# Shizheng-Wen/GAOT-3D

Hardware: AMD Instinct MI355X
Metric: mesh-points/sec fwd+bwd, 500K-pt DrivAerNet++ sample (higher is better)
Workload: dtype bf16; 1 GPU; configs[1]: one 500000-point car-like surface sample, latent 64x64x32, knn k=8 encoder + flipped decoder, C=32 P=2 d=256 h=8 F=1024 L=10 rope, attention dropout 0.1 (training mode), MSE + AdamW step; CSR build and geoembed stats inside the step (a decoder list that is the encoder's with its rows swapped shares the encoder's two lists); points=500000, edges=4000000, edges_decoder=4000000, layers=10, precision=bf16, points_per_gpu=500000, point_order=random

## Files before the change

gaot_3d_amd/_lib.py:

```python
from __future__ import annotations

import ctypes as C
import os

_HERE = os.path.dirname(os.path.abspath(__file__))
LIB_PATH = os.environ.get("GAOT_LIB") or os.path.join(_HERE, "lib", "libgaot3d_hip.so")

MAX_MLP_LAYERS = 5


class GaotError(RuntimeError):
    pass


class MlpT(C.Structure):
    _fields_ = [("n_hidden", C.c_int), ("hidden", C.c_int), ("channels", C.c_int),
                ("weight", C.c_void_p * MAX_MLP_LAYERS), ("bias", C.c_void_p * MAX_MLP_LAYERS)]


class MlpGradT(C.Structure):
    _fields_ = [("weight", C.c_void_p * MAX_MLP_LAYERS), ("bias", C.c_void_p * MAX_MLP_LAYERS)]


_lib = None

_p, _i, _i64, _sz, _f, _d = C.c_void_p, C.c_int, C.c_int64, C.c_size_t, C.c_float, C.c_double

SIGNATURES = {
    "gaot_abi_version": (_i, []),
    "gaot_last_error": (C.c_char_p, []),
    "gaot_launch_count": (_i64, [_i]),
    "gaot_csr_workspace_bytes": (_sz, [_i64, _i64]),
    "gaot_csr_build": (_i, [_p, _i, _i64, _i, _i64, _p, _p, _p, _p, _p, _sz, _p]),
    "gaot_gno_fwd_workspace_bytes": (_sz, [_i64, _i]),
    "gaot_gno_fwd": (_i, [C.POINTER(MlpT), _p, _p, _p, _p, _p, _p, _i64, _i64, _p, _i, _p, _sz, _p]),
    "gaot_gno_bwd_workspace_bytes": (_sz, [C.POINTER(MlpT), _i64, _i64]),
    "gaot_gno_bwd": (_i, [C.POINTER(MlpT), _p, _p, _p, _p, _p, _p, _p, _p, _i64, _i64, _i64, _p,
                          C.POINTER(MlpGradT), _i, _p, _sz, _p]),
    "gaot_gno_bwd_coords": (_i, [C.POINTER(MlpT), _p, _p, _p, _p, _p, _p, _p, _p, _i64, _i64, _i64, _p,
                                 C.POINTER(MlpGradT), _p, _i, _p, _sz, _p]),
    "gaot_geoembed_stats_workspace_bytes": (_sz, []),
    "gaot_geoembed_moments": (_i, [_p, _p, _p, _p, _i64, _p, _p]),
    "gaot_geoembed_from_moments": (_i, [_p, _i64, _p, _p, _sz, _p]),
    "gaot_geoembed_raw": (_i, [_p, _p, _p, _p, _i64, _p, _p, _p, _sz, _p]),
    "gaot_geoembed_finalize": (_i, [_p, _i64, _p, _i64, _p, _sz, _p]),
    "gaot_geoembed_from_moments_bwd_workspace_bytes": (_sz, [_i64]),
    "gaot_geoembed_from_moments_bwd": (_i, [_p, _p, _i64, _p, _p, _sz, _p]),
    "gaot_geoembed_moments_bwd": (_i, [_p, _p, _p, _p, _i64, _p, _p, _p, _p]),
    "gaot_gemm_workspace_bytes": (_sz, [_i64, _i64, _i64]),
    "gaot_gemm": (_i, [_p, _p, _p, _i64, _i64, _i64, _i64, _i64, _i64, _i, _i, _p, _i, _p, _i64, _p, _i, _p, _sz, _p]),
    "gaot_gemm_ex": (_i, [_p, _p, _p, _i64, _i64, _i64, _i64, _i64, _i64, _i, _i, _i, _i, _i, _p, _i, _p, _i64, _p, _i, _p,
                          _sz, _p]),
    "gaot_attn_fwd": (_i, [_p, _p, _p, _p, _p, _i64, _i64, _i64, _i64, _i, _i, _i, _i, _i, _f, _f, _p, _i, _i, _i, _p]),
    "gaot_attn_bwd": (_i, [_p] * 10 + [_i64] * 8 + [_i, _i, _i, _i, _i, _f, _f, _p, _i, _i, _i, _i, _p]),
    "gaot_attn_bwd_fused_f32_scratch_bytes": (_i64, [_i, _i, _i]),
    "gaot_attn_bwd_fused_f32": (_i, [_p] * 10 + [_i64] * 8 + [_i, _i, _i, _i, _i, _f, _f, _p, _i, _i, _i, _p, C.c_size_t, _p]),
    "gaot_attn_hd_fwd": (_i, [_p, _p, _p, _p, _p, _i64, _i64, _i64, _i64, _i, _i, _i, _i, _i, _f, _f, _p, _i, _i, _p]),
    "gaot_attn_hd_bwd": (_i, [_p] * 10 + [_i64] * 8 + [_i, _i, _i, _i, _i, _f, _f, _p, _i, _i, _i, _p]),
    "gaot_attn_dropout_mask": (_i, [_p, _f, _i, _i, _i, _p, _p]),
    "gaot_dropout_seed_next": (_i, [_p, C.c_uint64, _p, _p]),
    "gaot_dropout_seed_block": (_i, [_p, C.c_uint64, _i, _p, _p]),
    "gaot_attn_bf16_image_bytes": (_sz, [_i, _i, _i, _i]),
    "gaot_rope_table": (_i, [_p, _i, _i, _p, _p]),
    "gaot_qkv_image": (_i, [_p, _p, _p, _i64, _i64, _i64, _i, _i, _i, _p, _f, _p]),
    "gaot_qkv_image_packed": (_i, [_p, _p, _p, _i64, _i64, _i64, _i64, _i, _i, _p, _f, _i, _p]),
    "gaot_pack_heads": (_i, [_p, _p, _i64, _i, _i, _i, _p, _p, _i, _i, _i, _p]),
    "gaot_attn_bwd_bf16_scratch_bytes": (_sz, [_i, _i, _i, _i]),
    "gaot_attn_bwd_bf16_fused_eligible": (_i, [_i, _i, _i, _i]),
    "gaot_attn_fwd_bf16": (_i, [_p, _p, _p, _p, _p, _i, _i, _i, _i, _i, _f, _f, _p, _i, _i, _p]),
    "gaot_attn_bwd_bf16": (_i, [_p, _p, _p, _p, _p, _p, _p, _p, _i, _i, _i, _i, _i, _f, _f, _p, _i, _i, _i, _p]),
    "gaot_rmsnorm_fwd": (_i, [_p, _p, _p, _p, _p, _i64, _i, _f, _p]),
    "gaot_rmsnorm_bwd_workspace_bytes": (_sz, [_i64, _i]),
    "gaot_rmsnorm_bwd": (_i, [_p, _p, _p, _p, _p, _p, _p, _i64, _i, _p, _sz, _p]),
    "gaot_rmsnorm_bwd2": (_i, [_p, _p, _p, _p, _p, _p, _p, _p, _i64, _i, _p, _sz, _p]),
    "gaot_colsum_workspace_bytes": (_sz, [_i64, _i64]),
    "gaot_colsum": (_i, [_p, _i64, _i64, _i64, _p, _p, _sz, _p]),
    "gaot_gemm_ex_partials": (_i, [_p, _p, _p, _i64, _i64, _i64, _i64, _i64, _i64, _i, _i, _i, _i, _i, _p, _sz, _p, _p, _p]),
    "gaot_rmsnorm_bwd_parts": (_i64, [_i64]),
    "gaot_colsum_parts": (_i64, [_i64]),
    "gaot_reduce_multi": (_i, [_p, _i, _p]),
    "gaot_rope": (_i, [_p, _i64, _i64, _i, _i, _i, _i, _p, _i, _p]),
    "gaot_swiglu_fwd": (_i, [_p, _p, _i64, _i, _p]),
    "gaot_swiglu_bwd": (_i, [_p, _p, _p, _i64, _i, _p]),
    "gaot_adamw_step": (_i, [_p, _i, _p, _p, _d, _d, _d, _d, _p]),
    "gaot_mlp2_fwd": (_i, [_p, _i64, _i, _i, _i, _p, _p, _p, _p, _p, _p]),
    "gaot_mlp2_bwd_workspace_bytes": (_sz, [_i, _i]),
    "gaot_mlp2_bwd": (_i, [_p, _i64, _i, _i, _i, _p, _p, _p, _p, _p, _p, _p, _p, _p, _sz, _p]),
    "gaot_knn_grid": (_i, [_p, _i64, _p, _p, _i, _p, _p]),
    "gaot_radius_grid_count": (_i, [_p, _i64, _p, _p, _f, _i, _p, _p]),
    "gaot_radius_grid_fill": (_i, [_p, _i64, _p, _p, _f, _i, _p, _p, _p, _p]),
    "gaot_knn_brute": (_i, [_p, _i64, _p, _i64, _i, _p, _p]),
    "gaot_radius_brute_count": (_i, [_p, _i64, _p, _i64, _f, _i, _p, _p]),
    "gaot_radius_brute_fill": (_i, [_p, _i64, _p, _i64, _f, _i, _p, _p, _p, _p]),
    "gaot_exclusive_scan_workspace_bytes": (_sz, [_i64]),
    "gaot_exclusive_scan_i32": (_i, [_p, _i64, _p, _p, _sz, _p]),
    "gaot_segment_cap_flags": (_i, [_p, _p, _i64, _i, _p, _p]),
    "gaot_unique_pair_flags": (_i, [_p, _p, _i64, _p, _p]),
    "gaot_random_keep_flags": (_i, [_p, _i64, _d, _p, _p]),
    "gaot_dropout": (_i, [_p, _p, _d, _i64, _p, _p]),
    "gaot_segment_random_cap_flags": (_i, [_p, _p, _p, _i64, _i, _p, _p]),
    "gaot_compact_pairs": (_i, [_p, _p, _p, _p, _i64, _p, _p, _p]),
    "gaot_cast_bf16": (_i, [_p, _p, _i64, _p]),
    "gaot_cast_bf16_multi": (_i, [_p, _i, _p]),
    "gaot_cast_bf16_transpose_multi": (_i, [_p, _p, _p, _i, _p]),
    "gaot_swiglu_fwd_bf16": (_i, [_p, _p, _i64, _i, _p]),
    "gaot_ffn_w13_swiglu": (_i, [_p, _p, _p, _p, _i64, _i64, _i64, _i, _p]),
    "gaot_ffn_w2_bwd_swiglu": (_i, [_p, _p, _p, _p, _i64, _i64, _i64, _i, _p]),
    "gaot_swiglu_bwd_bf16": (_i, [_p, _p, _p, _i64, _i, _p]),
    "gaot_ffn_packed_bytes": (_i64, [_i, _i]),
    "gaot_ffn_pack": (_i, [_p, _p, _i, _p, _i, _p]),
    "gaot_ffn_pack_multi": (_i, [_p, _i, _i, _i, _p]),
    "gaot_ffn_fwd": (_i, [_p, _p, _p, _i64, _p, _p, _p, _i64, _i, _p]),
    "gaot_norm_ffn_fwd": (_i, [_p, _i64, _p, _f, _p, _p, _p, _p, _i64, _i, _p]),
    "gaot_block_packed_bytes": (_i64, [_i]),
    "gaot_block_pack_multi": (_i, [_p, _i, _i, _p]),
    "gaot_block_tail_fwd": (_i, [_p, _i64, _p, _i64, _p, _f, _p, _p, _p, _p, _p, _i64, _i, _p]),
    "gaot_qkv_packed_bytes": (_i64, [_i64, _i]),
    "gaot_qkv_pack_multi": (_i, [_p, _i, _i64, _i, _p]),
    "gaot_norm_qkv_image": (_i, [_p, _i64, _p, _f, _p, _p, _p, _p, _i64, _i, _i, _i, _p, _f, _p]),
    "gaot_skip_packed_bytes": (_i64, []),
    "gaot_skip_pack_multi": (_i, [_p, _i, _p]),
    "gaot_cat_norm_qkv_image": (_i, [_p, _i64, _p, _i64, _p, _p, _p, _p, _f, _p, _p, _p, _p, _i64, _i, _i, _i, _p, _f, _p]),
    "gaot_norm_bwd_parts": (_i64, [_i64]),
    "gaot_ffn_bwd_norm": (_i, [_p, _p, _p, _p, _i64, _p, _p, _p, _p, _p, _p, _p, _i64, _i, _p]),
    "gaot_qkv_bwd_norm": (_i, [_p, _i64, _p, _p, _i64, _p, _p, _p, _p, _p, _p, _i64, _p]),
    "gaot_qkv_bwd_norm_cat": (_i, [_p, _i64, _p, _p, _i64, _p, _p, _p, _p, _p, _p, _p, _i, _p, _i64, _p]),
    "gaot_oproj_bwd_image": (_i, [_p, _p, _p, _i, _p, _p, _i64, _i, _p]),
    "gaot_ffn_bwd_dag": (_i, [_p, _p, _p, _p, _p, _p, _i64, _i, _p]),
    "gaot_ffn_bwd": (_i, [_p, _p, _p, _p, _p, _p, _p, _i, _i64, _i, _p]),
    "gaot_act_bwd": (_i, [_p, _p, _p, _i64, _i, _p]),
    "gaot_act_fwd": (_i, [_p, _p, _i64, _i, _p]),
    "gaot_axpy": (_i, [_p, _p, _f, _p, _i64, _i64, _p]),
    "gaot_stream_copy": (_i, [_p, _p, _i64, _p]),
    "gaot_stream_copy_ex": (_i, [_p, _p, _i64, _i, _p]),
    "gaot_patchify": (_i, [_p, _p, _i, _i, _i, _i, _i, _i, _i, _p]),
    "gaot_mse_workspace_bytes": (_sz, []),
    "gaot_mse_fwd": (_i, [_p, _p, _i64, _p, _p, _sz, _p]),
    "gaot_mse_bwd": (_i, [_p, _p, _i64, _p, _p, _p]),
    "gaot_gather_rows": (_i, [_p, _i64, _p, _i64, _i, _p, _i64, _p]),
    "gaot_segment_reduce": (_i, [_p, _i64, _p, _p, _i64, _i, _i, _p, _p, _p]),
    "gaot_segment_reduce_bwd": (_i, [_p, _p, _p, _p, _i64, _i64, _i, _i, _p, _p]),
    "gaot_segment_softmax_fwd": (_i, [_p, _p, _i64, _p, _p]),
    "gaot_segment_softmax_bwd": (_i, [_p, _p, _p, _i64, _p, _p]),
    "gaot_edge_coords": (_i, [_p, _p, _p, _p, _i64, _i, _p, _i64, _p]),
    "gaot_mul": (_i, [_p, _p, _i64, _i, _i, _p, _p]),
    "gaot_mul_rowsum": (_i, [_p, _p, _i64, _i, _p, _p]),
    "gaot_affine_cols": (_i, [_p, _p, _p, _i64, _i, _p, _p]),
    "gaot_scale_mix_fwd": (_i, [_p, _i, _p, _p, _p, _i64, _i, _p]),
    "gaot_scale_mix_bwd": (_i, [_p, _i, _p, _p, _p, _p, _i64, _i, _p]),
}


def load():
    global _lib
    if _lib is not None:
        return _lib
    if not os.path.exists(LIB_PATH):
        raise GaotError(f"{LIB_PATH} not found: build it with `python -c 'import __graft_entry__ as g; g.build()'` "
                        f"or `make -C gaot_3d_amd/csrc` (there is no CPU/PyTorch fallback)")
    lib = C.CDLL(LIB_PATH)
    for name, (res, args) in SIGNATURES.items():
        fn = getattr(lib, name)
        fn.restype = res
        fn.argtypes = args
    if lib.gaot_abi_version() != 11:
        raise GaotError("libgaot3d_hip.so ABI version mismatch")
    _lib = lib
    return lib


def check(rc: int, what: str):
    if rc != 0:
        msg = load().gaot_last_error()
        raise GaotError(f"{what} failed (code {rc}): {msg.decode() if msg else ''}")
```

gaot_3d_amd/csrc/attn_bf16.hip:

```cpp
#include <stdlib.h>

#include <type_traits>

#include "attn_dropout.h"
#include "common.h"
#include "tile32.h"

namespace {

constexpr int D = 32;
constexpr float LOG2E = 1.4426950408889634f;
constexpr float LN2 = 0.6931471805599453f;
typedef float f32x2 __attribute__((ext_vector_type(2)));

__device__ __forceinline__ float xhalf(float v) { return __shfl_xor(v, 32, 64); }
__device__ __forceinline__ float max_halves(float v) {
    const unsigned u = __builtin_bit_cast(unsigned, v);
    const auto r = __builtin_amdgcn_permlane32_swap(u, u, false, false);
    return fmaxf(__builtin_bit_cast(float, (unsigned)r[0]), __builtin_bit_cast(float, (unsigned)r[1]));
}

__device__ __forceinline__ void stage_load4(uint4 (&regs)[2], const bf16_t* pa, int64_t lda, const bf16_t* pb, int64_t ldb,
                                            int64_t row0, int64_t nrows) {
#pragma unroll
// ... 67 lines not shown
                          float* __restrict__ delta, int B, int S, int H) {
    const int64_t i = (int64_t)blockIdx.x * blockDim.x + threadIdx.x;
    const int64_t n = (int64_t)B * S * H;
    if (i >= n) return;
    const int head = (int)(i % H);
    const int64_t row = i / H;
    const float* dp = d_o + row * H * D + head * D;
    const float* op = o + row * H * D + head * D;
    bf16_t* yp = dob + row * H * D + head * D;
    float s = 0.f;
#pragma unroll
    for (int c = 0; c < D / 4; ++c) {
        const float4 a = *reinterpret_cast<const float4*>(dp + 4 * c);
        const float4 b = *reinterpret_cast<const float4*>(op + 4 * c);
        s += a.x * b.x + a.y * b.y + a.z * b.z + a.w * b.w;
        const uint2 pk = make_uint2((unsigned)f2bf(a.x) | ((unsigned)f2bf(a.y) << 16),
                                    (unsigned)f2bf(a.z) | ((unsigned)f2bf(a.w) << 16));
        *reinterpret_cast<uint2*>(yp + 4 * c) = pk;
    }
    delta[((row / S) * H + head) * S + (row % S)] = s;
}

__global__ void k_delta_bf16(const bf16_t* __restrict__ dob, const float* __restrict__ o, float* __restrict__ delta, int B,
                             int S, int H) {
    const int64_t i = (int64_t)blockIdx.x * blockDim.x + threadIdx.x;
    const int64_t n = (int64_t)B * S * H;
    if (i >= n) return;
    const int head = (int)(i % H);
    const int64_t row = i / H;
    const bf16_t* dp = dob + row * H * D + head * D;
    const float* op = o + row * H * D + head * D;
    float s = 0.f;
#pragma unroll
    for (int c = 0; c < D / 8; ++c) {
        const uint4 a = *reinterpret_cast<const uint4*>(dp + 8 * c);
        const float4 b0 = *reinterpret_cast<const float4*>(op + 8 * c), b1 = *reinterpret_cast<const float4*>(op + 8 * c + 4);
        s += __uint_as_float(a.x << 16) * b0.x + __uint_as_float(a.x & 0xffff0000u) * b0.y + __uint_as_float(a.y << 16) * b0.z +
             __uint_as_float(a.y & 0xffff0000u) * b0.w + __uint_as_float(a.z << 16) * b1.x + __uint_as_float(a.z & 0xffff0000u) * b1.y +
             __uint_as_float(a.w << 16) * b1.z + __uint_as_float(a.w & 0xffff0000u) * b1.w;
    }
    delta[((row / S) * H + head) * S + (row % S)] = s;
}

struct FwdArgs {
    const bf16_t* qkv;
    float* o;
    float* lse;
    int64_t ld;
    int B, S, H, HKV;
    gdrop::Drop drop;
    int chunk;
    int64_t o_part, lse_part;
    const float* kmax2;
    int* redo;
};

constexpr int KN_BLOCKS = 64;
__global__ __launch_bounds__(256) void k_key_norm_max(const bf16_t* __restrict__ img, int64_t ld, int S, int H, int HKV,
                                                      float* __restrict__ out) {
    __shared__ float red[4];
    const int b = blockIdx.y, hkv = blockIdx.z;
    float m = 0.f;
    for (int64_t row = (int64_t)blockIdx.x * 256 + threadIdx.x; row < S; row += (int64_t)KN_BLOCKS * 256) {
        const bf16_t* kp = img + ((int64_t)b * S + row) * ld + (H + hkv) * D;
        float n2 = 0.f;
#pragma unroll
        for (int c = 0; c < D / 8; ++c) {
            const uint4 a = *reinterpret_cast<const uint4*>(kp + 8 * c);
            const unsigned w[4] = {a.x, a.y, a.z, a.w};
#pragma unroll
            for (int j = 0; j < 4; ++j) {
                const float lo = __uint_as_float(w[j] << 16), hi = __uint_as_float(w[j] & 0xffff0000u);
                n2 = fmaf(lo, lo, fmaf(hi, hi, n2));
            }
        }
        m = fmaxf(m, n2);
    }
#pragma unroll
    for (int o = 32; o > 0; o >>= 1) m = fmaxf(m, __shfl_xor(m, o, 64));
    if ((threadIdx.x & 63) == 0) red[threadIdx.x >> 6] = m;
    __syncthreads();
    if (threadIdx.x == 0) out[((int64_t)b * KN_BLOCKS + blockIdx.x) * HKV + hkv] = fmaxf(fmaxf(red[0], red[1]), fmaxf(red[2], red[3]));
}

template <int NTILES>
__device__ __forceinline__ void stage_col_words(uint32_t* bw_s, uint32_t ck, int64_t k0) {
    if (threadIdx.x < 16 * NTILES) {
        const int t = threadIdx.x >> 4, jj = threadIdx.x & 15;
        bw_s[t * 16 + ((jj >> 1) & 1) * 8 + (jj >> 2) * 2 + (jj & 1)] = gdrop::col_word(ck, (uint32_t)(k0 >> 1) + threadIdx.x);
    }
}
template <bool ZERO>
__device__ __forceinline__ void drop_select(f32x16& v, const f32x16& other, uint32_t aw, const uint32_t* bw_tile, int hf,
                                            uint32_t thr) {
    const uint4 w0 = *reinterpret_cast<const uint4*>(bw_tile + hf * 8);
    const uint4 w1 = *reinterpret_cast<const uint4*>(bw_tile + hf * 8 + 4);
    const uint32_t wd[8] = {w0.x, w0.y, w0.z, w0.w, w1.x, w1.y, w1.z, w1.w};
#pragma unroll
    for (int j = 0; j < 8; ++j) {
        const uint32_t x = aw ^ wd[j];
        v[2 * j] = ((x & 0xffffu) >= thr) ? v[2 * j] : (ZERO ? 0.f : other[2 * j]);
        v[2 * j + 1] = ((x >> 16) >= thr) ? v[2 * j + 1] : (ZERO ? 0.f : other[2 * j + 1]);
    }
}

typedef short s16x2 __attribute__((ext_vector_type(2)));
// ... 16 lines not shown

constexpr float RESCALE_SUM = 64.0f;
template <int OCC, int TPM, bool DROP, bool FAST, int FSB = 0>
__global__ __launch_bounds__(256, OCC) void k_attn_fwd_bf16(FwdArgs a) {
    __shared__ __attribute__((aligned(16))) char lds[2 * TPM * TILE_BYTES];
    __shared__ __attribute__((aligned(16))) uint32_t bw_s[DROP ? 16 * TPM : 4];
    const int wave = threadIdx.x >> 6, lane = threadIdx.x & 63, l31 = lane & 31, hf = lane >> 5;
    const int head = blockIdx.x % a.H, b = blockIdx.z;
    const int hkv = head / (a.H / a.HKV);
    const int64_t q0 = (int64_t)(blockIdx.x / a.H) * 128 + wave * 32;
    const int64_t rowbase = (int64_t)b * a.S;
    const bf16_t* qp = a.qkv + rowbase * a.ld + head * D;
    const bf16_t* kp = a.qkv + rowbase * a.ld + (a.H + hkv) * D;
    const bf16_t* vp = a.qkv + rowbase * a.ld + (a.H + a.HKV + hkv) * D;

    bf16x8 qf[2];
    {
        const int64_t qi = q0 + l31;
#pragma unroll
        for (int s = 0; s < 2; ++s) {
            if (qi < a.S) qf[s] = *reinterpret_cast<const bf16x8*>(qp + qi * a.ld + 16 * s + 8 * hf);
            else {
#pragma unroll
                for (int j = 0; j < 8; ++j) qf[s][j] = 0;
            }
        }
    }
    f32x16 acc, negm;
#pragma unroll
    for (int r = 0; r < 16; ++r) { acc[r] = 0.f; negm[r] = 0.f; }
    float m = 0.f, l = 0.f;
    uint32_t aw = 0, ck = 0;
    if constexpr (DROP) {
        const unsigned long long seed = *a.drop.seed;
        const int bh = a.drop.bh(b, head);
        aw = gdrop::row_word(gdrop::row_key(seed, bh), (uint32_t)(q0 + l31)) ^ 0x80008000u;
        ck = gdrop::col_key(seed, bh);
    }
    const short ts = (short)((int)a.drop.thr - 1 - 32768);
    const s16x2 tpk = {ts, ts};

    const int wg = blockIdx.x + gridDim.x * (blockIdx.y + gridDim.y * blockIdx.z);
    if constexpr (FAST) {
        constexpr float BOUND2 = 54.f * 54.f;
        float q2 = 0.f;
#pragma unroll
        for (int s = 0; s < 2; ++s)
#pragma unroll
            for (int j = 0; j < 8; ++j) {
                const float v = __uint_as_float((unsigned)(unsigned short)qf[s][j] << 16);
                q2 = fmaf(v, v, q2);
            }
        q2 += xhalf(q2);
        float k2 = a.kmax2[((int64_t)b * KN_BLOCKS + lane) * a.HKV + hkv];
#pragma unroll
        for (int o = 32; o > 0; o >>= 1) k2 = fmaxf(k2, __shfl_xor(k2, o, 64));
        const int over = __syncthreads_or(!(q2 * k2 <= BOUND2));
        if (threadIdx.x == 0) a.redo[wg] = over ? 1 : 0;
        if (over) return;
    } else {
        if (a.redo[wg] == 0) return;
    }

    const int64_t lo = (int64_t)blockIdx.y * a.chunk, hi = min((int64_t)a.S, lo + a.chunk);
    uint4 regs[TPM];
    stage_loadN<TPM>(regs, kp, a.ld, vp, a.ld, lo, a.S);
    for (int64_t k0 = lo; k0 < hi; k0 += 32 * TPM) {
        __syncthreads();
        stage_storeN<TPM>(regs, lds);
        if constexpr (DROP) stage_col_words<TPM>(bw_s, ck, k0);
        __syncthreads();
        if (k0 + 32 * TPM < hi) stage_loadN<TPM>(regs, kp, a.ld, vp, a.ld, k0 + 32 * TPM, a.S);
        auto do_tile = [&](int t, int64_t kb) {
            const char* kt = lds + t * TILE_BYTES;
            const char* vt = lds + (TPM + t) * TILE_BYTES;
            const bool first = (kb == lo);
            f32x16 sc;
            auto scores = [&]() {
                sc = __builtin_amdgcn_mfma_f32_32x32x16_bf16(frag_rows(kt, l31, hf, 0), qf[0], negm, 0, 0, 0);
                sc = __builtin_amdgcn_mfma_f32_32x32x16_bf16(frag_rows(kt, l31, hf, 1), qf[1], sc, 0, 0, 0);
                if (kb + 32 > a.S) {
                    const int nv = (int)(a.S - kb);
    #pragma unroll
                    for (int r = 0; r < 16; ++r)
                        if (mfma32_row(r, hf) >= nv) sc[r] = -INFINITY;
                }
            };
            if constexpr (FAST) {
                if constexpr ((FSB & 1) != 0) __builtin_amdgcn_sched_barrier(0);
                f32x16 zero;
    #pragma unroll
                for (int r = 0; r < 16; ++r) zero[r] = 0.f;
                sc = __builtin_amdgcn_mfma_f32_32x32x16_bf16(frag_rows(kt, l31, hf, 0), qf[0], zero, 0, 0, 0);
                sc = __builtin_amdgcn_mfma_f32_32x32x16_bf16(frag_rows(kt, l31, hf, 1), qf[1], sc, 0, 0, 0);
                if (kb + 32 > a.S) {
                    const int nv = (int)(a.S - kb);
    #pragma unroll
                    for (int r = 0; r < 16; ++r)
                        if (mfma32_row(r, hf) >= nv) sc[r] = -INFINITY;
                }
    #pragma unroll
                for (int r = 0; r < 16; ++r) sc[r] = __builtin_amdgcn_exp2f(sc[r]);
                if constexpr ((FSB & 2) != 0) __builtin_amdgcn_sched_barrier(0);
                bf16x8 p0, p1;
                acc_to_frags(sc, p0, p1);
                if constexpr ((FSB & 8) != 0) {
                    typedef __bf16 bf16x2_t __attribute__((ext_vector_type(2)));
// ... 1292 lines not shown
            for (int g = 0; g < 4; ++g) {
                float4 t = make_float4(dk[4 * g] * ksc, dk[4 * g + 1] * ksc, dk[4 * g + 2] * ksc, dk[4 * g + 3] * ksc);
                *reinterpret_cast<float4*>(dkp + 8 * g + 4 * hf) = unrope4(t, a.freqs, (int)ki, g, hf);
                float4 u = make_float4(dv[4 * g] * vsc, dv[4 * g + 1] * vsc, dv[4 * g + 2] * vsc, dv[4 * g + 3] * vsc);
                *reinterpret_cast<float4*>(dvp + 8 * g + 4 * hf) = u;
            }
        }
    });
}

#include "attn_fwd_asm.inc"
struct FwdAsmLds {
    static constexpr int QT = GAOT_ATTN_FWD_ASM_QT, KT = GAOT_ATTN_FWD_ASM_KT;
    static constexpr int STAGE = 0;
    static constexpr int BW = STAGE + 2 * KT * TILE_BYTES;
    static constexpr int TOTAL = BW + 16 * KT * 4;
    static constexpr int QUERIES = 4 * QT * 32, KEYS = KT * 32;
};
template <bool DROP, int LAB = 0>
__global__ __launch_bounds__(256, 1) void k_attn_fwd_asm(FwdArgs a) {
    using L = FwdAsmLds;
    constexpr int QT = L::QT, KT = L::KT;
    __shared__ __attribute__((aligned(1024))) char lds[L::TOTAL];
    const int wave = threadIdx.x >> 6, lane = threadIdx.x & 63, l31 = lane & 31, hf = lane >> 5;
    const int head = blockIdx.x % a.H, b = blockIdx.z, qblk = blockIdx.x / a.H;
    const int hkv = head / (a.H / a.HKV);
    const int64_t q0 = (int64_t)qblk * L::QUERIES + wave * (QT * 32);
    const int64_t rowbase = (int64_t)b * a.S;
    const bf16_t* qp = a.qkv + rowbase * a.ld + head * D;
    const bf16_t* kp = a.qkv + rowbase * a.ld + (a.H + hkv) * D;
    const bf16_t* vp = a.qkv + rowbase * a.ld + (a.H + a.HKV + hkv) * D;

    float q2max = 0.f;
    static_for<0, QT>([&](auto qc) {
        constexpr int qt = decltype(qc)::value;
        const int64_t qi = q0 + 32 * qt + l31;
        float q2 = 0.f;
        static_for<0, 2>([&](auto sc) {
            constexpr int s = decltype(sc)::value;
            const uint4 f = *reinterpret_cast<const uint4*>(qp + qi * a.ld + 16 * s + 8 * hf);
            agpr_write4<8 * qt + 4 * s>(f);
            const unsigned w[4] = {f.x, f.y, f.z, f.w};
#pragma unroll
            for (int j = 0; j < 4; ++j) {
                const float lo = __uint_as_float(w[j] << 16), hi = __uint_as_float(w[j] & 0xffff0000u);
                q2 = fmaf(lo, lo, fmaf(hi, hi, q2));
            }
        });
        q2 += xhalf(q2);
        q2max = fmaxf(q2max, q2);
    });
    {
        constexpr float BOUND2 = 54.f * 54.f;
        float k2 = a.kmax2[((int64_t)b * KN_BLOCKS + lane) * a.HKV + hkv];
#pragma unroll
        for (int o = 32; o > 0; o >>= 1) k2 = fmaxf(k2, __shfl_xor(k2, o, 64));
        const int over = __syncthreads_or(!(q2max * k2 <= BOUND2));
        if (threadIdx.x < 4)
            a.redo[(qblk * 4 + threadIdx.x) * a.H + head + (int64_t)(a.S / 128) * a.H * (blockIdx.y + gridDim.y * b)] = over ? 1 : 0;
        if (over) return;
    }
    uint32_t aw[QT] = {0, 0, 0, 0}, ck = 0;
    if constexpr (DROP) {
        const unsigned long long seed = *a.drop.seed;
        const int bh = a.drop.bh(b, head);
        const uint32_t rk = gdrop::row_key(seed, bh);
        ck = gdrop::col_key(seed, bh);
#pragma unroll
        for (int qt = 0; qt < QT; ++qt) aw[qt] = gdrop::row_word(rk, (uint32_t)(q0 + 32 * qt + l31)) ^ 0x80008000u;
    }
    const uint32_t ts = (uint32_t)((int)a.drop.thr - 1 - 32768) & 0xffffu;
    const uint32_t tpk = ts | (ts << 16);
    asm volatile(GAOT_ATTN_FWD_ASM_ZERO_ACC ::: GAOT_ATTN_FWD_ASM_ACC_CLOBBERS);
    float l0[QT] = {0.f, 0.f, 0.f, 0.f}, l1[QT] = {0.f, 0.f, 0.f, 0.f};

    const unsigned lbase = (unsigned)(uintptr_t)(__attribute__((address_space(3))) char*)lds;
    const unsigned a_k0 = lbase + L::STAGE + tile_off(l31, hf), a_k1 = lbase + L::STAGE + tile_off(l31, 2 + hf);
    unsigned a_v0, a_v1;
    {
        const int i = lane & 15, grp = (lane >> 4) & 1, col = 16 * grp + 4 * (i & 3), r0 = 4 * hf + (i >> 2), r1 = r0 + 8;
        a_v0 = lbase + L::STAGE + tile_off(r0, col >> 3) + ((col & 7) << 1);
        a_v1 = lbase + L::STAGE + tile_off(r1, col >> 3) + ((col & 7) << 1);
    }
    const unsigned a_w = lbase + L::BW + hf * 32;
    uint32_t* bw_s = reinterpret_cast<uint32_t*>(lds + L::BW);

    const int64_t lo = (int64_t)blockIdx.y * a.chunk, hi = min((int64_t)a.S, lo + a.chunk);
    uint4 regs[KT];
    stage_loadN<KT>(regs, kp, a.ld, vp, a.ld, lo, a.S);
    for (int64_t k0 = lo; k0 < hi; k0 += L::KEYS) {
        __syncthreads();
        stage_storeN<KT>(regs, lds + L::STAGE);
        if constexpr (DROP) stage_col_words<KT>(bw_s, ck, k0);
        __syncthreads();
        if (k0 + L::KEYS < hi) stage_loadN<KT>(regs, kp, a.ld, vp, a.ld, k0 + L::KEYS, a.S);
        if constexpr (LAB == 1) continue;
#if GAOT_ATTN_FWD_ASM_LSUM_MFMA
        if constexpr (DROP)
            asm volatile(GAOT_ATTN_FWD_STAGE_ASM_DROP
                         :: [a_k0] "v"(a_k0), [a_k1] "v"(a_k1), [a_v0] "v"(a_v0), [a_v1] "v"(a_v1), [a_w] "v"(a_w),
                            [aw0] "v"(aw[0]), [aw1] "v"(aw[1]), [aw2] "v"(aw[2]), [aw3] "v"(aw[3]), [tpk] "s"(tpk)
                         : GAOT_ATTN_FWD_STAGE_ASM_CLOBBERS);
        else
            asm volatile(GAOT_ATTN_FWD_STAGE_ASM_NODROP
                         :: [a_k0] "v"(a_k0), [a_k1] "v"(a_k1), [a_v0] "v"(a_v0), [a_v1] "v"(a_v1)
                         : GAOT_ATTN_FWD_STAGE_ASM_CLOBBERS);
#else
// ... 85 lines not shown
    const int64_t li = ((row / S) * H + head) * S + (row % S);
    float mx = -INFINITY;
    for (int p = 0; p < P; ++p) mx = fmaxf(mx, lse_parts[p * lse_part + li]);
    float den = 0.f;
    for (int p = 0; p < P; ++p) den += __expf(lse_parts[p * lse_part + li] - mx);
    float4 acc = make_float4(0.f, 0.f, 0.f, 0.f);
    const int64_t oi = row * (H * D) + head * D + 4 * g;
    for (int p = 0; p < P; ++p) {
        const float w = __expf(lse_parts[p * lse_part + li] - mx) / den;
        const float4 v = *reinterpret_cast<const float4*>(o_parts + p * o_part + oi);
        acc.x += w * v.x; acc.y += w * v.y; acc.z += w * v.z; acc.w += w * v.w;
    }
    *reinterpret_cast<float4*>(o + oi) = acc;
    if (g == 0) lse[li] = mx + logf(den);
}

__global__ void k_sum_parts(const float* __restrict__ parts, int P, int64_t part, int64_t n4, float* __restrict__ out) {
    const int64_t i = (int64_t)blockIdx.x * blockDim.x + threadIdx.x;
    if (i >= n4) return;
    float4 acc = reinterpret_cast<const float4*>(parts)[i];
    for (int p = 1; p < P; ++p) {
        const float4 v = reinterpret_cast<const float4*>(parts + p * part)[i];
        acc.x += v.x; acc.y += v.y; acc.z += v.z; acc.w += v.w;
    }
    reinterpret_cast<float4*>(out)[i] = acc;
}

__global__ void k_sum_cols(const float* __restrict__ parts, int P, int64_t part, int64_t rows, int ld, int col0, int ncols,
                           float* __restrict__ out) {
    const int64_t i = (int64_t)blockIdx.x * blockDim.x + threadIdx.x;
    const int c4 = ncols / 4;
    if (i >= rows * c4) return;
    const int64_t off = (i / c4) * ld + col0 + 4 * (i % c4);
    float4 acc = *reinterpret_cast<const float4*>(parts + off);
    for (int p = 1; p < P; ++p) {
        const float4 v = *reinterpret_cast<const float4*>(parts + p * part + off);
        acc.x += v.x; acc.y += v.y; acc.z += v.z; acc.w += v.w;
    }
    *reinterpret_cast<float4*>(out + off) = acc;
}

int split_parts(int64_t wgs, int S) {
    constexpr int tgt = 2048;
    if (wgs >= tgt / 2) return 1;
    int p = (int)std::min<int64_t>(8, ceil_div(tgt, wgs));
    p = std::min(p, std::max(1, S / 1024));
    return std::max(p, 1);
}
int split_chunk(int S, int P) { return (int)(ceil_div(ceil_div(S, P), 128) * 128); }

}

static size_t align256(size_t v) { return (v + 255) & ~(size_t)255; }
static size_t key_norm_off(int B, int S, int H, int HKV) { return (sizeof(bf16_t) * (size_t)B * S * (H + 2 * HKV) * D + 64 + 15) & ~(size_t)15; }
static size_t fwd_flags(int B, int S, int H) { return (size_t)B * 8 * (size_t)ceil_div(S, 128) * H; }
static size_t image_only_bytes(int B, int S, int H, int HKV) {
    return align256(key_norm_off(B, S, H, HKV) + sizeof(float) * (size_t)B * KN_BLOCKS * HKV + sizeof(int) * fwd_flags(B, S, H));
}

extern "C" size_t gaot_attn_bf16_image_bytes(int B, int S, int H, int HKV) {
    const int P = split_parts(ceil_div(S, 128) * H * B, S);
    size_t parts = P > 1 ? (size_t)P * ((size_t)B * S * H * D + (size_t)B * H * S) * sizeof(float) : 0;
    return image_only_bytes(B, S, H, HKV) + parts;
}
static size_t fused_dqpart_bytes(int B, int S, int H) { return (size_t)B * H * (size_t)ceil_div(S, 512) * (size_t)S * D * sizeof(bf16_t); }
static int fused_parts(int B, int S, int HKV) {
    const int64_t wgs = (int64_t)ceil_div(S, 512) * HKV * B;
    int p = 1;
    while (wgs * p < 256 && p < 8 && S / (2 * p) >= 1024) p *= 2;
    return p;
}
static int fused_chunk(int S, int P) { return (int)(ceil_div(ceil_div(S, P), 64) * 64); }
static bool fused_bwd_ok(int B, int S, int H, int HKV) {
    return (int64_t)ceil_div(S, 512) * HKV * B * fused_parts(B, S, HKV) >= 128 && fused_dqpart_bytes(B, S, H) <= ((size_t)1 << 30) &&
           (int64_t)S * (H + 2 * HKV) * D * 2 < 0x7fffffff;
}
extern "C" int gaot_attn_bwd_bf16_fused_eligible(int B, int S, int H, int HKV) { return fused_bwd_ok(B, S, H, HKV) ? 1 : 0; }
static size_t bwd_parts_bytes(int B, int S, int H, int HKV) {
    const int P = std::max(split_parts(ceil_div(S, 128) * H * B, S), fused_bwd_ok(B, S, H, HKV) ? fused_parts(B, S, HKV) : 1);
    return P > 1 ? align256((size_t)P * (size_t)B * S * (H + 2 * HKV) * D * sizeof(float)) : 0;
}
extern "C" size_t gaot_attn_bwd_bf16_scratch_bytes(int B, int S, int H, int HKV) {
    const size_t dqpart = fused_bwd_ok(B, S, H, HKV) ? fused_dqpart_bytes(B, S, H) : 0;
    return align256(sizeof(bf16_t) * (size_t)B * S * H * D + 64) + bwd_parts_bytes(B, S, H, HKV) + dqpart;
}

extern "C" int gaot_attn_fwd_bf16(const float* qkv, const float* rope_freqs, void* qkv_image, float* o, float* lse,
                                  int B, int S, int H, int HKV, int head_dim, float scale, float dropout_p,
                                  const unsigned long long* dropout_seed, int head0, int heads_total, gaot_stream_t stream) {
    GAOT_ENTER();
    if (head_dim != D) {
        gaot_set_error("gaot_attn_fwd_bf16: head_dim %d unsupported (only 32)", head_dim);
        return GAOT_ERR_UNSUPPORTED;
    }
    GAOT_CHECK_ARG(B > 0 && S > 0 && H > 0 && HKV > 0 && H % HKV == 0, "bad shape");
    GAOT_CHECK_ARG(qkv_image && o && lse, "null pointer");
    GAOT_CHECK_ARG((((uintptr_t)qkv | (uintptr_t)qkv_image | (uintptr_t)o) & 15) == 0, "buffers must be 16-byte aligned");
    GAOT_CHECK_ARG(dropout_p >= 0.f && dropout_p < 1.f && (dropout_p == 0.f || dropout_seed), "dropout_p in [0,1) and a seed");
    GAOT_CHECK_ARG(heads_total == 0 || (head0 >= 0 && head0 + H <= heads_total), "head0 + H <= heads_total");
    hipStream_t st = (hipStream_t)stream;
    const int ld = (H + 2 * HKV) * D;
    const int64_t rows = (int64_t)B * S;
    const int64_t n = rows * (ld / 2);
    if (qkv)
        GAOT_KLAUNCH(k_prep_qkv, dim3((unsigned)ceil_div(n, 256)), dim3(256), 0, st, qkv, (bf16_t*)qkv_image, rows, ld, H,
                     HKV, S, rope_freqs, scale * LOG2E);
    float* kmax2 = reinterpret_cast<float*>(reinterpret_cast<char*>(qkv_image) + key_norm_off(B, S, H, HKV));
    int* redo = reinterpret_cast<int*>(kmax2 + (size_t)B * KN_BLOCKS * HKV);
    GAOT_KLAUNCH(k_key_norm_max, dim3(KN_BLOCKS, (unsigned)B, (unsigned)HKV), dim3(256), 0, st, (const bf16_t*)qkv_image,
                 (int64_t)ld, S, H, HKV, kmax2);
    const int P = split_parts(ceil_div(S, 128) * H * B, S);
    float* o_parts = reinterpret_cast<float*>(reinterpret_cast<char*>(qkv_image) + image_only_bytes(B, S, H, HKV));
    const int64_t o_part = rows * H * D, lse_part = (int64_t)B * H * S;
    float* lse_parts = o_parts + (size_t)P * o_part;
    FwdArgs a{(const bf16_t*)qkv_image, P > 1 ? o_parts : o, P > 1 ? lse_parts : lse, ld, B, S, H, HKV,
              gdrop::make_drop(dropout_seed, dropout_p, H, head0, heads_total), P > 1 ? split_chunk(S, P) : S, o_part, lse_part, kmax2, redo};
    const dim3 fgrid((unsigned)(ceil_div(S, 128) * H), (unsigned)(P > 1 ? ceil_div(S, a.chunk) : 1), (unsigned)B);
    static const int fwd_lab = [] { const char* e = getenv("GAOT_ATTN_FWD_LAB"); return e ? atoi(e) : 0; }();
    const bool dot2 = fwd_lab == 8 || (fwd_lab != 1 && a.drop.thr);
    const bool fwd_asm = [] { const char* e = getenv("GAOT_ATTN_FWD_ASM"); return !e || atoi(e) != 0; }();
    if (fwd_asm && fwd_lab == 0 && S % FwdAsmLds::QUERIES == 0 && (P == 1 || a.chunk % FwdAsmLds::KEYS == 0) &&
        (int64_t)(S / FwdAsmLds::QUERIES) * H * B * fgrid.y >= 128) {
        const dim3 agrid((unsigned)((S / FwdAsmLds::QUERIES) * H), fgrid.y, (unsigned)B);
        static const int asm_lab = [] { const char* e = getenv("GAOT_ATTN_FWD_ASM_LAB"); return e ? atoi(e) : 0; }();
        if (asm_lab == 1) {
            if (a.drop.thr) GAOT_KLAUNCH((k_attn_fwd_asm<true, 1>), agrid, dim3(256), 0, st, a);
            else GAOT_KLAUNCH((k_attn_fwd_asm<false, 1>), agrid, dim3(256), 0, st, a);
        } else if (a.drop.thr) {
            GAOT_KLAUNCH((k_attn_fwd_asm<true>), agrid, dim3(256), 0, st, a);
            GAOT_KLAUNCH((k_attn_fwd_bf16<3, 4, true, false>), fgrid, dim3(256), 0, st, a);
        } else {
            GAOT_KLAUNCH((k_attn_fwd_asm<false>), agrid, dim3(256), 0, st, a);
            GAOT_KLAUNCH((k_attn_fwd_bf16<3, 4, false, false>), fgrid, dim3(256), 0, st, a);
        }
    } else if (a.drop.thr) {
        if (dot2) GAOT_KLAUNCH((k_attn_fwd_bf16<4, 4, true, true, 8>), fgrid, dim3(256), 0, st, a);
        else GAOT_KLAUNCH((k_attn_fwd_bf16<4, 4, true, true>), fgrid, dim3(256), 0, st, a);
        GAOT_KLAUNCH((k_attn_fwd_bf16<3, 4, true, false>), fgrid, dim3(256), 0, st, a);
    } else {
        if (dot2) GAOT_KLAUNCH((k_attn_fwd_bf16<4, 4, false, true, 8>), fgrid, dim3(256), 0, st, a);
        else GAOT_KLAUNCH((k_attn_fwd_bf16<4, 4, false, true>), fgrid, dim3(256), 0, st, a);
        GAOT_KLAUNCH((k_attn_fwd_bf16<3, 4, false, false>), fgrid, dim3(256), 0, st, a);
    }
    if (P > 1)
        GAOT_KLAUNCH(k_attn_combine, dim3((unsigned)ceil_div(rows * H * 8, 256)), dim3(256), 0, st, o_parts, lse_parts,
                           (int)fgrid.y, o_part, lse_part, B, S, H, o, lse);
    GAOT_LAUNCH_CHECK();
    return GAOT_OK;
}

extern "C" int gaot_attn_bwd_bf16(const void* qkv_image, const float* o, const float* d_o, const float* lse,
                                  void* do_image, float* delta, float* dqkv, const float* rope_freqs, int B, int S, int H,
                                  int HKV, int head_dim, float scale, float dropout_p,
                                  const unsigned long long* dropout_seed, int head0, int heads_total, int phase_mask,
                                  gaot_stream_t stream) {
    GAOT_ENTER();
    if (head_dim != D) {
        gaot_set_error("gaot_attn_bwd_bf16: head_dim %d unsupported (only 32)", head_dim);
        return GAOT_ERR_UNSUPPORTED;
    }
    GAOT_CHECK_ARG(B > 0 && S > 0 && H > 0 && HKV > 0 && H % HKV == 0, "bad shape");
    GAOT_CHECK_ARG(qkv_image && o && (d_o || !(phase_mask & 1)) && lse && do_image && delta && dqkv, "null pointer");
    GAOT_CHECK_ARG(dropout_p >= 0.f && dropout_p < 1.f && (dropout_p == 0.f || dropout_seed), "dropout_p in [0,1) and a seed");
    GAOT_CHECK_ARG(heads_total == 0 || (head0 >= 0 && head0 + H <= heads_total), "head0 + H <= heads_total");
    hipStream_t st = (hipStream_t)stream;
    const int ld = (H + 2 * HKV) * D;
    const int P0 = split_parts(ceil_div(S, 128) * H * B, S);
    const bool kb_dkv = (int64_t)ceil_div(S, 256) * HKV * B >= 512, kb_dq = (int64_t)ceil_div(S, 256) * H * B >= 512;
    const int P = (kb_dkv || kb_dq) ? 1 : P0;
// ... 126 lines not shown
```

gaot_3d_amd/csrc/csr.hip:

```cpp
#include "csr_impl.h"

extern "C" size_t gaot_csr_workspace_bytes(int64_t num_edges, int64_t num_rows) {
    (void)num_rows;
    const int64_t nblk = ceil_div(num_edges, RS_TILE);
    const int64_t tn = 256 * nblk;
    const int64_t nbt = ceil_div(tn, SCAN_TILE);
    return sizeof(int) * (size_t)(4 + 4 * num_edges + 2 * (tn + 1) + nbt + 1) + 64;
}

extern "C" int gaot_csr_build(const void* edge_index, int index_is_i64, int64_t num_edges, int sort_row,
                              int64_t num_rows, int32_t* rowptr, int32_t* perm, int32_t* key_sorted,
                              int32_t* other_sorted, void* workspace, size_t workspace_bytes, gaot_stream_t stream) {
    GAOT_ENTER();
    GAOT_CHECK_ARG(num_edges >= 0 && num_rows >= 0, "negative size");
    GAOT_CHECK_ARG(num_edges < (int64_t)1 << 31 && num_rows < ((int64_t)1 << 31) - 1, "sizes must fit int32");
    GAOT_CHECK_ARG(sort_row == 0 || sort_row == 1, "sort_row must be 0 or 1");
    GAOT_CHECK_ARG(rowptr && workspace, "null pointer");
    GAOT_CHECK_ARG(num_edges == 0 || (edge_index && perm && key_sorted && other_sorted), "null pointer");
    GAOT_CHECK_ARG(workspace_bytes >= gaot_csr_workspace_bytes(num_edges, num_rows), "workspace too small");
    hipStream_t st = (hipStream_t)stream;
    int rc = index_is_i64 ? csr_build_t<int64_t>((const int64_t*)edge_index, num_edges, sort_row, num_rows, rowptr,
                                                 perm, key_sorted, other_sorted, workspace, st)
                          : csr_build_t<int32_t>((const int32_t*)edge_index, num_edges, sort_row, num_rows, rowptr,
                                                 perm, key_sorted, other_sorted, workspace, st);
    if (rc != GAOT_OK) return rc;
    GAOT_LAUNCH_CHECK();
    return GAOT_OK;
}
```

gaot_3d_amd/csrc/csr_impl.h:

```cpp
#pragma once
#include "common.h"

namespace {

__global__ void k_zero_flags(int* __restrict__ p, int n) {
    if ((int)threadIdx.x < n) p[threadIdx.x] = 0;
}

template <typename IDX>
__global__ void k_check_sorted(const IDX* __restrict__ keys, int64_t E, int* __restrict__ unsorted) {
    int64_t i = (int64_t)blockIdx.x * blockDim.x + threadIdx.x;
    const int64_t stride = (int64_t)gridDim.x * blockDim.x;
    bool bad = false;
    for (; i < E; i += stride) bad |= (i > 0) && (keys[i] < keys[i - 1]);
    if (__any(bad) && (threadIdx.x & 63) == 0) *unsorted = 1;
}

template <typename IDX>
__global__ void k_sorted_build(const IDX* __restrict__ keys, const IDX* __restrict__ other, int64_t E, int64_t Q,
                               const int* __restrict__ unsorted, int* __restrict__ rowptr, int* __restrict__ perm,
                               int* __restrict__ key_sorted, int* __restrict__ other_sorted) {
    if (*unsorted) return;
    int64_t i = (int64_t)blockIdx.x * blockDim.x + threadIdx.x;
    const int64_t stride = (int64_t)gridDim.x * blockDim.x;
    for (; i < E; i += stride) {
        const int k = (int)keys[i];
        perm[i] = (int)i;
        key_sorted[i] = k;
        other_sorted[i] = (int)other[i];
        const int kprev = (i > 0) ? (int)keys[i - 1] : -1;
        for (int r = kprev + 1; r <= k; ++r) rowptr[r] = (int)i;
        if (i == E - 1)
            for (int64_t r = (int64_t)k + 1; r <= Q; ++r) rowptr[r] = (int)E;
    }
}

constexpr int SCAN_BLOCK = 256;
constexpr int SCAN_ITEMS = 8;
constexpr int SCAN_TILE = SCAN_BLOCK * SCAN_ITEMS;

__global__ void k_scan_reduce(const int* __restrict__ in, int64_t n, int* __restrict__ block_sums) {
    __shared__ int red[SCAN_BLOCK / 64];
    const int64_t base = (int64_t)blockIdx.x * SCAN_TILE;
    int s = 0;
#pragma unroll
    for (int j = 0; j < SCAN_ITEMS; ++j) {
        int64_t i = base + (int64_t)threadIdx.x * SCAN_ITEMS + j;
        if (i < n) s += in[i];
    }
#pragma unroll
    for (int o = 32; o > 0; o >>= 1) s += __shfl_xor(s, o, 64);
    if ((threadIdx.x & 63) == 0) red[threadIdx.x >> 6] = s;
    __syncthreads();
    if (threadIdx.x == 0) {
        int t = 0;
        for (int w = 0; w < SCAN_BLOCK / 64; ++w) t += red[w];
        block_sums[blockIdx.x] = t;
    }
}

__global__ void k_scan_blocksums(int* __restrict__ block_sums, int nb) {
    __shared__ int carry;
    __shared__ int wsum[SCAN_BLOCK / 64];
    if (threadIdx.x == 0) carry = 0;
    __syncthreads();
    for (int base = 0; base < nb; base += SCAN_BLOCK) {
        int i = base + threadIdx.x;
        int v = (i < nb) ? block_sums[i] : 0;
        int incl = v;
        const int lane = threadIdx.x & 63;
#pragma unroll
        for (int o = 1; o < 64; o <<= 1) {
            int t = __shfl_up(incl, o, 64);
            if (lane >= o) incl += t;
        }
        if (lane == 63) wsum[threadIdx.x >> 6] = incl;
        __syncthreads();
        int woff = 0;
        for (int w = 0; w < (int)(threadIdx.x >> 6); ++w) woff += wsum[w];
        const int c = carry;
        if (i < nb) block_sums[i] = c + woff + incl - v;
        __syncthreads();
        if (threadIdx.x == SCAN_BLOCK - 1) carry = c + woff + incl;
        __syncthreads();
    }
}

__global__ void k_scan_apply(const int* __restrict__ in, int64_t n, const int* __restrict__ block_offs,
                             int* __restrict__ out) {
    __shared__ int wsum[SCAN_BLOCK / 64];
    const int64_t base = (int64_t)blockIdx.x * SCAN_TILE + (int64_t)threadIdx.x * SCAN_ITEMS;
    int v[SCAN_ITEMS];
    int s = 0;
#pragma unroll
    for (int j = 0; j < SCAN_ITEMS; ++j) {
        v[j] = (base + j < n) ? in[base + j] : 0;
        s += v[j];
    }
    int incl = s;
    const int lane = threadIdx.x & 63;
#pragma unroll
    for (int o = 1; o < 64; o <<= 1) {
        int t = __shfl_up(incl, o, 64);
        if (lane >= o) incl += t;
    }
    if (lane == 63) wsum[threadIdx.x >> 6] = incl;
    __syncthreads();
    int off = block_offs[blockIdx.x];
    for (int w = 0; w < (int)(threadIdx.x >> 6); ++w) off += wsum[w];
    int run = off + incl - s;
#pragma unroll
    for (int j = 0; j < SCAN_ITEMS; ++j) {
        if (base + j < n) {
            out[base + j] = run;
        }
        run += v[j];
        if (base + j == n - 1) out[n] = run;
    }
}

constexpr int RS_TILE = 4096;
constexpr int RS_ROUNDS = RS_TILE / 256;

template <typename KIN>
__global__ __launch_bounds__(256) void k_rs_hist(const KIN* __restrict__ keys, int64_t E, int shift, int nd, int nblk,
                                                 int* __restrict__ table, const int* __restrict__ unsorted) {
    __shared__ int h[256];
    if (!*unsorted) return;
    h[threadIdx.x] = 0;
    __syncthreads();
    const int64_t base = (int64_t)blockIdx.x * RS_TILE;
#pragma unroll 4
    for (int j = 0; j < RS_ROUNDS; ++j) {
        const int64_t i = base + j * 256 + threadIdx.x;
        if (i < E) atomicAdd(&h[((int)keys[i] >> shift) & (nd - 1)], 1);
    }
    __syncthreads();
    if ((int)threadIdx.x < nd) table[(int64_t)threadIdx.x * nblk + blockIdx.x] = h[threadIdx.x];
}

template <typename KIN>
__global__ __launch_bounds__(256) void k_rs_scatter(const KIN* __restrict__ keys_in, const int* __restrict__ ids_in,
                                                    int64_t E, int shift, int nbits, int nblk,
                                                    const int* __restrict__ table, int* __restrict__ keys_out,
                                                    int* __restrict__ ids_out, const int* __restrict__ unsorted) {
    __shared__ int wcnt[4][256];
    if (!*unsorted) return;
    const int wave = threadIdx.x >> 6, lane = threadIdx.x & 63;
    const int nd = 1 << nbits;
    const int64_t base = (int64_t)blockIdx.x * RS_TILE + (int64_t)wave * (RS_ROUNDS * 64);
    for (int i = threadIdx.x; i < 4 * 256; i += 256) (&wcnt[0][0])[i] = 0;
    __syncthreads();
    int key[RS_ROUNDS], rnk[RS_ROUNDS];
    const unsigned long long lt = (1ull << lane) - 1ull;
#pragma unroll
    for (int j = 0; j < RS_ROUNDS; ++j) {
        const int64_t idx = base + j * 64 + lane;
        const bool valid = idx < E;
        const int k = valid ? (int)keys_in[idx] : 0;
        const int d = (k >> shift) & (nd - 1);
        unsigned long long m = __ballot(valid);
        for (int b = 0; b < nbits; ++b) {
            const bool bit = (d >> b) & 1;
            const unsigned long long bb = __ballot(bit);
            m &= bit ? bb : ~bb;
        }
        const int r = __popcll(m & lt);
        const int before = wcnt[wave][d];
        rnk[j] = before + r;
        key[j] = k;
        if (valid && r == 0) wcnt[wave][d] = before + __popcll(m);
    }
    __syncthreads();
    if ((int)threadIdx.x < nd) {
        int run = table[(int64_t)threadIdx.x * nblk + blockIdx.x];
#pragma unroll
        for (int w = 0; w < 4; ++w) {
            const int c = wcnt[w][threadIdx.x];
            wcnt[w][threadIdx.x] = run;
            run += c;
        }
    }
    __syncthreads();
#pragma unroll
    for (int j = 0; j < RS_ROUNDS; ++j) {
        const int64_t idx = base + j * 64 + lane;
        if (idx < E) {
            const int pos = wcnt[wave][(key[j] >> shift) & (nd - 1)] + rnk[j];
            keys_out[pos] = key[j];
            ids_out[pos] = ids_in ? ids_in[idx] : (int)idx;
        }
    }
}

template <typename IDX>
__global__ void k_emit_sorted(const int* __restrict__ keys, const int* __restrict__ ids, const IDX* __restrict__ other,
                              int64_t E, int64_t Q, const int* __restrict__ unsorted, int* __restrict__ rowptr,
                              int* __restrict__ perm, int* __restrict__ key_sorted, int* __restrict__ other_sorted) {
    if (!*unsorted) return;
    int64_t i = (int64_t)blockIdx.x * blockDim.x + threadIdx.x;
    const int64_t stride = (int64_t)gridDim.x * blockDim.x;
    for (; i < E; i += stride) {
        const int k = keys[i], id = ids[i];
        perm[i] = id;
        key_sorted[i] = k;
        other_sorted[i] = (int)other[id];
        const int kprev = (i > 0) ? keys[i - 1] : -1;
        for (int r = kprev + 1; r <= k; ++r) rowptr[r] = (int)i;
        if (i == E - 1)
            for (int64_t r = (int64_t)k + 1; r <= Q; ++r) rowptr[r] = (int)E;
    }
}

static int rs_bits(int64_t Q) {
    int b = 1;
    while (((int64_t)1 << b) < Q) ++b;
    return b;
}

template <typename IDX>
int csr_build_t(const IDX* edge_index, int64_t E, int sort_row, int64_t Q, int32_t* rowptr, int32_t* perm,
                int32_t* key_sorted, int32_t* other_sorted, void* ws, hipStream_t st) {
    const IDX* keys = edge_index + (sort_row ? E : 0);
    const IDX* other = edge_index + (sort_row ? 0 : E);
    const int nblk = (int)ceil_div(E, RS_TILE);
    const int64_t tn = (int64_t)256 * nblk;
    int* flags = (int*)ws;
    int* unsorted = flags + 1;
    int* kbuf0 = flags + 4;
    int* kbuf1 = kbuf0 + E;
    int* ibuf0 = kbuf1 + E;
    int* ibuf1 = ibuf0 + E;
    int* table = ibuf1 + E;
    int* tscan = table + tn + 1;
    int* bsum = tscan + tn + 1;
    GAOT_KLAUNCH(k_zero_flags, dim3(1), dim3(64), 0, st, flags, 4);
    if (E == 0) {
        (void)hipMemsetAsync(rowptr, 0, sizeof(int) * (size_t)(Q + 1), st);
        return GAOT_OK;
    }
    const int tb = 256;
    const int gb = (int)std::min<int64_t>(ceil_div(E, tb), 256 * 16);
    GAOT_KLAUNCH((k_check_sorted<IDX>), dim3(gb), dim3(tb), 0, st, keys, E, unsorted);
    GAOT_KLAUNCH((k_sorted_build<IDX>), dim3(gb), dim3(tb), 0, st, keys, other, E, Q, unsorted, rowptr, perm,
                       key_sorted, other_sorted);
    const int bits = rs_bits(Q);
    const int passes = (bits + 7) / 8;
    const int width = (bits + passes - 1) / passes;
    const int* kin = nullptr;
    const int* iin = nullptr;
    for (int p = 0; p < passes; ++p) {
        const int shift = p * width;
        const int nd = 1 << width;
        int* kout = (p & 1) ? kbuf1 : kbuf0;
        int* iout = (p & 1) ? ibuf1 : ibuf0;
        const int64_t n = (int64_t)nd * nblk;
        const int nb = (int)ceil_div(n, SCAN_TILE);
        if (p == 0) GAOT_KLAUNCH((k_rs_hist<IDX>), dim3(nblk), dim3(256), 0, st, keys, E, shift, nd, nblk, table, unsorted);
        else GAOT_KLAUNCH((k_rs_hist<int>), dim3(nblk), dim3(256), 0, st, kin, E, shift, nd, nblk, table, unsorted);
        GAOT_KLAUNCH(k_scan_reduce, dim3(nb), dim3(SCAN_BLOCK), 0, st, table, n, bsum);
        GAOT_KLAUNCH(k_scan_blocksums, dim3(1), dim3(SCAN_BLOCK), 0, st, bsum, nb);
        GAOT_KLAUNCH(k_scan_apply, dim3(nb), dim3(SCAN_BLOCK), 0, st, table, n, bsum, tscan);
        if (p == 0)
            GAOT_KLAUNCH((k_rs_scatter<IDX>), dim3(nblk), dim3(256), 0, st, keys, (const int*)nullptr, E, shift, width,
                               nblk, tscan, kout, iout, unsorted);
        else
            GAOT_KLAUNCH((k_rs_scatter<int>), dim3(nblk), dim3(256), 0, st, kin, iin, E, shift, width, nblk, tscan,
                               kout, iout, unsorted);
        kin = kout;
        iin = iout;
    }
    GAOT_KLAUNCH((k_emit_sorted<IDX>), dim3(gb), dim3(tb), 0, st, kin, iin, other, E, Q, unsorted, rowptr, perm,
                       key_sorted, other_sorted);
    return GAOT_OK;
}

}
```

gaot_3d_amd/csrc/ffn_fused.hip:

```cpp
#include "common.h"

namespace {

typedef unsigned short bf16_t;
typedef unsigned u32x4 __attribute__((ext_vector_type(4)));

#ifndef GAOT_FFN_ABL
#define GAOT_FFN_ABL 0
#endif
#ifdef GAOT_FFN_TIMING
__device__ unsigned long long g_ffn_t[64];
#define FFN_STAMP(i) do { if (blockIdx.x == 0 && threadIdx.x == 0) g_ffn_t[i] = __builtin_readcyclecounter(); } while (0)
#else
#define FFN_STAMP(i) do { } while (0)
#endif
constexpr int D = 256, RB = 64, FC = 128;
constexpr int H_BYTES = RB * D * 2;
constexpr int U_BYTES = RB * FC * 2;
constexpr int AG_BYTES = RB * 2 * FC * 2;

__device__ __forceinline__ unsigned pack2(float a, float b) {
    return (unsigned)__builtin_bit_cast(bf16_t, (__bf16)a) | ((unsigned)__builtin_bit_cast(bf16_t, (__bf16)b) << 16);
}
__device__ __forceinline__ float rbf(float v) { return __uint_as_float((unsigned)__builtin_bit_cast(bf16_t, (__bf16)v) << 16); }
// ... 1368 lines not shown
        gaot_set_error("gaot_oproj_bwd_image: too many rows for 32-bit buffer offsets");
        return GAOT_ERR_UNSUPPORTED;
    }
    const bf16_t* wotp = (const bf16_t*)packed + ((int64_t)2 * F * D + (int64_t)D * F) * 2 + (int64_t)D * D;
    const int nblk = ((int)rows + RB - 1) / RB, per = (nblk + 7) / 8;
    GAOT_KLAUNCH(k_oproj_bwd, dim3((unsigned)(8 * per)), dim3(256), H_BYTES, (hipStream_t)stream, dh, attn_out, (const u32x4*)wotp, (bf16_t*)do_image,
                 delta, (int)rows, S, D / 32);
    GAOT_LAUNCH_CHECK();
    return GAOT_OK;
}

namespace {
struct QkvTable {
    const float* w[PACK_MAX];
    bf16_t* packed[PACK_MAX];
};
__global__ void k_qkv_pack(QkvTable t, int N, int with_backward) {
    const float* w = t.w[blockIdx.y];
    bf16_t* p = t.packed[blockIdx.y];
    const int nfr = N * D / 8;
    for (int id = blockIdx.x * blockDim.x + threadIdx.x; id < nfr * (with_backward ? 2 : 1); id += gridDim.x * blockDim.x) {
        if (id < nfr) {
            const int lane = id & 63, s2 = (id >> 6) & 15, jt = (id >> 10) & 1, wv = (id >> 11) & 3, pn = id >> 13;
            const float* src = w + (int64_t)(256 * pn + 64 * wv + 32 * jt + (lane & 31)) * D + 16 * s2 + 8 * (lane >> 5);
            *reinterpret_cast<u32x4*>(p + (int64_t)id * 8) = u32x4{pack2(src[0], src[1]), pack2(src[2], src[3]), pack2(src[4], src[5]), pack2(src[6], src[7])};
        } else {
            const int i2 = id - nfr, ns = N / 16;
            const int lane = i2 & 63, rest = i2 >> 6, s2 = rest % ns, jt = (rest / ns) & 1, wv = rest / (2 * ns);
            const float* st = w + (int64_t)(16 * s2 + 8 * (lane >> 5)) * D + (wv * 64 + jt * 32 + (lane & 31));
            *reinterpret_cast<u32x4*>(p + (int64_t)id * 8) =
                u32x4{pack2(st[0], st[D]), pack2(st[2 * D], st[3 * D]), pack2(st[4 * D], st[5 * D]), pack2(st[6 * D], st[7 * D])};
        }
    }
}

__global__ void k_skip_pack(QkvTable t) {
    const float* w = t.w[blockIdx.y];
    bf16_t* p = t.packed[blockIdx.y];
    for (int id = blockIdx.x * blockDim.x + threadIdx.x; id < D * 2 * D / 8; id += gridDim.x * blockDim.x) {
        const int lane = id & 63, s2 = (id >> 6) & 31, jt = (id >> 11) & 1, wv = id >> 12;
        const float* src = w + (int64_t)(64 * wv + 32 * jt + (lane & 31)) * (2 * D) + 16 * s2 + 8 * (lane >> 5);
        *reinterpret_cast<u32x4*>(p + (int64_t)id * 8) = u32x4{pack2(src[0], src[1]), pack2(src[2], src[3]), pack2(src[4], src[5]), pack2(src[6], src[7])};
        const int s3 = (id >> 6) & 15, jt3 = (id >> 10) & 1, w3 = (id >> 11) & 3, half = id >> 13;
        const float* st = w + (int64_t)(16 * s3 + 8 * (lane >> 5)) * (2 * D) + (256 * half + 64 * w3 + 32 * jt3 + (lane & 31));
        *reinterpret_cast<u32x4*>(p + (int64_t)D * 2 * D + (int64_t)id * 8) =
            u32x4{pack2(st[0], st[2 * D]), pack2(st[4 * D], st[6 * D]), pack2(st[8 * D], st[10 * D]), pack2(st[12 * D], st[14 * D])};
    }
}

struct QkvArgs {
    const float* X; int ldx; const float* NW; float eps; const u32x4* Wp; bf16_t* IMG; bf16_t* YB; float* RSTD;
    const float* table; int S, nq, nk; float qscale; int M, N;
    const float* XB; int ldxb; const u32x4* WSp; const float* BS; float* XO;
};
constexpr int QKV_LDS = H_BYTES + 256 + 64 * 144, QKV_LDS_CAT = 2 * H_BYTES + 256 + 1024 + 64 * 144;
template <bool CAT>
__global__ __launch_bounds__(256, 1) void k_norm_qkv(QkvArgs a) {
    constexpr int RD = 3, LA = 2;
    extern __shared__ __attribute__((aligned(1024))) char lds[];
    const int wave = threadIdx.x >> 6, lane = threadIdx.x & 63, l31 = lane & 31, hf = lane >> 5;
    const int M = a.M, N = a.N, NP = N / 256;
    const int nblk = (M + RB - 1) / RB, per = (nblk + 7) / 8;
    const int t = (blockIdx.x & 7) * per + (blockIdx.x >> 3);
    if ((int)(blockIdx.x >> 3) >= per || t >= nblk) return;
    const int m0 = t * RB;
    const int wv = __builtin_amdgcn_readfirstlane(wave);
    const __amdgpu_buffer_rsrc_t wrs = __builtin_amdgcn_make_buffer_rsrc((void*)a.Wp, 0, N * D * 2, 0x00020000);
    u32x4 wr[RD][8];
    auto wload = [&](u32x4 (&dst)[8], int g) {
        const int pn = g >> 2, st = g & 3;
#pragma unroll
        for (int jt = 0; jt < 2; ++jt)
#pragma unroll
            for (int s2 = 0; s2 < 4; ++s2)
                dst[jt * 4 + s2] = __builtin_bit_cast(u32x4, __builtin_amdgcn_raw_buffer_load_b128(wrs, lane * 16, ((((pn * 4 + wv) * 2 + jt) * 16) + 4 * st + s2) * 1024, 0));
    };
    wload(wr[0], 0);
    wload(wr[1], 1);
    float* rstd_l = reinterpret_cast<float*>(lds + (CAT ? 2 * H_BYTES : H_BYTES));
    if constexpr (CAT) {
        const int sw0 = l31 & 15;
        const int64_t xab = (int64_t)M * a.ldx * 4, xbb = (int64_t)M * a.ldxb * 4, xob = (int64_t)M * D * 4, ybbytes = (int64_t)M * D * 2;
        const __amdgpu_buffer_rsrc_t xars = __builtin_amdgcn_make_buffer_rsrc((void*)a.X, 0, (int)(xab > 0x7fffffff ? 0x7fffffff : xab), 0x00020000);
        const __amdgpu_buffer_rsrc_t xbrs = __builtin_amdgcn_make_buffer_rsrc((void*)a.XB, 0, (int)(xbb > 0x7fffffff ? 0x7fffffff : xbb), 0x00020000);
        const __amdgpu_buffer_rsrc_t xors = __builtin_amdgcn_make_buffer_rsrc((void*)a.XO, 0, (int)(xob > 0x7fffffff ? 0x7fffffff : xob), 0x00020000);
        const __amdgpu_buffer_rsrc_t ybrs = __builtin_amdgcn_make_buffer_rsrc((void*)a.YB, 0, (int)(ybbytes > 0x7fffffff ? 0x7fffffff : ybbytes), 0x00020000);
        const __amdgpu_buffer_rsrc_t wsrs = __builtin_amdgcn_make_buffer_rsrc((void*)a.WSp, 0, D * 2 * D * 2, 0x00020000);
        u32x4 wo[2][8];
        auto woload = [&](u32x4 (&dst)[8], int st) {
#pragma unroll
            for (int jt = 0; jt < 2; ++jt)
#pragma unroll
                for (int s2 = 0; s2 < 4; ++s2)
                    dst[jt * 4 + s2] = __builtin_bit_cast(u32x4, __builtin_amdgcn_raw_buffer_load_b128(wsrs, lane * 16, (((wv * 2 + jt) * 32) + 4 * st + s2) * 1024, 0));
        };
        woload(wo[0], 0);
        woload(wo[1], 1);
#pragma unroll
        for (int half = 0; half < 2; ++half) {
            f32x4 d0[8], d1[8];
#pragma unroll
            for (int i = 0; i < 8; ++i) {
                const int row = 8 * i + (threadIdx.x >> 5), m = m0 + row;
                const unsigned off = m < M ? (unsigned)m * (unsigned)(half ? a.ldxb : a.ldx) * 4u + (unsigned)(threadIdx.x & 31) * 32u : 0x80000000u;
                d0[i] = __builtin_bit_cast(f32x4, __builtin_amdgcn_raw_buffer_load_b128(half ? xbrs : xars, off, 0, 0));
                d1[i] = __builtin_bit_cast(f32x4, __builtin_amdgcn_raw_buffer_load_b128(half ? xbrs : xars, off, 16, 0));
// ... 79 lines not shown
        }
    } else {
        const int64_t xbytes = (int64_t)M * a.ldx * 4, ybbytes = (int64_t)M * D * 2;
        const __amdgpu_buffer_rsrc_t xrs = __builtin_amdgcn_make_buffer_rsrc((void*)a.X, 0, (int)(xbytes > 0x7fffffff ? 0x7fffffff : xbytes), 0x00020000);
        const __amdgpu_buffer_rsrc_t ybrs = __builtin_amdgcn_make_buffer_rsrc((void*)a.YB, 0, (int)(ybbytes > 0x7fffffff ? 0x7fffffff : ybbytes), 0x00020000);
        const float4 g = reinterpret_cast<const float4*>(a.NW)[lane];
        float4 v[16];
        float ss[16];
#pragma unroll
        for (int j = 0; j < 16; ++j) {
            const int m = m0 + wave * 16 + j;
            v[j] = __builtin_bit_cast(float4, __builtin_amdgcn_raw_buffer_load_b128(xrs, m < M ? (unsigned)m * (unsigned)a.ldx * 4u + lane * 16u : 0x80000000u, 0, 0));
        }
#pragma unroll
        for (int j = 0; j < 16; ++j) {
            ss[j] = 0.f;
            ss[j] += v[j].x * v[j].x + v[j].y * v[j].y + v[j].z * v[j].z + v[j].w * v[j].w;
        }
#pragma unroll
        for (int o = 32; o > 0; o >>= 1)
#pragma unroll
            for (int j = 0; j < 16; ++j) ss[j] += __shfl_xor(ss[j], o, 64);
#pragma unroll
        for (int j = 0; j < 16; ++j) {
            const int rl = wave * 16 + j, m = m0 + rl;
            const float r = rsqrtf(ss[j] / (float)D + a.eps);
            const float4 o = make_float4(v[j].x * r * g.x, v[j].y * r * g.y, v[j].z * r * g.z, v[j].w * r * g.w);
            typedef unsigned u32x2 __attribute__((ext_vector_type(2)));
            const u32x2 pk = {pack2(o.x, o.y), pack2(o.z, o.w)};
            *reinterpret_cast<u32x2*>(lds + rl * 512 + ((((lane >> 1) ^ (rl & 15))) << 4) + 8 * (lane & 1)) = pk;
            __builtin_amdgcn_raw_buffer_store_b64(pk, ybrs, m < M ? (unsigned)m * (unsigned)D * 2u + lane * 8u : 0x80000000u, 0, 0);
            if (lane == 0) {
                rstd_l[rl] = r;
                if (m < M) a.RSTD[m] = r;
            }
        }
    }
    __builtin_amdgcn_s_barrier();
    const int64_t ibytes = (int64_t)M * N * 2;
    const __amdgpu_buffer_rsrc_t irs = __builtin_amdgcn_make_buffer_rsrc((void*)a.IMG, 0, (int)(ibytes > 0x7fffffff ? 0x7fffffff : ibytes), 0x00020000);
    const __amdgpu_buffer_rsrc_t trs = __builtin_amdgcn_make_buffer_rsrc((void*)a.table, 0, a.table ? a.S * 128 : 0, 0x00020000);
    const int sw = l31 & 15;
    const char* hb = lds + l31 * 512;
    char* tabl = lds + (CAT ? QKV_LDS_CAT : QKV_LDS) - 64 * 144;
    {
        const int row = threadIdx.x >> 2, pc = threadIdx.x & 3, m = m0 + row, mm = m < M ? m : M - 1;
        const f32x4 t0 = __builtin_bit_cast(f32x4, __builtin_amdgcn_raw_buffer_load_b128(trs, (mm % a.S) * 128 + 32 * pc, 0, 0));
        const f32x4 t1 = __builtin_bit_cast(f32x4, __builtin_amdgcn_raw_buffer_load_b128(trs, (mm % a.S) * 128 + 32 * pc + 16, 0, 0));
        *reinterpret_cast<f32x4*>(tabl + row * 144 + 32 * pc) = t0;
        *reinterpret_cast<f32x4*>(tabl + row * 144 + 32 * pc + 16) = t1;
    }
    __builtin_amdgcn_s_barrier();
    f32x16 accc[2][2], accn[2][2];
    bf16x8 hn0 = *reinterpret_cast<const bf16x8*>(hb + ((hf ^ sw) << 4)), hn1 = *reinterpret_cast<const bf16x8*>(hb + 32 * 512 + ((hf ^ sw) << 4));
    auto panel_step = [&](f32x16 (&acc)[2][2], int pn, int st, auto epi) {
        const int g = 4 * pn + st;
        auto run = [&](auto rot) {
            constexpr int R = decltype(rot)::value;
            wload(wr[(R + st + LA) % RD], g + LA);
#pragma unroll
            for (int s2 = 0; s2 < 4; ++s2) {
                __builtin_amdgcn_sched_barrier(0);
                const bf16x8 h0 = hn0, h1 = hn1;
                const int slot = ((2 * ((4 * st + s2 + 1) & 15) + hf) ^ sw) << 4;
                hn0 = *reinterpret_cast<const bf16x8*>(hb + slot);
                hn1 = *reinterpret_cast<const bf16x8*>(hb + 32 * 512 + slot);
                const bf16x8 w0 = __builtin_bit_cast(bf16x8, wr[(R + st) % RD][s2]), w1 = __builtin_bit_cast(bf16x8, wr[(R + st) % RD][4 + s2]);
                acc[0][0] = __builtin_amdgcn_mfma_f32_32x32x16_bf16(w0, h0, acc[0][0], 0, 0, 0);
                acc[1][0] = __builtin_amdgcn_mfma_f32_32x32x16_bf16(w1, h0, acc[1][0], 0, 0, 0);
                acc[0][1] = __builtin_amdgcn_mfma_f32_32x32x16_bf16(w0, h1, acc[0][1], 0, 0, 0);
                acc[1][1] = __builtin_amdgcn_mfma_f32_32x32x16_bf16(w1, h1, acc[1][1], 0, 0, 0);
                epi(4 * st + s2);
                __builtin_amdgcn_sched_group_barrier(0x100, 2, 0);
#pragma unroll
                for (int k = 0; k < 4; ++k) {
                    __builtin_amdgcn_sched_group_barrier(0x008, 1, 0);
                    __builtin_amdgcn_sched_group_barrier(0x002, 8, 0);
                }
            }
        };
        const int rot = (4 * pn) % 3;
        if (rot == 0) run(std::integral_constant<int, 0>{});
        else if (rot == 1) run(std::integral_constant<int, 1>{});
        else run(std::integral_constant<int, 2>{});
    };
    auto zero4 = [&](f32x16 (&acc)[2][2]) {
#pragma unroll
        for (int jt = 0; jt < 2; ++jt)
#pragma unroll
            for (int i = 0; i < 2; ++i)
#pragma unroll
                for (int r = 0; r < 16; ++r) acc[jt][i][r] = 0.f;
    };
    zero4(accc);
#pragma unroll
    for (int st = 0; st < 4; ++st) panel_step(accc, 0, st, [](int) {});
    for (int pn = 0; pn < NP; ++pn) {
        auto piece = [&](int e) {
            const int i = e >> 2, jt = (e >> 1) & 1, q0 = e & 1;
            const int m = m0 + 32 * i + l31;
            const unsigned rowoff = m < M ? (unsigned)m * (unsigned)N * 2u : 0x80000000u;
            const int head = 8 * pn + 2 * wave + jt;
            const bool rope = a.table && head < a.nq + a.nk;
            const float sc = head < a.nq ? a.qscale : 1.0f;
            unsigned pk[2][2];
#pragma unroll
            for (int h2 = 0; h2 < 2; ++h2) {
                const int q = q0 + 2 * h2;
                float v0 = accc[jt][i][4 * q], v1 = accc[jt][i][4 * q + 1], v2 = accc[jt][i][4 * q + 2], v3 = accc[jt][i][4 * q + 3];
                if (rope) {
                    const f32x4 tb = *reinterpret_cast<const f32x4*>(tabl + (32 * i + l31) * 144 + 16 * hf + 32 * q);
                    const float r0 = v0 * tb[0] - v1 * tb[1], r1 = v1 * tb[0] + v0 * tb[1];
                    const float r2 = v2 * tb[2] - v3 * tb[3], r3 = v3 * tb[2] + v2 * tb[3];
                    v0 = r0; v1 = r1; v2 = r2; v3 = r3;
                }
                pk[h2][0] = pack2(v0 * sc, v1 * sc);
                pk[h2][1] = pack2(v2 * sc, v3 * sc);
            }
            const auto r0 = __builtin_amdgcn_permlane32_swap(pk[0][0], pk[1][0], false, false);
            const auto r1 = __builtin_amdgcn_permlane32_swap(pk[0][1], pk[1][1], false, false);
            const u32x4 v = {(unsigned)r0[0], (unsigned)r1[0], (unsigned)r0[1], (unsigned)r1[1]};
            __builtin_amdgcn_raw_buffer_store_b128(v, irs, rowoff + (head * 32 + 8 * q0 + 16 * hf) * 2, 0, 0);
        };
        zero4(accn);
#pragma unroll
        for (int st = 0; st < 4; ++st)
            panel_step(accn, pn + 1, st, [&](int ks) { if ((ks & 1) == 0) piece(ks >> 1); });
        __builtin_amdgcn_sched_barrier(0);
#pragma unroll
        for (int jt = 0; jt < 2; ++jt)
#pragma unroll
            for (int i = 0; i < 2; ++i) accc[jt][i] = accn[jt][i];
    }
}
}

extern "C" int64_t gaot_qkv_packed_bytes(int64_t N, int with_backward) { return N * D * 2 * (with_backward ? 2 : 1); }

extern "C" int gaot_qkv_pack_multi(const gaot_qkv_pack_t* items, int num, int64_t N, int with_backward, gaot_stream_t stream) {
    GAOT_ENTER();
    GAOT_CHECK_ARG(items && num > 0 && N > 0 && N % 256 == 0, "bad argument (N must be a multiple of 256)");
    for (int i0 = 0; i0 < num; i0 += PACK_MAX) {
        QkvTable t{};
        const int n = std::min(PACK_MAX, num - i0);
        for (int i = 0; i < n; ++i) {
            GAOT_CHECK_ARG(items[i0 + i].w && items[i0 + i].packed && ((uintptr_t)items[i0 + i].packed % 16) == 0, "null or misaligned pointer in the table");
            t.w[i] = items[i0 + i].w; t.packed[i] = (bf16_t*)items[i0 + i].packed;
        }
        GAOT_KLAUNCH(k_qkv_pack, dim3((unsigned)std::min<int64_t>(ceil_div(N * D / 8 * (with_backward ? 2 : 1), 256), 256), (unsigned)n), dim3(256), 0,
                     (hipStream_t)stream, t, (int)N, with_backward);
    }
    GAOT_LAUNCH_CHECK();
    return GAOT_OK;
}

extern "C" int gaot_norm_qkv_image(const float* x, int64_t ldx, const float* norm_weight, float eps, const void* packed, void* image, void* yb,
                                   float* rstd, int64_t rows, int S, int H, int HKV, const float* rope_table, float qscale, gaot_stream_t stream) {
    GAOT_ENTER();
    const int64_t N = (int64_t)(H + 2 * HKV) * 32;
    GAOT_CHECK_ARG(x && norm_weight && packed && image && yb && rstd && rows > 0 && S > 0 && H > 0 && HKV > 0 && N % 256 == 0,
                   "bad argument ((H + 2 HKV) * 32 must be a multiple of 256)");
    GAOT_CHECK_ARG(((uintptr_t)x % 16) == 0 && ((uintptr_t)norm_weight % 16) == 0 && ((uintptr_t)packed % 16) == 0 && ((uintptr_t)image % 16) == 0 &&
                   ((uintptr_t)yb % 16) == 0 && ldx % 4 == 0 && ldx >= D, "16-byte alignment");
    if (rows * N * 2 >= 0x7fffffff || rows * ldx * 4 >= 0x7fffffff) {
        gaot_set_error("gaot_norm_qkv_image: too many rows for 32-bit buffer offsets");
        return GAOT_ERR_UNSUPPORTED;
    }
    static bool attr_set = false;
    if (!attr_set) {
        hipError_t e = hipFuncSetAttribute((const void*)k_norm_qkv<false>, hipFuncAttributeMaxDynamicSharedMemorySize, QKV_LDS);
        if (e != hipSuccess) {
            gaot_set_error("norm_qkv: cannot set dynamic LDS %d: %s", QKV_LDS, hipGetErrorString(e));
            return GAOT_ERR_LAUNCH;
        }
        attr_set = true;
    }
    const QkvArgs a{x, (int)ldx, norm_weight, eps, (const u32x4*)packed, (bf16_t*)image, (bf16_t*)yb, rstd, rope_table, S, H, HKV, qscale, (int)rows, (int)N,
                    nullptr, 0, nullptr, nullptr, nullptr};
    const int nblk = ((int)rows + RB - 1) / RB, per = (nblk + 7) / 8;
    GAOT_KLAUNCH(k_norm_qkv<false>, dim3((unsigned)(8 * per)), dim3(256), QKV_LDS, (hipStream_t)stream, a);
    GAOT_LAUNCH_CHECK();
    return GAOT_OK;
}

extern "C" int64_t gaot_skip_packed_bytes(void) { return 2 * (int64_t)D * 2 * D * 2; }
extern "C" int gaot_skip_pack_multi(const gaot_qkv_pack_t* items, int num, gaot_stream_t stream) {
    GAOT_ENTER();
    GAOT_CHECK_ARG(items && num > 0, "bad argument");
    for (int i0 = 0; i0 < num; i0 += PACK_MAX) {
        QkvTable t{};
        const int n = std::min(PACK_MAX, num - i0);
        for (int i = 0; i < n; ++i) {
            GAOT_CHECK_ARG(items[i0 + i].w && items[i0 + i].packed && ((uintptr_t)items[i0 + i].packed % 16) == 0, "null or misaligned pointer in the table");
            t.w[i] = items[i0 + i].w; t.packed[i] = (bf16_t*)items[i0 + i].packed;
        }
        GAOT_KLAUNCH(k_skip_pack, dim3(64, (unsigned)n), dim3(256), 0, (hipStream_t)stream, t);
    }
    GAOT_LAUNCH_CHECK();
    return GAOT_OK;
}
extern "C" int gaot_cat_norm_qkv_image(const float* xa, int64_t ldxa, const float* xb, int64_t ldxb, const void* skip_packed, const float* skip_bias,
                                       float* x_out, const float* norm_weight, float eps, const void* packed, void* image, void* yb, float* rstd,
                                       int64_t rows, int S, int H, int HKV, const float* rope_table, float qscale, gaot_stream_t stream) {
    GAOT_ENTER();
    const int64_t N = (int64_t)(H + 2 * HKV) * 32;
    GAOT_CHECK_ARG(xa && xb && skip_packed && x_out && norm_weight && packed && image && yb && rstd && rows > 0 && S > 0 && H > 0 && HKV > 0 &&
                   N % 256 == 0, "bad argument ((H + 2 HKV) * 32 must be a multiple of 256)");
    GAOT_CHECK_ARG(((uintptr_t)xa % 16) == 0 && ((uintptr_t)xb % 16) == 0 && ((uintptr_t)skip_packed % 16) == 0 && ((uintptr_t)skip_bias % 16) == 0 &&
                   ((uintptr_t)x_out % 16) == 0 && ((uintptr_t)norm_weight % 16) == 0 && ((uintptr_t)packed % 16) == 0 && ((uintptr_t)image % 16) == 0 &&
                   ((uintptr_t)yb % 16) == 0 && ldxa % 4 == 0 && ldxa >= D && ldxb % 4 == 0 && ldxb >= D, "16-byte alignment");
    if (rows * N * 2 >= 0x7fffffff || rows * ldxa * 4 >= 0x7fffffff || rows * ldxb * 4 >= 0x7fffffff) {
        gaot_set_error("gaot_cat_norm_qkv_image: too many rows for 32-bit buffer offsets");
        return GAOT_ERR_UNSUPPORTED;
    }
    static bool attr_set = false;
    if (!attr_set) {
        hipError_t e = hipFuncSetAttribute((const void*)k_norm_qkv<true>, hipFuncAttributeMaxDynamicSharedMemorySize, QKV_LDS_CAT);
        if (e != hipSuccess) {
            gaot_set_error("cat_norm_qkv: cannot set dynamic LDS %d: %s", QKV_LDS_CAT, hipGetErrorString(e));
            return GAOT_ERR_LAUNCH;
        }
        attr_set = true;
    }
    const QkvArgs a{xa, (int)ldxa, norm_weight, eps, (const u32x4*)packed, (bf16_t*)image, (bf16_t*)yb, rstd, rope_table, S, H, HKV, qscale, (int)rows, (int)N,
                    xb, (int)ldxb, (const u32x4*)skip_packed, skip_bias, x_out};
    const int nblk = ((int)rows + RB - 1) / RB, per = (nblk + 7) / 8;
    GAOT_KLAUNCH(k_norm_qkv<true>, dim3((unsigned)(8 * per)), dim3(256), QKV_LDS_CAT, (hipStream_t)stream, a);
    GAOT_LAUNCH_CHECK();
    return GAOT_OK;
}

extern "C" int64_t gaot_norm_bwd_parts(int64_t rows) { return (rows + RB - 1) / RB; }

extern "C" int gaot_ffn_bwd_norm(const void* yb, const float* dy, const void* packed, const float* h, int64_t ldh, const float* norm_weight,
                                 const float* rstd, void* dag, void* u, void* dyb, float* dh, float* dw_part, int64_t rows, int F,
                                 gaot_stream_t stream) {
    GAOT_ENTER();
    GAOT_CHECK_ARG(yb && dy && packed && h && norm_weight && rstd && dag && u && dh && dw_part && rows > 0 && F > 0 && F % FC == 0,
                   "bad argument (F must be a multiple of 128)");
    GAOT_CHECK_ARG(((uintptr_t)yb % 16) == 0 && ((uintptr_t)packed % 16) == 0 && ((uintptr_t)dy % 16) == 0 && ((uintptr_t)dag % 16) == 0 &&
                   ((uintptr_t)u % 16) == 0 && ((uintptr_t)dyb % 16) == 0 && ((uintptr_t)dh % 16) == 0 && ((uintptr_t)h % 16) == 0 &&
                   ((uintptr_t)norm_weight % 16) == 0 && ldh % 4 == 0 && ldh >= D, "16-byte alignment");
    if (rows * (int64_t)F * 4 >= 0x7fffffff) {
        gaot_set_error("gaot_ffn_bwd_norm: rows * F too large for 32-bit buffer offsets");
        return GAOT_ERR_UNSUPPORTED;
    }
    static_assert(BWDX_LDS >= NB_LDS, "the epilogue reuses the kernel's LDS");
    static bool attr_set = false;
    if (!attr_set) {
        hipError_t e = hipFuncSetAttribute((const void*)k_ffn_bwd_dx<true>, hipFuncAttributeMaxDynamicSharedMemorySize, BWDX_LDS);
        if (e != hipSuccess) {
            gaot_set_error("ffn_bwd_norm: cannot set dynamic LDS %d: %s", BWDX_LDS, hipGetErrorString(e));
            return GAOT_ERR_LAUNCH;
        }
        attr_set = true;
    }
    const bf16_t* p = (const bf16_t*)packed;
    const bf16_t* w2tp = p + (int64_t)2 * F * D + (int64_t)D * F;
    const bf16_t* w13tp = w2tp + (int64_t)D * F;
    const int nblk = ((int)rows + RB - 1) / RB, per = (nblk + 7) / 8;
    GAOT_KLAUNCH(k_ffn_bwd_dx<true>, dim3((unsigned)(8 * per)), dim3(256), BWDX_LDS, (hipStream_t)stream, (const bf16_t*)yb, dy, (const u32x4*)p,
                 (const u32x4*)w2tp, (const u32x4*)w13tp, (bf16_t*)dag, (bf16_t*)u, (bf16_t*)dyb, dh, (int)rows, F, 1,
                 NormBwdArgs{h, (int)ldh, norm_weight, rstd, dw_part});
    GAOT_LAUNCH_CHECK();
    return GAOT_OK;
}

namespace {
struct QkvBwdArgs {
    const float* DQKV; const u32x4* WTp; const float* X; int ldx; const float* NW; const float* RSTD; const float* DRES; const float* DTAP;
    float* DX; float* DWP; int M, N;
    const u32x4* WSTp; float* DXA; float* DXB; int same;
};
constexpr int QKVB_LDS = NB_LDS > 2 * H_BYTES ? NB_LDS : 2 * H_BYTES, QKVB_LDS_CAT = NB_LDS + H_BYTES;
template <bool CATB>
__global__ __launch_bounds__(256, 1) void k_qkv_bwd_norm(QkvBwdArgs a) {
    constexpr int RD = 3, LA = 2;
    extern __shared__ __attribute__((aligned(1024))) char lds[];
// ... 201 lines not shown
```

gaot_3d_amd/csrc/gno.hip:

```cpp
#include <type_traits>

#include "gno_common.h"

namespace {

using namespace gno;

template <int NH, int H>
struct FwdLds {
    static constexpr int KB = H / 32;
    static constexpr int w0 = 0;
    static constexpr int b0 = w0 + IN0P * H;
    static constexpr int wl = b0 + H;
    static constexpr int wL = wl + (NH - 1) * (H * H + H);
    static constexpr int bL = wL + H * 32;
    static constexpr int weights_end = bL + 32;
};

template <int NH, int H, int T>
__global__ __launch_bounds__(256, 2) void k_gno_fwd(MlpPtrs mlp, const float* __restrict__ y_pos,
                                                    const float* __restrict__ x_pos, const float* __restrict__ f_y,
                                                    const int* __restrict__ src_s, const int* __restrict__ dst_s,
                                                    const int* __restrict__ rowptr, int64_t E, float* __restrict__ out,
                                                    float* __restrict__ part) {
// ... 690 lines not shown
                + (size_t)num_queries * 32;
    return sizeof(float) * fl + gaot_gno_bwd_bf16_image_bytes(mlp->n_hidden) + 512;
}

namespace {
#define GNO_BWD_CHECK(cond, msg)                          \
    do {                                                  \
        if (!(cond)) {                                    \
            gaot_set_error("%s: %s", fn, msg);            \
            return GAOT_ERR_ARG;                          \
        }                                                 \
    } while (0)
int gno_bwd_impl(const char* fn, const gaot_mlp_t* mlp, const float* y_pos, const float* x_pos, const float* f_y,
                 const float* grad_out, const int32_t* rowptr_dst, const int32_t* src_sorted, const int32_t* dst_sorted,
                 const int32_t* rowptr_src, int64_t num_edges, int64_t num_sources, int64_t num_queries, float* grad_f_y,
                 const gaot_mlp_grad_t* grads, float* gcoord, int precision, void* workspace, size_t workspace_bytes,
                 gaot_stream_t stream) {
    GNO_BWD_CHECK(mlp && grads, "null mlp");
    if (!mlp_supported(mlp, true, precision)) {
        gaot_set_error("%s: unsupported MLP shape (n_hidden=%d hidden=%d channels=%d; four hidden layers in bf16 mode only)", fn,
                       mlp->n_hidden, mlp->hidden, mlp->channels);
        return GAOT_ERR_UNSUPPORTED;
    }
    GNO_BWD_CHECK(num_edges >= 0 && num_sources >= 0 && num_queries >= 0, "negative size");
    GNO_BWD_CHECK(precision != 1 || (num_sources <= (1 << 24) && num_queries <= (1 << 24)),
                   "bf16 GNO backward: more than 2^24 source or query rows (run the mesh point-sharded or in fp32 mode)");
    GNO_BWD_CHECK(precision != 1 || num_edges < ((int64_t)1 << 27),
                   "bf16 GNO backward: 2^27 or more edges in one launch (run the mesh point-sharded or in fp32 mode)");
    GNO_BWD_CHECK(workspace_bytes >= gaot_gno_bwd_workspace_bytes(mlp, num_edges, num_queries), "workspace too small");
    GNO_BWD_CHECK(rowptr_src && rowptr_dst, "null rowptr");
    hipStream_t st = (hipStream_t)stream;
    const int nh = mlp->n_hidden, h = mlp->hidden;
    const int total = param_total(nh, h);
    const int grid = bwd_grid(num_edges);
    const int n_waves = grid;
    float* part = (float*)workspace;
    float* wt = part + ceil_div(num_edges, 16) * 2 * 32;
    float* flat = wt + total;
    float* wpart = flat + total;
    float* gs = wpart + (size_t)grid * total;
    void* images = (void*)(((uintptr_t)(gs + (size_t)num_queries * 32) + 255) & ~(uintptr_t)255);
    GNO_BWD_CHECK(precision == 0 || precision == 1, "precision must be 0 (fp32) or 1 (bf16 matrix cores)");

    MlpPtrs p, pt;
    int off = 0;
    for (int l = 0; l <= nh; ++l) {
        p.w[l] = mlp->weight[l];
        p.b[l] = mlp->bias[l];
        GNO_BWD_CHECK(p.w[l] && p.b[l] && grads->weight[l] && grads->bias[l], "null MLP parameter / gradient");
        const int out_dim = (l == nh) ? 32 : h;
        const int in_dim = (l == 0) ? IN0 : h;
        pt.w[l] = wt + off;
        pt.b[l] = p.b[l];
        if (num_edges > 0)
            GAOT_KLAUNCH(k_transpose_w, dim3((unsigned)ceil_div(out_dim * in_dim, 256)), dim3(256), 0, st, p.w[l],
                               out_dim, in_dim, wt + off);
        off += out_dim * in_dim;
    }
    ScatterDesc sd;
    sd.n = 2 * (nh + 1);
    {
        int o = 0;
        for (int l = 0; l <= nh; ++l) {
            const int out_dim = (l == nh) ? 32 : h;
            const int in_dim = (l == 0) ? IN0 : h;
            sd.dst[2 * l] = grads->weight[l];
            sd.off[2 * l] = o;
            o += out_dim * in_dim;
            sd.dst[2 * l + 1] = grads->bias[l];
            sd.off[2 * l + 1] = o;
            o += out_dim;
        }
        sd.off[sd.n] = o;
    }
    if (num_edges == 0) {
        hipMemsetAsync(flat, 0, sizeof(float) * total, st);
    } else {
        GNO_BWD_CHECK(y_pos && x_pos && f_y && grad_out && src_sorted && dst_sorted && grad_f_y, "null pointer");
        const bool cg = gcoord != nullptr;
        GAOT_KLAUNCH(k_scale_by_inv_deg, dim3((unsigned)ceil_div(num_queries * 8, 256)), dim3(256), 0, st, grad_out,
                           rowptr_dst, num_queries, gs);
        int rc = GAOT_OK;
        if (precision == 1) {
            rc = gaot_gno_bwd_bf16_dispatch(nh, p.w, p.b, pt.w[0], images, y_pos, x_pos, f_y, gs, src_sorted, dst_sorted,
                                            rowptr_src, num_edges, grad_f_y, part, wpart, gcoord, grid, st);
        } else if (!cg) {
            switch (nh) {
                case 1: rc = launch_bwd<1, 64, false>(p, pt, y_pos, x_pos, f_y, gs, src_sorted, dst_sorted, rowptr_src, num_edges, grad_f_y, part, wpart, nullptr, grid, st); break;
                case 2: rc = launch_bwd<2, 64, false>(p, pt, y_pos, x_pos, f_y, gs, src_sorted, dst_sorted, rowptr_src, num_edges, grad_f_y, part, wpart, nullptr, grid, st); break;
                case 3: rc = launch_bwd<3, 64, false>(p, pt, y_pos, x_pos, f_y, gs, src_sorted, dst_sorted, rowptr_src, num_edges, grad_f_y, part, wpart, nullptr, grid, st); break;
            }
        } else {
            switch (nh) {
                case 1: rc = launch_bwd<1, 64, true>(p, pt, y_pos, x_pos, f_y, gs, src_sorted, dst_sorted, rowptr_src, num_edges, grad_f_y, part, wpart, gcoord, grid, st); break;
                case 2: rc = launch_bwd<2, 64, true>(p, pt, y_pos, x_pos, f_y, gs, src_sorted, dst_sorted, rowptr_src, num_edges, grad_f_y, part, wpart, gcoord, grid, st); break;
                case 3: rc = launch_bwd<3, 64, true>(p, pt, y_pos, x_pos, f_y, gs, src_sorted, dst_sorted, rowptr_src, num_edges, grad_f_y, part, wpart, gcoord, grid, st); break;
            }
        }
        if (rc != GAOT_OK) return rc;
        GAOT_KLAUNCH(k_reduce_params, dim3((unsigned)ceil_div(total, 64)), dim3(256), 0, st, wpart, n_waves,
                           total, flat);
    }
    GAOT_KLAUNCH(k_scatter_params, dim3((unsigned)ceil_div(total, 256)), dim3(256), 0, st, flat, sd);
    if (num_sources > 0) {
        const int64_t n = num_sources * 8;
        if (precision == 1)
            GAOT_KLAUNCH((k_segment_fixup<32, 4>), dim3(segment_fixup_grid(n)), dim3(256), 0, st, rowptr_src,
// ... 35 lines not shown
```

gaot_3d_amd/ops.py:

```python
from __future__ import annotations

import ctypes as C
import functools
import os
from dataclasses import dataclass
from typing import List, Optional, Sequence, Tuple

import torch

from . import _lib
from ._lib import GaotError, MlpGradT, MlpT, check

Tensor = torch.Tensor


_raw_stream = getattr(torch._C, "_cuda_getCurrentRawStream", None)


def _stream() -> C.c_void_p:
    if _raw_stream is not None:
        return C.c_void_p(_raw_stream(torch.cuda.current_device()))
    return C.c_void_p(torch.cuda.current_stream().cuda_stream)


# ... 38 lines not shown
        return False


def timing_reset(enabled: bool):
    TIMING["enabled"] = enabled
    TIMING["events"] = {}


def timing_summary():
    return {k: (len(v), sum(a.elapsed_time(b) for a, b in v)) for k, v in TIMING["events"].items()}


@dataclass
class SortedEdges:
    rowptr: Tensor
    perm: Tensor
    key: Tensor
    other: Tensor
    num_rows: int

    @property
    def num_edges(self) -> int:
        return int(self.key.shape[0])


def csr_build(edge_index: Tensor, sort_row: int, num_rows: int) -> SortedEdges:
    lib = _lib.load()
    if edge_index.dtype not in (torch.int32, torch.int64):
        raise GaotError(f"edge_index must be int32 or int64, got {edge_index.dtype}")
    ei = _req(edge_index, edge_index.dtype, "edge_index")
    if ei.dim() != 2 or ei.shape[0] != 2:
        raise GaotError(f"edge_index must be [2,E], got {tuple(ei.shape)}")
    e = int(ei.shape[1])
    dev = ei.device
    rowptr = torch.empty(num_rows + 1, dtype=torch.int32, device=dev)
    perm = torch.empty(e, dtype=torch.int32, device=dev)
    key = torch.empty(e, dtype=torch.int32, device=dev)
    other = torch.empty(e, dtype=torch.int32, device=dev)
    nb = lib.gaot_csr_workspace_bytes(e, num_rows)
    ws = _ws(nb, dev)
    check(lib.gaot_csr_build(_ptr(ei), int(ei.dtype == torch.int64), e, sort_row, num_rows, _ptr(rowptr), _ptr(perm),
                             _ptr(key), _ptr(other), _ptr(ws), ws.numel(), _stream()), "gaot_csr_build")
    return SortedEdges(rowptr, perm, key, other, num_rows)


@dataclass
class BipartiteGraph:
    by_dst: SortedEdges
    by_src: SortedEdges
    num_src: int
    num_dst: int


def build_graph(edge_index: Tensor, num_src: int, num_dst: int) -> BipartiteGraph:
    return BipartiteGraph(csr_build(edge_index, 1, num_dst), csr_build(edge_index, 0, num_src), num_src, num_dst)


def _mlp_struct(weights: Sequence[Tensor], biases: Sequence[Tensor]) -> Tuple[MlpT, List[Tensor]]:
    n = len(weights)
    if n < 2 or n > _lib.MAX_MLP_LAYERS:
        raise GaotError(f"kernel MLP must have 2..{_lib.MAX_MLP_LAYERS} linear layers, got {n}")
    keep = []
    m = MlpT()
    m.n_hidden = n - 1
    m.hidden = int(weights[0].shape[0])
    m.channels = int(weights[-1].shape[0])
    for l, (w, b) in enumerate(zip(weights, biases)):
        if w.dim() == 3:
            w = w[:, :, 0]
        w = _req(w, torch.float32, f"mlp.weight[{l}]")
        b = _req(b, torch.float32, f"mlp.bias[{l}]")
        exp_in = 6 if l == 0 else m.hidden
        exp_out = m.channels if l == n - 1 else m.hidden
        if tuple(w.shape) != (exp_out, exp_in):
            raise GaotError(f"kernel MLP layer {l}: weight shape {tuple(w.shape)} unsupported by the fused HIP path "
                            f"(needs [{exp_out},{exp_in}]: coord_dim 3, equal hidden widths)")
        keep += [w, b]
        m.weight[l] = w.data_ptr()
        m.bias[l] = b.data_ptr()
    return m, keep


def gno_forward(weights, biases, y_pos: Tensor, x_pos: Tensor, f_y: Tensor, g: BipartiteGraph,
                precision: Optional[int] = None) -> Tensor:
    lib = _lib.load()
    prec = _PRECISION["mode"] if precision is None else precision
    m, keep = _mlp_struct(weights, biases)
    y_pos = _req(y_pos, torch.float32, "y_pos")
    x_pos = _req(x_pos, torch.float32, "x_pos")
    f_y = _req(f_y, torch.float32, "f_y")
    if f_y.shape[1] != m.channels:
        raise GaotError(f"f_y has {f_y.shape[1]} channels, kernel MLP outputs {m.channels}")
    q = g.num_dst
    e = g.by_dst.num_edges
    out = torch.empty(q, m.channels, dtype=torch.float32, device=x_pos.device)
    ws = _ws(lib.gaot_gno_fwd_workspace_bytes(e, m.channels), x_pos.device)
    with _timed(f"gno_fwd_nh{m.n_hidden}"):
        check(lib.gaot_gno_fwd(C.byref(m), _ptr(y_pos), _ptr(x_pos), _ptr(f_y), _ptr(g.by_dst.other), _ptr(g.by_dst.key),
                               _ptr(g.by_dst.rowptr), e, q, _ptr(out), prec, _ptr(ws), ws.numel(), _stream()), "gaot_gno_fwd")
    return out


def gno_backward(weights, biases, y_pos: Tensor, x_pos: Tensor, f_y: Tensor, grad_out: Tensor, g: BipartiteGraph,
                 precision: Optional[int] = None, coords: bool = False):
    lib = _lib.load()
    prec = _PRECISION["mode"] if precision is None else precision
    m, keep = _mlp_struct(weights, biases)
    y_pos = _req(y_pos, torch.float32, "y_pos")
# ... 397 lines not shown
    if qkv.dim() != 2 or tuple(qkv.shape) != (b * s, (h + 2 * hkv) * head_dim):
        raise GaotError(f"attn_hd_fwd: qkv must be [{b * s}, {(h + 2 * hkv) * head_dim}], got {tuple(qkv.shape)}")
    ld = qkv.shape[1]
    dev = qkv.device
    o = torch.empty(b * s, h * head_dim, dtype=torch.float32, device=dev)
    lse = torch.empty(b, h, s, dtype=torch.float32, device=dev)
    base = qkv.data_ptr()
    q, k, v = C.c_void_p(base), C.c_void_p(base + 4 * h * head_dim), C.c_void_p(base + 4 * (h + hkv) * head_dim)
    with _timed("attn_hd_fwd"):
        dp, sp = _drop_args(dropout_p, seed)
        check(lib.gaot_attn_hd_fwd(q, k, v, _ptr(o), _ptr(lse), ld, ld, ld, h * head_dim, b, s, h, hkv, head_dim, float(scale),
                                   dp, sp, int(head0), int(heads_total), _stream()), "gaot_attn_hd_fwd")
    return o, lse


def attn_hd_bwd(qkv: Tensor, o: Tensor, d_o: Tensor, lse: Tensor, b: int, s: int, h: int, hkv: int, head_dim: int,
                scale: float, dropout_p: float = 0.0, seed: Optional[Tensor] = None, head0: int = 0,
                heads_total: int = 0) -> Tensor:
    lib = _lib.load()
    dp, sp = _drop_args(dropout_p, seed)
    qkv = _req(qkv, torch.float32, "qkv")
    o = _req(o, torch.float32, "o")
    d_o = _req(d_o, torch.float32, "d_o")
    lse = _req(lse, torch.float32, "lse")
    if head_dim not in (64, 128):
        raise GaotError(f"attn_hd_bwd: head_dim {head_dim} unsupported (only 64 and 128)")
    if tuple(qkv.shape) != (b * s, (h + 2 * hkv) * head_dim) or tuple(o.shape) != (b * s, h * head_dim) or o.shape != d_o.shape \
            or lse.numel() != b * h * s:
        raise GaotError("attn_hd_bwd: qkv / o / d_o / lse do not match (b, s, h, hkv, head_dim)")
    ld = qkv.shape[1]
    dev = qkv.device
    dqkv = torch.empty_like(qkv)
    delta = torch.empty(b, h, s, dtype=torch.float32, device=dev)
    base, gbase = qkv.data_ptr(), dqkv.data_ptr()
    offk, offv = 4 * h * head_dim, 4 * (h + hkv) * head_dim
    for name, mask in (("attn_hd_bwd_delta", 1), ("attn_hd_bwd_dkv", 2), ("attn_hd_bwd_dq", 4)):
        with _timed(name):
            check(lib.gaot_attn_hd_bwd(C.c_void_p(base), C.c_void_p(base + offk), C.c_void_p(base + offv), _ptr(o),
                                       _ptr(d_o), _ptr(lse), _ptr(delta), C.c_void_p(gbase), C.c_void_p(gbase + offk),
                                       C.c_void_p(gbase + offv), ld, ld, ld, h * head_dim, h * head_dim, ld, ld, ld, b, s, h, hkv,
                                       head_dim, float(scale), dp, sp, int(head0), int(heads_total), mask, _stream()),
                  "gaot_attn_hd_bwd")
    return dqkv


def attn_fwd_bf16(qkv: Optional[Tensor], freqs: Optional[Tensor], b: int, s: int, h: int, hkv: int, scale: float,
                  dropout_p: float = 0.0, seed: Optional[Tensor] = None, image: Optional[Tensor] = None, head0: int = 0,
                  heads_total: int = 0):
    lib = _lib.load()
    dev = image.device if image is not None else qkv.device
    o = torch.empty(b * s, h * 32, dtype=torch.float32, device=dev)
    lse = torch.empty(b, h, s, dtype=torch.float32, device=dev)
    img = image if image is not None else _ws(lib.gaot_attn_bf16_image_bytes(b, s, h, hkv), dev)
    with _timed("attn_fwd"):
        dp, sp = _drop_args(dropout_p, seed)
        check(lib.gaot_attn_fwd_bf16(_ptr(None if image is not None else qkv), _ptr(freqs), _ptr(img), _ptr(o), _ptr(lse), b, s,
                                     h, hkv, 32, float(scale), dp, sp, int(head0), int(heads_total), _stream()), "gaot_attn_fwd_bf16")
    return o, lse, img


_ROPE_TABLES: dict = {}


def rope_table(freqs: Tensor, s: int) -> Tensor:
    key = (id(freqs), int(s))
    ent = _ROPE_TABLES.get(key)
    if ent is not None and ent[0] is freqs and ent[1] == freqs._version:
        _ROPE_TABLES[key] = _ROPE_TABLES.pop(key)
        return ent[2]
    if freqs.numel() != 16 or freqs.dtype != torch.float32:
        raise GaotError("rope_table: 16 fp32 frequencies (head_dim 32) expected")
    t = torch.empty(s, 16, 2, dtype=torch.float32, device=freqs.device)
    check(_lib.load().gaot_rope_table(_ptr(freqs), int(s), 16, _ptr(t), _stream()), "gaot_rope_table")
    _ROPE_TABLES.pop(key, None)
    _ROPE_TABLES[key] = (freqs, freqs._version, t)
    while len(_ROPE_TABLES) > 64:
        _ROPE_TABLES.pop(next(iter(_ROPE_TABLES)))
    return t


def qkv_image(xb: Tensor, wcat: Tensor, rows: int, b: int, s: int, h: int, hkv: int, freqs: Optional[Tensor],
              scale: float) -> Tensor:
    lib = _lib.load()
    if xb.dtype != torch.bfloat16 or wcat.dtype != torch.bfloat16 or not (xb.is_contiguous() and wcat.is_contiguous()):
        raise GaotError("qkv_image: contiguous bf16 operands expected")
    img = _ws(lib.gaot_attn_bf16_image_bytes(b, s, h, hkv), xb.device)
    table = rope_table(freqs, s) if freqs is not None else None
    with _timed("qkv_image"):
        check(lib.gaot_qkv_image(_ptr(xb), _ptr(wcat), _ptr(img), rows, xb.shape[1], wcat.shape[1], s, h, hkv, _ptr(table),
                                 _qscale(scale), _stream()), "gaot_qkv_image")
    return img


def attn_bwd_scratch(b: int, s: int, h: int, hkv: int, device) -> Tensor:
    return _ws(_lib.load().gaot_attn_bwd_bf16_scratch_bytes(b, s, h, hkv), device)


def attn_bwd_bf16(img: Tensor, o: Tensor, d_o: Optional[Tensor], lse: Tensor, b: int, s: int, h: int, hkv: int, scale: float,
                  dropout_p: float = 0.0, seed: Optional[Tensor] = None, freqs: Optional[Tensor] = None,
                  do_image: Optional[Tensor] = None, fused: Optional[bool] = None, head0: int = 0, heads_total: int = 0,
                  delta: Optional[Tensor] = None) -> Tensor:
    lib = _lib.load()
    dp, sp = _drop_args(dropout_p, seed)
    dev = o.device
    dqkv = torch.empty(b * s, (h + 2 * hkv) * 32, dtype=torch.float32, device=dev)
    have_delta = delta is not None
    if have_delta and (do_image is None or tuple(delta.shape) != (b, h, s) or delta.dtype != torch.float32):
        raise GaotError("attn_bwd_bf16: delta needs do_image and the shape [b, h, s]")
    if not have_delta:
        delta = torch.empty(b, h, s, dtype=torch.float32, device=dev)
    doimg = do_image if do_image is not None else attn_bwd_scratch(b, s, h, hkv, dev)
# ... 226 lines not shown
    _fields_ = [("w", C.c_void_p), ("packed", C.c_void_p)]


def qkv_pack_multi(ws, with_backward: bool) -> List[Tensor]:
    lib = _lib.load()
    ws = list(ws)
    if not ws:
        return []
    n = ws[0].shape[0]
    nb = int(lib.gaot_qkv_packed_bytes(n, int(with_backward)))
    buf = torch.empty(len(ws) * nb, dtype=torch.uint8, device=ws[0].device)
    outs = [buf[i * nb:(i + 1) * nb] for i in range(len(ws))]
    items = (_QkvPackItem * len(ws))()
    for i, (w, o) in enumerate(zip(ws, outs)):
        if w.dtype != torch.float32 or not w.is_contiguous() or tuple(w.shape) != (n, 256):
            raise GaotError("qkv_pack_multi: contiguous fp32 [N, 256] weights of one N expected")
        items[i] = _QkvPackItem(w.data_ptr(), o.data_ptr())
    check(lib.gaot_qkv_pack_multi(items, len(ws), n, int(with_backward), _stream()), "gaot_qkv_pack_multi")
    return outs


def skip_pack_multi(ws) -> List[Tensor]:
    lib = _lib.load()
    ws = list(ws)
    if not ws:
        return []
    nb = int(lib.gaot_skip_packed_bytes())
    buf = torch.empty(len(ws) * nb, dtype=torch.uint8, device=ws[0].device)
    outs = [buf[i * nb:(i + 1) * nb] for i in range(len(ws))]
    items = (_QkvPackItem * len(ws))()
    for i, (w, o) in enumerate(zip(ws, outs)):
        if w.dtype != torch.float32 or not w.is_contiguous() or tuple(w.shape) != (256, 512):
            raise GaotError("skip_pack_multi: contiguous fp32 [256, 512] weights expected")
        items[i] = _QkvPackItem(w.data_ptr(), o.data_ptr())
    check(lib.gaot_skip_pack_multi(items, len(ws), _stream()), "gaot_skip_pack_multi")
    return outs


def cat_norm_qkv_image(xa: Tensor, xb: Tensor, skip_packed: Tensor, skip_bias: Optional[Tensor], norm_weight: Tensor, eps: float, packed: Tensor,
                       b: int, s: int, h: int, hkv: int, freqs: Optional[Tensor], scale: float):
    lib = _lib.load()
    rows = xa.shape[0]
    for t in (xa, xb):
        if t.dtype != torch.float32 or t.dim() != 2 or tuple(t.shape) != (rows, 256) or t.stride(1) != 1 or rows != b * s:
            raise GaotError("cat_norm_qkv_image: fp32 [b * s, 256] inputs expected")
    nw = _req(norm_weight, torch.float32, "norm_weight")
    bs = None if skip_bias is None else _req(skip_bias, torch.float32, "skip_bias")
    img = _ws(lib.gaot_attn_bf16_image_bytes(b, s, h, hkv), xa.device)
    xo = torch.empty(rows, 256, dtype=torch.float32, device=xa.device)
    yb = torch.empty(rows, 256, dtype=torch.bfloat16, device=xa.device)
    rstd = torch.empty(rows, dtype=torch.float32, device=xa.device)
    table = rope_table(freqs, s) if freqs is not None else None
    with _timed("cat_norm_qkv_image"):
        check(lib.gaot_cat_norm_qkv_image(_ptr(xa), xa.stride(0), _ptr(xb), xb.stride(0), _ptr(skip_packed), _ptr(bs), _ptr(xo), _ptr(nw), float(eps),
                                          _ptr(packed), _ptr(img), _ptr(yb), _ptr(rstd), rows, s, h, hkv, _ptr(table), _qscale(scale), _stream()),
              "gaot_cat_norm_qkv_image")
    return img, xo, yb, rstd


def norm_qkv_image(x: Tensor, norm_weight: Tensor, eps: float, packed: Tensor, b: int, s: int, h: int, hkv: int, freqs: Optional[Tensor],
                   scale: float):
    lib = _lib.load()
    rows = x.shape[0]
    if x.dtype != torch.float32 or x.dim() != 2 or x.shape[1] != 256 or x.stride(1) != 1 or rows != b * s:
        raise GaotError("norm_qkv_image: fp32 [b * s, 256] input expected")
    nw = _req(norm_weight, torch.float32, "norm_weight")
    img = _ws(lib.gaot_attn_bf16_image_bytes(b, s, h, hkv), x.device)
    yb = torch.empty(rows, 256, dtype=torch.bfloat16, device=x.device)
    rstd = torch.empty(rows, dtype=torch.float32, device=x.device)
    table = rope_table(freqs, s) if freqs is not None else None
    with _timed("norm_qkv_image"):
        check(lib.gaot_norm_qkv_image(_ptr(x), x.stride(0), _ptr(nw), float(eps), _ptr(packed), _ptr(img), _ptr(yb), _ptr(rstd), rows, s, h, hkv,
                                      _ptr(table), _qscale(scale), _stream()), "gaot_norm_qkv_image")
    return img, yb, rstd


def _finish_parts(part: Tensor, n: int, parts: int, lanes: int, defer: bool) -> Tensor:
    out = torch.empty(n, dtype=torch.float32, device=part.device)
    if defer:
        _defer(part, out, n, parts, lanes)
        return out
    arr = (_ReduceDesc * 1)()
    arr[0].part, arr[0].out, arr[0].n, arr[0].parts, arr[0].lanes = part.data_ptr(), out.data_ptr(), n, parts, lanes
    check(_lib.load().gaot_reduce_multi(arr, 1, _stream()), "gaot_reduce_multi")
    return out


def ffn_bwd_norm(yb: Tensor, dy: Tensor, packed: Tensor, f: int, h: Tensor, norm_weight: Tensor, rstd: Tensor, defer: bool = False):
    lib = _lib.load()
    rows = yb.shape[0]
    if yb.dtype != torch.bfloat16 or not yb.is_contiguous() or yb.shape[1] != 256:
        raise GaotError("ffn_bwd_norm: contiguous bf16 [rows, 256] input expected")
    if dy.dtype != torch.float32 or not dy.is_contiguous() or tuple(dy.shape) != (rows, 256):
        raise GaotError("ffn_bwd_norm: contiguous fp32 [rows, 256] gradient expected")
    if h.dtype != torch.float32 or tuple(h.shape) != (rows, 256) or h.stride(1) != 1:
        raise GaotError("ffn_bwd_norm: fp32 [rows, 256] norm input expected")
    nw = _req(norm_weight, torch.float32, "norm_weight")
    dev = yb.device
    dag = torch.empty(rows, 2 * f, dtype=torch.bfloat16, device=dev)
    u = torch.empty(rows, f, dtype=torch.bfloat16, device=dev)
    dyb = torch.empty(rows, 256, dtype=torch.bfloat16, device=dev)
    dh = torch.empty(rows, 256, dtype=torch.float32, device=dev)
    parts = int(lib.gaot_norm_bwd_parts(rows))
    part = torch.empty(parts, 256, dtype=torch.float32, device=dev)
    with _timed("ffn_bwd_norm"):
        check(lib.gaot_ffn_bwd_norm(_ptr(yb), _ptr(dy), _ptr(packed), _ptr(h), h.stride(0), _ptr(nw), _ptr(rstd), _ptr(dag), _ptr(u), _ptr(dyb),
                                    _ptr(dh), _ptr(part), rows, int(f), _stream()), "gaot_ffn_bwd_norm")
    return dh, dag, u, dyb, _finish_parts(part, 256, parts, 32, defer)


def qkv_bwd_norm(dqkv: Tensor, packed: Tensor, x: Tensor, norm_weight: Tensor, rstd: Tensor, dres: Optional[Tensor] = None,
                 dtap: Optional[Tensor] = None, defer: bool = False):
    lib = _lib.load()
    rows, n = dqkv.shape
    if dqkv.dtype != torch.float32 or not dqkv.is_contiguous() or n % 256:
        raise GaotError("qkv_bwd_norm: contiguous fp32 [rows, N] gradient with N a multiple of 256 expected")
    if x.dtype != torch.float32 or tuple(x.shape) != (rows, 256) or x.stride(1) != 1:
        raise GaotError("qkv_bwd_norm: fp32 [rows, 256] norm input expected")
    nw = _req(norm_weight, torch.float32, "norm_weight")
    dres = None if dres is None else _req(dres, torch.float32, "dres")
    dtap = None if dtap is None else _req(dtap, torch.float32, "dtap")
    dev = dqkv.device
    dx = torch.empty(rows, 256, dtype=torch.float32, device=dev)
    parts = int(lib.gaot_norm_bwd_parts(rows))
    part = torch.empty(parts, 256, dtype=torch.float32, device=dev)
    with _timed("qkv_bwd_norm"):
# ... 248 lines not shown
```

include/gaot3d_hip.h:

```cpp
#ifndef GAOT3D_HIP_H
#define GAOT3D_HIP_H

#include <stddef.h>
#include <stdint.h>

#ifdef __cplusplus
extern "C" {
#endif

#define GAOT_OK 0
#define GAOT_ERR_ARG 1
#define GAOT_ERR_LAUNCH 2
#define GAOT_ERR_UNSUPPORTED 3

#define GAOT_ABI_VERSION 11
#define GAOT_MAX_MLP_LAYERS 5

typedef void* gaot_stream_t;

int gaot_abi_version(void);
const char* gaot_last_error(void);
int64_t gaot_launch_count(int reset);

size_t gaot_csr_workspace_bytes(int64_t num_edges, int64_t num_rows);
int gaot_csr_build(const void* edge_index, int index_is_i64, int64_t num_edges, int sort_row, int64_t num_rows,
                   int32_t* rowptr, int32_t* perm, int32_t* key_sorted, int32_t* other_sorted, void* workspace,
                   size_t workspace_bytes, gaot_stream_t stream);

typedef struct {
    int n_hidden;
    int hidden;
    int channels;
    const float* weight[GAOT_MAX_MLP_LAYERS];
    const float* bias[GAOT_MAX_MLP_LAYERS];
} gaot_mlp_t;

typedef struct {
    float* weight[GAOT_MAX_MLP_LAYERS];
    float* bias[GAOT_MAX_MLP_LAYERS];
} gaot_mlp_grad_t;

size_t gaot_gno_fwd_workspace_bytes(int64_t num_edges, int channels);
int gaot_gno_fwd(const gaot_mlp_t* mlp , const float* y_pos, const float* x_pos, const float* f_y,
                 const int32_t* src_sorted, const int32_t* dst_sorted, const int32_t* rowptr_dst, int64_t num_edges,
                 int64_t num_queries, float* out ,
                 int precision ,
                 void* workspace, size_t workspace_bytes, gaot_stream_t stream);

size_t gaot_gno_bwd_workspace_bytes(const gaot_mlp_t* mlp , int64_t num_edges, int64_t num_queries);
int gaot_gno_bwd(const gaot_mlp_t* mlp , const float* y_pos, const float* x_pos, const float* f_y,
                 const float* grad_out , const int32_t* rowptr_dst,
                 const int32_t* src_sorted , const int32_t* dst_sorted ,
                 const int32_t* rowptr_src, int64_t num_edges, int64_t num_sources, int64_t num_queries,
                 float* grad_f_y , const gaot_mlp_grad_t* grads ,
                 int precision, void* workspace, size_t workspace_bytes, gaot_stream_t stream);
int gaot_gno_bwd_coords(const gaot_mlp_t* mlp , const float* y_pos, const float* x_pos, const float* f_y,
                        const float* grad_out, const int32_t* rowptr_dst, const int32_t* src_sorted, const int32_t* dst_sorted,
                        const int32_t* rowptr_src, int64_t num_edges, int64_t num_sources, int64_t num_queries,
                        float* grad_f_y, const gaot_mlp_grad_t* grads , float* grad_edge_coords ,
                        int precision, void* workspace, size_t workspace_bytes, gaot_stream_t stream);

size_t gaot_geoembed_stats_workspace_bytes(void);
int gaot_geoembed_moments(const float* source_pos, const float* query_pos, const int32_t* rowptr_dst,
                          const int32_t* src_sorted, int64_t num_queries, double* moments, gaot_stream_t stream);
int gaot_geoembed_from_moments(const double* moments, int64_t num_queries, float* features, void* workspace,
                               size_t workspace_bytes, gaot_stream_t stream);
int gaot_geoembed_raw(const float* source_pos, const float* query_pos, const int32_t* rowptr_dst, const int32_t* src_sorted,
                      int64_t num_queries, float* features, double* colsums, void* workspace, size_t workspace_bytes,
                      gaot_stream_t stream);
int gaot_geoembed_finalize(float* features, int64_t num_queries, const double* colsums, int64_t num_queries_total,
                           void* workspace, size_t workspace_bytes, gaot_stream_t stream);
size_t gaot_geoembed_from_moments_bwd_workspace_bytes(int64_t num_queries);
int gaot_geoembed_from_moments_bwd(const double* moments, const float* grad_features, int64_t num_queries,
                                   double* grad_moments, void* workspace, size_t workspace_bytes, gaot_stream_t stream);
int gaot_geoembed_moments_bwd(const float* source_pos, const float* query_pos, const int32_t* rowptr_dst,
                              const int32_t* src_sorted, int64_t num_queries, const double* grad_moments,
                              float* grad_edge , float* grad_query , gaot_stream_t stream);

size_t gaot_gemm_workspace_bytes(int64_t M, int64_t N, int64_t K);
int gaot_gemm(const float* A, const float* B, float* C, int64_t M, int64_t N, int64_t K, int64_t lda, int64_t ldb,
              int64_t ldc, int a_trans, int b_trans, const float* bias, int act, const float* residual, int64_t ldr,
              float* preact, int precision, void* workspace, size_t workspace_bytes, gaot_stream_t stream);
int gaot_gemm_ex(const void* A, const void* B, void* C, int64_t M, int64_t N, int64_t K, int64_t lda, int64_t ldb,
                 int64_t ldc, int a_trans, int b_trans, int a_bf16, int b_bf16, int c_bf16, const float* bias, int act,
                 const float* residual, int64_t ldr, float* preact, int precision, void* workspace,
                 size_t workspace_bytes, gaot_stream_t stream);

int gaot_attn_fwd(const float* q, const float* k, const float* v, float* o, float* lse, int64_t ldq, int64_t ldk,
                  int64_t ldv, int64_t ldo, int B, int S, int H, int HKV, int head_dim, float scale, float dropout_p,
                  const unsigned long long* dropout_seed, int head0, int heads_total, int precision, gaot_stream_t stream);
int gaot_attn_bwd(const float* q, const float* k, const float* v, const float* o, const float* d_o, const float* lse,
                  float* delta, float* dq, float* dk, float* dv, int64_t ldq, int64_t ldk, int64_t ldv, int64_t ldo,
                  int64_t lddo, int64_t lddq, int64_t lddk, int64_t lddv, int B, int S, int H, int HKV, int head_dim,
                  float scale, float dropout_p, const unsigned long long* dropout_seed, int head0, int heads_total,
                  int precision, int phase_mask , gaot_stream_t stream);
int64_t gaot_attn_bwd_fused_f32_scratch_bytes(int B, int S, int H);
int gaot_attn_bwd_fused_f32(const float* q, const float* k, const float* v, const float* o, const float* d_o, const float* lse,
                            float* delta, float* dq, float* dk, float* dv, int64_t ldq, int64_t ldk, int64_t ldv, int64_t ldo,
                            int64_t lddo, int64_t lddq, int64_t lddk, int64_t lddv, int B, int S, int H, int HKV, int head_dim,
                            float scale, float dropout_p, const unsigned long long* dropout_seed, int head0, int heads_total,
                            int run_delta, void* scratch, size_t scratch_bytes, gaot_stream_t stream);
int gaot_attn_hd_fwd(const float* q, const float* k, const float* v, float* o, float* lse, int64_t ldq, int64_t ldk,
                     int64_t ldv, int64_t ldo, int B, int S, int H, int HKV, int head_dim, float scale, float dropout_p,
                     const unsigned long long* dropout_seed, int head0, int heads_total, gaot_stream_t stream);
int gaot_attn_hd_bwd(const float* q, const float* k, const float* v, const float* o, const float* d_o, const float* lse,
                     float* delta, float* dq, float* dk, float* dv, int64_t ldq, int64_t ldk, int64_t ldv, int64_t ldo,
                     int64_t lddo, int64_t lddq, int64_t lddk, int64_t lddv, int B, int S, int H, int HKV, int head_dim,
                     float scale, float dropout_p, const unsigned long long* dropout_seed, int head0, int heads_total,
                     int phase_mask , gaot_stream_t stream);
int gaot_attn_dropout_mask(const unsigned long long* dropout_seed, float dropout_p, int B, int H, int S,
                           unsigned char* keep, gaot_stream_t stream);
int gaot_dropout_seed_next(unsigned long long* state, unsigned long long stride, unsigned long long* out,
                           gaot_stream_t stream);
int gaot_dropout_seed_block(unsigned long long* state, unsigned long long stride, int n, unsigned long long* out, gaot_stream_t stream);

int gaot_rope_table(const float* freqs, int S, int half_dim, float* table, gaot_stream_t stream);
int gaot_qkv_image(const void* x_bf16, const void* w_bf16, void* image, int64_t rows, int64_t lda, int64_t ldw, int S, int H,
                   int HKV, const float* rope_table, float qscale, gaot_stream_t stream);
int gaot_qkv_image_packed(const void* x_bf16, const void* w_bf16, void* packed, int64_t rows, int64_t lda, int64_t ldw,
                          int64_t pos0, int H, int HKV, const float* rope_table, float qscale, int world, gaot_stream_t stream);
int gaot_pack_heads(void* rows_buf, void* blocks_buf, int64_t rows, int ld, int world, int nseg, const int* col0,
                    const int* width, int rows_dtype, int blocks_dtype, int to_blocks, gaot_stream_t stream);
size_t gaot_attn_bf16_image_bytes(int B, int S, int H, int HKV);
size_t gaot_attn_bwd_bf16_scratch_bytes(int B, int S, int H, int HKV);
int gaot_attn_bwd_bf16_fused_eligible(int B, int S, int H, int HKV);
int gaot_attn_fwd_bf16(const float* qkv, const float* rope_freqs, void* qkv_image, float* o, float* lse, int B, int S,
                       int H, int HKV, int head_dim, float scale, float dropout_p,
                       const unsigned long long* dropout_seed, int head0, int heads_total, gaot_stream_t stream);
int gaot_attn_bwd_bf16(const void* qkv_image, const float* o, const float* d_o, const float* lse, void* do_image,
                       float* delta, float* dqkv, const float* rope_freqs, int B, int S, int H, int HKV, int head_dim,
                       float scale, float dropout_p, const unsigned long long* dropout_seed, int head0, int heads_total,
                       int phase_mask, gaot_stream_t stream);

int gaot_rmsnorm_fwd(const float* x, const float* weight, float* y, float* rstd, void* y_bf16 , int64_t rows, int dim, float eps,
                     gaot_stream_t stream);
size_t gaot_rmsnorm_bwd_workspace_bytes(int64_t rows, int dim);
int gaot_rmsnorm_bwd(const float* x, const float* weight, const float* dy, const float* rstd, const float* dx_add,
                     float* dx, float* dweight, int64_t rows, int dim, void* workspace, size_t workspace_bytes,
                     gaot_stream_t stream);
int gaot_rmsnorm_bwd2(const float* x, const float* weight, const float* dy, const float* rstd, const float* dx_add,
                      const float* dx_add2, float* dx, float* dweight, int64_t rows, int dim, void* workspace, size_t workspace_bytes,
                      gaot_stream_t stream);
size_t gaot_colsum_workspace_bytes(int64_t M, int64_t N);
int gaot_colsum(const float* x, int64_t M, int64_t N, int64_t ld, float* out, void* workspace, size_t workspace_bytes,
                gaot_stream_t stream);
typedef struct {
    const float* part;
    float* out;
    int64_t n;
    int32_t parts;
    int32_t lanes;
} gaot_reduce_desc_t;
int gaot_gemm_ex_partials(const void* A, const void* B, void* C, int64_t M, int64_t N, int64_t K, int64_t lda, int64_t ldb,
                          int64_t ldc, int a_trans, int b_trans, int a_bf16, int b_bf16, int precision, void* workspace,
                          size_t workspace_bytes, int* splits_out, int* lanes_out, gaot_stream_t stream);
int64_t gaot_rmsnorm_bwd_parts(int64_t rows);
int64_t gaot_colsum_parts(int64_t M);
int gaot_reduce_multi(const gaot_reduce_desc_t* descs, int count, gaot_stream_t stream);
int gaot_rope(float* x, int64_t rows, int64_t ld, int col0, int nheads, int head_dim, int seq_len, const float* freqs,
              int inverse, gaot_stream_t stream);
int gaot_swiglu_fwd(const float* ag, float* u, int64_t rows, int F, gaot_stream_t stream);
int gaot_swiglu_bwd(const float* ag, const float* du, float* dag, int64_t rows, int F, gaot_stream_t stream);
int gaot_cast_bf16(const float* src, void* dst, int64_t n, gaot_stream_t stream);
typedef struct {
    const float* src;
    void* dst;
    int64_t numel;
} gaot_cast_tensor_t;
int gaot_cast_bf16_multi(const gaot_cast_tensor_t* tensors, int num_tensors, gaot_stream_t stream);
int gaot_cast_bf16_transpose_multi(const gaot_cast_tensor_t* tensors, const int* rows, const int* cols, int num_tensors,
                                   gaot_stream_t stream);
int gaot_swiglu_fwd_bf16(const void* ag, void* u, int64_t rows, int F, gaot_stream_t stream);
int gaot_ffn_w13_swiglu(const void* x_bf16, const void* w13_bf16, void* ag, void* u, int64_t rows, int64_t lda, int64_t ldw, int F,
                        gaot_stream_t stream);
int gaot_swiglu_bwd_bf16(const void* ag, const void* du, void* dag, int64_t rows, int F, gaot_stream_t stream);
int gaot_ffn_w2_bwd_swiglu(const void* dy_bf16, const void* w2t_bf16, const void* ag, void* dag, int64_t rows, int64_t lda,
                           int64_t ldw, int F, gaot_stream_t stream);
int64_t gaot_ffn_packed_bytes(int F, int with_backward);
int gaot_ffn_pack(const float* w13, const float* w2, int F, void* packed, int with_backward, gaot_stream_t stream);
typedef struct {
    const float* w13;
    const float* w2;
    void* packed;
} gaot_ffn_pack_t;
int gaot_ffn_pack_multi(const gaot_ffn_pack_t* items, int num, int F, int with_backward, gaot_stream_t stream);
int gaot_ffn_fwd(const void* x_bf16, const void* packed, const float* residual, int64_t ldr, float* y, void* ag, void* u, int64_t rows,
                 int F, gaot_stream_t stream);
int gaot_norm_ffn_fwd(const float* h, int64_t ldh, const float* norm_weight, float eps, const void* packed, float* y, void* yb,
                      float* rstd, int64_t rows, int F, gaot_stream_t stream);
typedef struct {
    const float* w13;
    const float* w2;
    const float* wo;
    void* packed;
} gaot_block_pack_t;
int64_t gaot_block_packed_bytes(int F);
int gaot_block_pack_multi(const gaot_block_pack_t* items, int num, int F, gaot_stream_t stream);
int gaot_block_tail_fwd(const float* attn_out, int64_t ldo, const float* x, int64_t ldx, const float* norm_weight, float eps,
                        const void* packed, float* h, float* y, void* yb, float* rstd, int64_t rows, int F, gaot_stream_t stream);
typedef struct {
    const float* w;
    void* packed;
} gaot_qkv_pack_t;
int64_t gaot_qkv_packed_bytes(int64_t N, int with_backward);
int gaot_qkv_pack_multi(const gaot_qkv_pack_t* items, int num, int64_t N, int with_backward, gaot_stream_t stream);
int gaot_norm_qkv_image(const float* x, int64_t ldx, const float* norm_weight, float eps, const void* packed, void* image, void* yb,
                        float* rstd, int64_t rows, int S, int H, int HKV, const float* rope_table, float qscale, gaot_stream_t stream);
int64_t gaot_skip_packed_bytes(void);
int gaot_skip_pack_multi(const gaot_qkv_pack_t* items, int num, gaot_stream_t stream);
int gaot_cat_norm_qkv_image(const float* xa, int64_t ldxa, const float* xb, int64_t ldxb, const void* skip_packed, const float* skip_bias,
                            float* x_out, const float* norm_weight, float eps, const void* packed, void* image, void* yb, float* rstd,
                            int64_t rows, int S, int H, int HKV, const float* rope_table, float qscale, gaot_stream_t stream);
int64_t gaot_norm_bwd_parts(int64_t rows);
int gaot_ffn_bwd_norm(const void* yb, const float* dy, const void* packed, const float* h, int64_t ldh, const float* norm_weight,
                      const float* rstd, void* dag, void* u, void* dyb, float* dh, float* dw_part, int64_t rows, int F, gaot_stream_t stream);
int gaot_qkv_bwd_norm(const float* dqkv, int64_t N, const void* packed, const float* x, int64_t ldx, const float* norm_weight,
                      const float* rstd, const float* dres, const float* dtap, float* dx, float* dw_part, int64_t rows, gaot_stream_t stream);
int gaot_qkv_bwd_norm_cat(const float* dqkv, int64_t N, const void* packed, const float* x, int64_t ldx, const float* norm_weight,
                          const float* rstd, const float* dres, const void* skip_packed, float* dx, float* dxa, float* dxb, int same,
                          float* dw_part, int64_t rows, gaot_stream_t stream);
int gaot_oproj_bwd_image(const float* dh, const float* attn_out, const void* packed, int F, void* do_image, float* delta, int64_t rows,
                         int S, gaot_stream_t stream);
int gaot_ffn_bwd_dag(const void* x_bf16, const float* dy, const void* packed, void* dag, void* u, void* dyb, int64_t rows, int F,
                     gaot_stream_t stream);
int gaot_ffn_bwd(const void* x_bf16, const float* dy, const void* packed, void* dag, void* u, void* dyb, float* dx, int add_dy,
                 int64_t rows, int F, gaot_stream_t stream);
int gaot_act_fwd(const float* z, float* h, int64_t n, int act, gaot_stream_t stream);
int gaot_act_bwd(const float* z, const float* dh, float* dz, int64_t n, int act, gaot_stream_t stream);
int gaot_axpy(const float* a, const float* b, float alpha, float* out, int64_t n, int64_t period, gaot_stream_t stream);
int gaot_stream_copy(const void* src, void* dst, int64_t bytes, gaot_stream_t stream);
int gaot_stream_copy_ex(const void* src, void* dst, int64_t bytes, int variant, gaot_stream_t stream);
int gaot_patchify(const float* src, float* dst, int B, int D, int H, int W, int P, int C, int to_tokens,
                  gaot_stream_t stream);
size_t gaot_mse_workspace_bytes(void);
int gaot_mse_fwd(const float* pred, const float* target, int64_t n, float* loss, void* workspace, size_t workspace_bytes,
                 gaot_stream_t stream);
int gaot_mse_bwd(const float* pred, const float* target, int64_t n, const float* grad_loss, float* dpred,
                 gaot_stream_t stream);

int gaot_scale_mix_fwd(const float* const* xs, int num_scales, const float* logits, float* out, float* weights,
                       int64_t n, int channels, gaot_stream_t stream);
int gaot_scale_mix_bwd(const float* const* xs, int num_scales, const float* weights, const float* dout,
                       float* const* dxs, float* dlogits, int64_t n, int channels, gaot_stream_t stream);

typedef struct {
    float* param;
    const float* grad;
    float* exp_avg;
    float* exp_avg_sq;
    int64_t numel;
} gaot_adamw_tensor_t;
int gaot_adamw_step(const gaot_adamw_tensor_t* tensors, int num_tensors, const float* lr, float* step, double beta1,
                    double beta2, double eps, double weight_decay, gaot_stream_t stream);

typedef struct {
    int32_t dims[3];
    float lo[3];
    float hi[3];
} gaot_grid_t;
int gaot_knn_grid(const float* pos, int64_t num_points, const gaot_grid_t* grid, const float* token_pos, int k,
                  int32_t* out_idx, gaot_stream_t stream);
int gaot_radius_grid_count(const float* pos, int64_t num_points, const gaot_grid_t* grid, const float* token_pos,
                           float radius, int cap, int32_t* counts, gaot_stream_t stream);
int gaot_radius_grid_fill(const float* pos, int64_t num_points, const gaot_grid_t* grid, const float* token_pos,
                          float radius, int cap, const int32_t* offsets, int32_t* out_point, int32_t* out_token,
// ... 51 lines not shown
```

Before: 25.19 million points/s.

## Build both CSR orderings in one pass and fuse key-norm max into QKV image

Adds a paired CSR builder that sorts the edge list by source and by destination in a single shared pipeline, replacing two separate csr_build calls. It also adds _kn variants of the norm+QKV image kernels that write per-64-row key-norm partial maxima while producing the image. The attention forward then skips its separate k_key_norm_max launch and reduces those partials inside the kernel. This saves launches and a re-read of the key image, at the cost of a longer reduction loop inside attention and more workspace for the partials.

```diff
diff --git a/gaot_3d_amd/_lib.py b/gaot_3d_amd/_lib.py
--- a/gaot_3d_amd/_lib.py
+++ b/gaot_3d_amd/_lib.py
@@ -32,6 +32,8 @@
     "gaot_launch_count": (_i64, [_i]),
     "gaot_csr_workspace_bytes": (_sz, [_i64, _i64]),
     "gaot_csr_build": (_i, [_p, _i, _i64, _i, _i64, _p, _p, _p, _p, _p, _sz, _p]),
+    "gaot_csr_pair_workspace_bytes": (_sz, [_i64, _i64, _i64]),
+    "gaot_csr_build_pair": (_i, [_p, _i, _i64, _i64, _i64, _p, _p, _p, _p, _p, _p, _p, _p, _p, _sz, _p]),
     "gaot_gno_fwd_workspace_bytes": (_sz, [_i64, _i]),
     "gaot_gno_fwd": (_i, [C.POINTER(MlpT), _p, _p, _p, _p, _p, _p, _i64, _i64, _p, _i, _p, _sz, _p]),
     "gaot_gno_bwd_workspace_bytes": (_sz, [C.POINTER(MlpT), _i64, _i64]),
@@ -68,6 +70,8 @@
     "gaot_attn_bwd_bf16_scratch_bytes": (_sz, [_i, _i, _i, _i]),
     "gaot_attn_bwd_bf16_fused_eligible": (_i, [_i, _i, _i, _i]),
     "gaot_attn_fwd_bf16": (_i, [_p, _p, _p, _p, _p, _i, _i, _i, _i, _i, _f, _f, _p, _i, _i, _p]),
+    "gaot_attn_bf16_key_norm_offset": (_sz, [_i, _i, _i, _i]),
+    "gaot_attn_fwd_bf16_kn": (_i, [_p, _p, _p, _i, _i, _i, _i, _i, _f, _f, _p, _i, _i, _i, _p]),
     "gaot_attn_bwd_bf16": (_i, [_p, _p, _p, _p, _p, _p, _p, _p, _i, _i, _i, _i, _i, _f, _f, _p, _i, _i, _i, _p]),
     "gaot_rmsnorm_fwd": (_i, [_p, _p, _p, _p, _p, _i64, _i, _f, _p]),
     "gaot_rmsnorm_bwd_workspace_bytes": (_sz, [_i64, _i]),
@@ -118,9 +122,11 @@
     "gaot_qkv_packed_bytes": (_i64, [_i64, _i]),
     "gaot_qkv_pack_multi": (_i, [_p, _i, _i64, _i, _p]),
     "gaot_norm_qkv_image": (_i, [_p, _i64, _p, _f, _p, _p, _p, _p, _i64, _i, _i, _i, _p, _f, _p]),
+    "gaot_norm_qkv_image_kn": (_i, [_p, _i64, _p, _f, _p, _p, _p, _p, _i64, _i, _i, _i, _p, _f, _p]),
     "gaot_skip_packed_bytes": (_i64, []),
     "gaot_skip_pack_multi": (_i, [_p, _i, _p]),
     "gaot_cat_norm_qkv_image": (_i, [_p, _i64, _p, _i64, _p, _p, _p, _p, _f, _p, _p, _p, _p, _i64, _i, _i, _i, _p, _f, _p]),
+    "gaot_cat_norm_qkv_image_kn": (_i, [_p, _i64, _p, _i64, _p, _p, _p, _p, _f, _p, _p, _p, _p, _i64, _i, _i, _i, _p, _f, _p]),
     "gaot_norm_bwd_parts": (_i64, [_i64]),
     "gaot_ffn_bwd_norm": (_i, [_p, _p, _p, _p, _i64, _p, _p, _p, _p, _p, _p, _p, _i64, _i, _p]),
     "gaot_qkv_bwd_norm": (_i, [_p, _i64, _p, _p, _i64, _p, _p, _p, _p, _p, _p, _i64, _p]),
diff --git a/gaot_3d_amd/csrc/attn_bf16.hip b/gaot_3d_amd/csrc/attn_bf16.hip
--- a/gaot_3d_amd/csrc/attn_bf16.hip
+++ b/gaot_3d_amd/csrc/attn_bf16.hip
@@ -143,6 +143,7 @@
     int chunk;
     int64_t o_part, lse_part;
     const float* kmax2;
+    int kn;
     int* redo;
 };
 
@@ -265,7 +266,8 @@
                 q2 = fmaf(v, v, q2);
             }
         q2 += xhalf(q2);
-        float k2 = a.kmax2[((int64_t)b * KN_BLOCKS + lane) * a.HKV + hkv];
+        float k2 = 0.f;
+        for (int i = lane; i < a.kn; i += 64) k2 = fmaxf(k2, a.kmax2[((int64_t)b * a.kn + i) * a.HKV + hkv]);
 #pragma unroll
         for (int o = 32; o > 0; o >>= 1) k2 = fmaxf(k2, __shfl_xor(k2, o, 64));
         const int over = __syncthreads_or(!(q2 * k2 <= BOUND2));
@@ -1664,7 +1666,8 @@
     });
     {
         constexpr float BOUND2 = 54.f * 54.f;
-        float k2 = a.kmax2[((int64_t)b * KN_BLOCKS + lane) * a.HKV + hkv];
+        float k2 = 0.f;
+        for (int i = lane; i < a.kn; i += 64) k2 = fmaxf(k2, a.kmax2[((int64_t)b * a.kn + i) * a.HKV + hkv]);
 #pragma unroll
         for (int o = 32; o > 0; o >>= 1) k2 = fmaxf(k2, __shfl_xor(k2, o, 64));
         const int over = __syncthreads_or(!(q2max * k2 <= BOUND2));
@@ -1856,10 +1859,11 @@
 }
 
 static size_t align256(size_t v) { return (v + 255) & ~(size_t)255; }
+static size_t key_norm_parts_max(int S) { return (size_t)std::max(KN_BLOCKS, S % 64 == 0 ? S / 64 : 0); }
 static size_t key_norm_off(int B, int S, int H, int HKV) { return (sizeof(bf16_t) * (size_t)B * S * (H + 2 * HKV) * D + 64 + 15) & ~(size_t)15; }
 static size_t fwd_flags(int B, int S, int H) { return (size_t)B * 8 * (size_t)ceil_div(S, 128) * H; }
 static size_t image_only_bytes(int B, int S, int H, int HKV) {
-    return align256(key_norm_off(B, S, H, HKV) + sizeof(float) * (size_t)B * KN_BLOCKS * HKV + sizeof(int) * fwd_flags(B, S, H));
+    return align256(key_norm_off(B, S, H, HKV) + sizeof(float) * (size_t)B * key_norm_parts_max(S) * HKV + sizeof(int) * fwd_flags(B, S, H));
 }
 
 extern "C" size_t gaot_attn_bf16_image_bytes(int B, int S, int H, int HKV) {
@@ -1889,12 +1893,31 @@
     return align256(sizeof(bf16_t) * (size_t)B * S * H * D + 64) + bwd_parts_bytes(B, S, H, HKV) + dqpart;
 }
 
+extern "C" size_t gaot_attn_bf16_key_norm_offset(int B, int S, int H, int HKV) { return key_norm_off(B, S, H, HKV); }
+
+static int attn_fwd_bf16_impl(const char* fn, const float* qkv, const float* rope_freqs, void* qkv_image, float* o, float* lse,
+                              int B, int S, int H, int HKV, int head_dim, float scale, float dropout_p,
+                              const unsigned long long* dropout_seed, int head0, int heads_total, int key_norm_parts,
+                              gaot_stream_t stream);
 extern "C" int gaot_attn_fwd_bf16(const float* qkv, const float* rope_freqs, void* qkv_image, float* o, float* lse,
                                   int B, int S, int H, int HKV, int head_dim, float scale, float dropout_p,
                                   const unsigned long long* dropout_seed, int head0, int heads_total, gaot_stream_t stream) {
+    return attn_fwd_bf16_impl("gaot_attn_fwd_bf16", qkv, rope_freqs, qkv_image, o, lse, B, S, H, HKV, head_dim, scale, dropout_p,
+                              dropout_seed, head0, heads_total, 0, stream);
+}
+extern "C" int gaot_attn_fwd_bf16_kn(void* qkv_image, float* o, float* lse, int B, int S, int H, int HKV, int head_dim,
+                                     float scale, float dropout_p, const unsigned long long* dropout_seed, int head0,
+                                     int heads_total, int key_norm_parts, gaot_stream_t stream) {
+    return attn_fwd_bf16_impl("gaot_attn_fwd_bf16_kn", nullptr, nullptr, qkv_image, o, lse, B, S, H, HKV, head_dim, scale, dropout_p,
+                              dropout_seed, head0, heads_total, key_norm_parts, stream);
+}
+static int attn_fwd_bf16_impl(const char* fn, const float* qkv, const float* rope_freqs, void* qkv_image, float* o, float* lse,
+                              int B, int S, int H, int HKV, int head_dim, float scale, float dropout_p,
+                              const unsigned long long* dropout_seed, int head0, int heads_total, int key_norm_parts,
+                              gaot_stream_t stream) {
     GAOT_ENTER();
     if (head_dim != D) {
-        gaot_set_error("gaot_attn_fwd_bf16: head_dim %d unsupported (only 32)", head_dim);
+        gaot_set_error("%s: head_dim %d unsupported (only 32)", fn, head_dim);
         return GAOT_ERR_UNSUPPORTED;
     }
     GAOT_CHECK_ARG(B > 0 && S > 0 && H > 0 && HKV > 0 && H % HKV == 0, "bad shape");
@@ -1902,6 +1925,8 @@
     GAOT_CHECK_ARG((((uintptr_t)qkv | (uintptr_t)qkv_image | (uintptr_t)o) & 15) == 0, "buffers must be 16-byte aligned");
     GAOT_CHECK_ARG(dropout_p >= 0.f && dropout_p < 1.f && (dropout_p == 0.f || dropout_seed), "dropout_p in [0,1) and a seed");
     GAOT_CHECK_ARG(heads_total == 0 || (head0 >= 0 && head0 + H <= heads_total), "head0 + H <= heads_total");
+    GAOT_CHECK_ARG(key_norm_parts == 0 || (!qkv && S % 64 == 0 && key_norm_parts == S / 64),
+                   "key_norm_parts: 0, or S / 64 for an image whose key-norm area is filled (S a multiple of 64)");
     hipStream_t st = (hipStream_t)stream;
     const int ld = (H + 2 * HKV) * D;
     const int64_t rows = (int64_t)B * S;
@@ -1910,15 +1935,17 @@
         GAOT_KLAUNCH(k_prep_qkv, dim3((unsigned)ceil_div(n, 256)), dim3(256), 0, st, qkv, (bf16_t*)qkv_image, rows, ld, H,
                      HKV, S, rope_freqs, scale * LOG2E);
     float* kmax2 = reinterpret_cast<float*>(reinterpret_cast<char*>(qkv_image) + key_norm_off(B, S, H, HKV));
-    int* redo = reinterpret_cast<int*>(kmax2 + (size_t)B * KN_BLOCKS * HKV);
-    GAOT_KLAUNCH(k_key_norm_max, dim3(KN_BLOCKS, (unsigned)B, (unsigned)HKV), dim3(256), 0, st, (const bf16_t*)qkv_image,
-                 (int64_t)ld, S, H, HKV, kmax2);
+    int* redo = reinterpret_cast<int*>(kmax2 + (size_t)B * key_norm_parts_max(S) * HKV);
+    if (key_norm_parts == 0)
+        GAOT_KLAUNCH(k_key_norm_max, dim3(KN_BLOCKS, (unsigned)B, (unsigned)HKV), dim3(256), 0, st, (const bf16_t*)qkv_image,
+                     (int64_t)ld, S, H, HKV, kmax2);
     const int P = split_parts(ceil_div(S, 128) * H * B, S);
     float* o_parts = reinterpret_cast<float*>(reinterpret_cast<char*>(qkv_image) + image_only_bytes(B, S, H, HKV));
     const int64_t o_part = rows * H * D, lse_part = (int64_t)B * H * S;
     float* lse_parts = o_parts + (size_t)P * o_part;
     FwdArgs a{(const bf16_t*)qkv_image, P > 1 ? o_parts : o, P > 1 ? lse_parts : lse, ld, B, S, H, HKV,
-              gdrop::make_drop(dropout_seed, dropout_p, H, head0, heads_total), P > 1 ? split_chunk(S, P) : S, o_part, lse_part, kmax2, redo};
+              gdrop::make_drop(dropout_seed, dropout_p, H, head0, heads_total), P > 1 ? split_chunk(S, P) : S, o_part, lse_part, kmax2,
+              key_norm_parts ? key_norm_parts : KN_BLOCKS, redo};
     const dim3 fgrid((unsigned)(ceil_div(S, 128) * H), (unsigned)(P > 1 ? ceil_div(S, a.chunk) : 1), (unsigned)B);
     static const int fwd_lab = [] { const char* e = getenv("GAOT_ATTN_FWD_LAB"); return e ? atoi(e) : 0; }();
     const bool dot2 = fwd_lab == 8 || (fwd_lab != 1 && a.drop.thr);
diff --git a/gaot_3d_amd/csrc/csr.hip b/gaot_3d_amd/csrc/csr.hip
--- a/gaot_3d_amd/csrc/csr.hip
+++ b/gaot_3d_amd/csrc/csr.hip
@@ -1,3 +1,5 @@
+#include <stdlib.h>
+
 #include "csr_impl.h"
 
 extern "C" size_t gaot_csr_workspace_bytes(int64_t num_edges, int64_t num_rows) {
@@ -27,3 +29,32 @@
     GAOT_LAUNCH_CHECK();
     return GAOT_OK;
 }
+
+extern "C" size_t gaot_csr_pair_workspace_bytes(int64_t num_edges, int64_t num_rows0, int64_t num_rows1) {
+    (void)num_rows0;
+    (void)num_rows1;
+    return sizeof(int) * (size_t)pair_layout(num_edges).total + 64;
+}
+
+extern "C" int gaot_csr_build_pair(const void* edge_index, int index_is_i64, int64_t num_edges, int64_t num_rows0,
+                                   int64_t num_rows1, int32_t* rowptr0, int32_t* perm0, int32_t* key_sorted0,
+                                   int32_t* other_sorted0, int32_t* rowptr1, int32_t* perm1, int32_t* key_sorted1,
+                                   int32_t* other_sorted1, void* workspace, size_t workspace_bytes, gaot_stream_t stream) {
+    GAOT_ENTER();
+    GAOT_CHECK_ARG(num_edges >= 0 && num_rows0 >= 0 && num_rows1 >= 0, "negative size");
+    GAOT_CHECK_ARG(num_edges < (int64_t)1 << 31 && num_rows0 < ((int64_t)1 << 31) - 1 && num_rows1 < ((int64_t)1 << 31) - 1,
+                   "sizes must fit int32");
+    GAOT_CHECK_ARG(rowptr0 && rowptr1 && workspace, "null pointer");
+    GAOT_CHECK_ARG(num_edges == 0 || (edge_index && perm0 && key_sorted0 && other_sorted0 && perm1 && key_sorted1 &&
+                                      other_sorted1), "null pointer");
+    GAOT_CHECK_ARG(((uintptr_t)workspace & 15) == 0, "workspace must be 16-byte aligned");
+    GAOT_CHECK_ARG(workspace_bytes >= gaot_csr_pair_workspace_bytes(num_edges, num_rows0, num_rows1), "workspace too small");
+    hipStream_t st = (hipStream_t)stream;
+    const int64_t Q[2] = {num_rows0, num_rows1};
+    int32_t* const out[2][4] = {{rowptr0, perm0, key_sorted0, other_sorted0}, {rowptr1, perm1, key_sorted1, other_sorted1}};
+    int rc = index_is_i64 ? csr_build_pair_t<int64_t>((const int64_t*)edge_index, num_edges, Q, out, workspace, st)
+                          : csr_build_pair_t<int32_t>((const int32_t*)edge_index, num_edges, Q, out, workspace, st);
+    if (rc != GAOT_OK) return rc;
+    GAOT_LAUNCH_CHECK();
+    return GAOT_OK;
+}
diff --git a/gaot_3d_amd/csrc/csr_impl.h b/gaot_3d_amd/csrc/csr_impl.h
--- a/gaot_3d_amd/csrc/csr_impl.h
+++ b/gaot_3d_amd/csrc/csr_impl.h
@@ -8,19 +8,22 @@
 }
 
 template <typename IDX>
-__global__ void k_check_sorted(const IDX* __restrict__ keys, int64_t E, int* __restrict__ unsorted) {
+__device__ __forceinline__ void check_sorted_body(const IDX* __restrict__ keys, int64_t E, int* __restrict__ unsorted) {
     int64_t i = (int64_t)blockIdx.x * blockDim.x + threadIdx.x;
     const int64_t stride = (int64_t)gridDim.x * blockDim.x;
     bool bad = false;
     for (; i < E; i += stride) bad |= (i > 0) && (keys[i] < keys[i - 1]);
     if (__any(bad) && (threadIdx.x & 63) == 0) *unsorted = 1;
 }
-
-template <typename IDX>
-__global__ void k_sorted_build(const IDX* __restrict__ keys, const IDX* __restrict__ other, int64_t E, int64_t Q,
-                               const int* __restrict__ unsorted, int* __restrict__ rowptr, int* __restrict__ perm,
-                               int* __restrict__ key_sorted, int* __restrict__ other_sorted) {
-    if (*unsorted) return;
+template <typename IDX>
+__global__ void k_check_sorted(const IDX* __restrict__ keys, int64_t E, int* __restrict__ unsorted) {
+    check_sorted_body<IDX>(keys, E, unsorted);
+}
+
+template <typename IDX>
+__device__ __forceinline__ void sorted_build_body(const IDX* __restrict__ keys, const IDX* __restrict__ other, int64_t E,
+                                                  int64_t Q, int* __restrict__ rowptr, int* __restrict__ perm,
+                                                  int* __restrict__ key_sorted, int* __restrict__ other_sorted) {
     int64_t i = (int64_t)blockIdx.x * blockDim.x + threadIdx.x;
     const int64_t stride = (int64_t)gridDim.x * blockDim.x;
     for (; i < E; i += stride) {
@@ -34,12 +37,19 @@
             for (int64_t r = (int64_t)k + 1; r <= Q; ++r) rowptr[r] = (int)E;
     }
 }
+template <typename IDX>
+__global__ void k_sorted_build(const IDX* __restrict__ keys, const IDX* __restrict__ other, int64_t E, int64_t Q,
+                               const int* __restrict__ unsorted, int* __restrict__ rowptr, int* __restrict__ perm,
+                               int* __restrict__ key_sorted, int* __restrict__ other_sorted) {
+    if (*unsorted) return;
+    sorted_build_body<IDX>(keys, other, E, Q, rowptr, perm, key_sorted, other_sorted);
+}
 
 constexpr int SCAN_BLOCK = 256;
 constexpr int SCAN_ITEMS = 8;
 constexpr int SCAN_TILE = SCAN_BLOCK * SCAN_ITEMS;
 
-__global__ void k_scan_reduce(const int* __restrict__ in, int64_t n, int* __restrict__ block_sums) {
+__device__ __forceinline__ void scan_reduce_body(const int* __restrict__ in, int64_t n, int* __restrict__ block_sums) {
     __shared__ int red[SCAN_BLOCK / 64];
     const int64_t base = (int64_t)blockIdx.x * SCAN_TILE;
     int s = 0;
@@ -58,8 +68,11 @@
         block_sums[blockIdx.x] = t;
     }
 }
-
-__global__ void k_scan_blocksums(int* __restrict__ block_sums, int nb) {
+__global__ void k_scan_reduce(const int* __restrict__ in, int64_t n, int* __restrict__ block_sums) {
+    scan_reduce_body(in, n, block_sums);
+}
+
+__device__ __forceinline__ void scan_blocksums_body(int* __restrict__ block_sums, int nb) {
     __shared__ int carry;
     __shared__ int wsum[SCAN_BLOCK / 64];
     if (threadIdx.x == 0) carry = 0;
@@ -85,9 +98,10 @@
         __syncthreads();
     }
 }
-
-__global__ void k_scan_apply(const int* __restrict__ in, int64_t n, const int* __restrict__ block_offs,
-                             int* __restrict__ out) {
+__global__ void k_scan_blocksums(int* __restrict__ block_sums, int nb) { scan_blocksums_body(block_sums, nb); }
+
+__device__ __forceinline__ void scan_apply_body(const int* __restrict__ in, int64_t n, const int* __restrict__ block_offs,
+                                                int* __restrict__ out) {
     __shared__ int wsum[SCAN_BLOCK / 64];
     const int64_t base = (int64_t)blockIdx.x * SCAN_TILE + (int64_t)threadIdx.x * SCAN_ITEMS;
     int v[SCAN_ITEMS];
@@ -118,15 +132,18 @@
         if (base + j == n - 1) out[n] = run;
     }
 }
+__global__ void k_scan_apply(const int* __restrict__ in, int64_t n, const int* __restrict__ block_offs,
+                             int* __restrict__ out) {
+    scan_apply_body(in, n, block_offs, out);
+}
 
 constexpr int RS_TILE = 4096;
 constexpr int RS_ROUNDS = RS_TILE / 256;
 
 template <typename KIN>
-__global__ __launch_bounds__(256) void k_rs_hist(const KIN* __restrict__ keys, int64_t E, int shift, int nd, int nblk,
-                                                 int* __restrict__ table, const int* __restrict__ unsorted) {
+__device__ __forceinline__ void rs_hist_body(const KIN* __restrict__ keys, int64_t E, int shift, int nd, int nblk,
+                                             int* __restrict__ table) {
     __shared__ int h[256];
-    if (!*unsorted) return;
     h[threadIdx.x] = 0;
     __syncthreads();
     const int64_t base = (int64_t)blockIdx.x * RS_TILE;
@@ -138,14 +155,18 @@
     __syncthreads();
     if ((int)threadIdx.x < nd) table[(int64_t)threadIdx.x * nblk + blockIdx.x] = h[threadIdx.x];
 }
-
 template <typename KIN>
-__global__ __launch_bounds__(256) void k_rs_scatter(const KIN* __restrict__ keys_in, const int* __restrict__ ids_in,
-                                                    int64_t E, int shift, int nbits, int nblk,
-                                                    const int* __restrict__ table, int* __restrict__ keys_out,
-                                                    int* __restrict__ ids_out, const int* __restrict__ unsorted) {
+__global__ __launch_bounds__(256) void k_rs_hist(const KIN* __restrict__ keys, int64_t E, int shift, int nd, int nblk,
+                                                 int* __restrict__ table, const int* __restrict__ unsorted) {
+    if (!*unsorted) return;
+    rs_hist_body<KIN>(keys, E, shift, nd, nblk, table);
+}
+
+template <typename KIN>
+__device__ __forceinline__ void rs_scatter_body(const KIN* __restrict__ keys_in, const int* __restrict__ ids_in, int64_t E,
+                                                int shift, int nbits, int nblk, const int* __restrict__ table,
+                                                int* __restrict__ keys_out, int* __restrict__ ids_out) {
     __shared__ int wcnt[4][256];
-    if (!*unsorted) return;
     const int wave = threadIdx.x >> 6, lane = threadIdx.x & 63;
     const int nd = 1 << nbits;
     const int64_t base = (int64_t)blockIdx.x * RS_TILE + (int64_t)wave * (RS_ROUNDS * 64);
@@ -192,12 +213,20 @@
         }
     }
 }
-
-template <typename IDX>
-__global__ void k_emit_sorted(const int* __restrict__ keys, const int* __restrict__ ids, const IDX* __restrict__ other,
-                              int64_t E, int64_t Q, const int* __restrict__ unsorted, int* __restrict__ rowptr,
-                              int* __restrict__ perm, int* __restrict__ key_sorted, int* __restrict__ other_sorted) {
+template <typename KIN>
+__global__ __launch_bounds__(256) void k_rs_scatter(const KIN* __restrict__ keys_in, const int* __restrict__ ids_in,
+                                                    int64_t E, int shift, int nbits, int nblk,
+                                                    const int* __restrict__ table, int* __restrict__ keys_out,
+                                                    int* __restrict__ ids_out, const int* __restrict__ unsorted) {
     if (!*unsorted) return;
+    rs_scatter_body<KIN>(keys_in, ids_in, E, shift, nbits, nblk, table, keys_out, ids_out);
+}
+
+template <typename IDX>
+__device__ __forceinline__ void emit_sorted_body(const int* __restrict__ keys, const int* __restrict__ ids,
+                                                 const IDX* __restrict__ other, int64_t E, int64_t Q, int* __restrict__ rowptr,
+                                                 int* __restrict__ perm, int* __restrict__ key_sorted,
+                                                 int* __restrict__ other_sorted) {
     int64_t i = (int64_t)blockIdx.x * blockDim.x + threadIdx.x;
     const int64_t stride = (int64_t)gridDim.x * blockDim.x;
     for (; i < E; i += stride) {
@@ -210,6 +239,13 @@
         if (i == E - 1)
             for (int64_t r = (int64_t)k + 1; r <= Q; ++r) rowptr[r] = (int)E;
     }
+}
+template <typename IDX>
+__global__ void k_emit_sorted(const int* __restrict__ keys, const int* __restrict__ ids, const IDX* __restrict__ other,
+                              int64_t E, int64_t Q, const int* __restrict__ unsorted, int* __restrict__ rowptr,
+                              int* __restrict__ perm, int* __restrict__ key_sorted, int* __restrict__ other_sorted) {
+    if (!*unsorted) return;
+    emit_sorted_body<IDX>(keys, ids, other, E, Q, rowptr, perm, key_sorted, other_sorted);
 }
 
 static int rs_bits(int64_t Q) {
@@ -275,4 +311,220 @@
     return GAOT_OK;
 }
 
-}
+struct PairRow {
+    const void* keys;
+    const void* other;
+    int64_t Q;
+    int passes, width;
+    int* rowptr;
+    int* perm;
+    int* key_sorted;
+    int* other_sorted;
+    int* kbuf[2];
+    int* ibuf[2];
+    int* table;
+    int* tscan;
+    int* bsum;
+};
+struct PairArgs {
+    PairRow r[2];
+    int* flags;
+};
+
+template <typename IDX>
+__global__ void k_check_sorted_pair(PairArgs a, int64_t E) {
+    check_sorted_body<IDX>((const IDX*)a.r[blockIdx.y].keys, E, a.flags + 1 + blockIdx.y);
+}
+
+template <typename IDX>
+__global__ void k_sorted_build_pair(PairArgs a, int64_t E) {
+    if (a.flags[1 + blockIdx.y]) return;
+    const PairRow& r = a.r[blockIdx.y];
+    sorted_build_body<IDX>((const IDX*)r.keys, (const IDX*)r.other, E, r.Q, r.rowptr, r.perm, r.key_sorted, r.other_sorted);
+}
+
+template <typename KIN>
+__global__ __launch_bounds__(256) void k_rs_hist_pair(PairArgs a, int64_t E, int p, int nblk) {
+    const PairRow& r = a.r[blockIdx.y];
+    if (p >= r.passes || !a.flags[1 + blockIdx.y]) return;
+    const KIN* keys = (p == 0) ? (const KIN*)r.keys : (const KIN*)r.kbuf[(p - 1) & 1];
+    rs_hist_body<KIN>(keys, E, p * r.width, 1 << r.width, nblk, r.table);
+}
+
+template <typename KIN>
+__global__ __launch_bounds__(256) void k_rs_scatter_pair(PairArgs a, int64_t E, int p, int nblk) {
+    const PairRow& r = a.r[blockIdx.y];
+    if (p >= r.passes || !a.flags[1 + blockIdx.y]) return;
+    const KIN* keys = (p == 0) ? (const KIN*)r.keys : (const KIN*)r.kbuf[(p - 1) & 1];
+    const int* ids = (p == 0) ? nullptr : r.ibuf[(p - 1) & 1];
+    rs_scatter_body<KIN>(keys, ids, E, p * r.width, r.width, nblk, r.tscan, r.kbuf[p & 1], r.ibuf[p & 1]);
+}
+
+template <typename IDX>
+__global__ void k_emit_sorted_pair(PairArgs a, int64_t E) {
+    if (!a.flags[1 + blockIdx.y]) return;
+    const PairRow& r = a.r[blockIdx.y];
+    const int last = (r.passes - 1) & 1;
+    emit_sorted_body<IDX>(r.kbuf[last], r.ibuf[last], (const IDX*)r.other, E, r.Q, r.rowptr, r.perm, r.key_sorted,
+                          r.other_sorted);
+}
+
+__global__ void k_scan_reduce_pair(PairArgs a, int p, int nblk) {
+    const PairRow& r = a.r[blockIdx.y];
+    if (p >= r.passes || !a.flags[1 + blockIdx.y]) return;
+    const int64_t n = ((int64_t)1 << r.width) * nblk;
+    if ((int64_t)blockIdx.x * SCAN_TILE >= n) return;
+    scan_reduce_body(r.table, n, r.bsum);
+}
+__global__ void k_scan_blocksums_pair(PairArgs a, int p, int nblk) {
+    const PairRow& r = a.r[blockIdx.y];
+    if (p >= r.passes || !a.flags[1 + blockIdx.y]) return;
+    scan_blocksums_body(r.bsum, (int)((((int64_t)1 << r.width) * nblk + SCAN_TILE - 1) / SCAN_TILE));
+}
+__global__ void k_scan_apply_pair(PairArgs a, int p, int nblk) {
+    const PairRow& r = a.r[blockIdx.y];
+    if (p >= r.passes || !a.flags[1 + blockIdx.y]) return;
+    const int64_t n = ((int64_t)1 << r.width) * nblk;
+    if ((int64_t)blockIdx.x * SCAN_TILE >= n) return;
+    scan_apply_body(r.table, n, r.bsum, r.tscan);
+}
+
+constexpr int SCAN1_THREADS = 1024;
+constexpr int SCAN1_WAVES = SCAN1_THREADS / 64;
+__device__ __forceinline__ int4 scan1_load(const int* __restrict__ in, int i, int n) {
+    if (i + 4 <= n) return *reinterpret_cast<const int4*>(in + i);
+    int4 v = make_int4(0, 0, 0, 0);
+    if (i < n) v.x = in[i];
+    if (i + 1 < n) v.y = in[i + 1];
+    if (i + 2 < n) v.z = in[i + 2];
+    return v;
+}
+__global__ __launch_bounds__(SCAN1_THREADS) void k_scan_single_pair(PairArgs a, int p, int nblk) {
+    __shared__ int wtot[SCAN1_WAVES];
+    const PairRow& r = a.r[blockIdx.y];
+    if (p >= r.passes || !a.flags[1 + blockIdx.y]) return;
+    const int* __restrict__ in = r.table;
+    int* __restrict__ out = r.tscan;
+    const int n = (1 << r.width) * nblk;
+    const int wave = threadIdx.x >> 6, lane = threadIdx.x & 63;
+    const int steps = ((n + SCAN1_WAVES - 1) / SCAN1_WAVES + 255) / 256;
+    const int lo = wave * steps * 256 + lane * 4;
+    int s = 0;
+#pragma unroll 4
+    for (int t = 0; t < steps; ++t) {
+        const int4 v = scan1_load(in, lo + t * 256, n);
+        s += v.x + v.y + v.z + v.w;
+    }
+#pragma unroll
+    for (int o = 32; o > 0; o >>= 1) s += __shfl_xor(s, o, 64);
+    if (lane == 0) wtot[wave] = s;
+    __syncthreads();
+    int carry = 0;
+    for (int w = 0; w < wave; ++w) carry += wtot[w];
+    int4 nxt = scan1_load(in, lo, n);
+    for (int t = 0; t < steps; ++t) {
+        const int4 v = nxt;
+        const int i = lo + t * 256;
+        if (t + 1 < steps) nxt = scan1_load(in, i + 256, n);
+        const int ls = v.x + v.y + v.z + v.w;
+        int incl = ls;
+#pragma unroll
+        for (int o = 1; o < 64; o <<= 1) {
+            const int u = __shfl_up(incl, o, 64);
+            if (lane >= o) incl += u;
+        }
+        const int e0 = carry + incl - ls;
+        const int4 w4 = make_int4(e0, e0 + v.x, e0 + v.x + v.y, e0 + v.x + v.y + v.z);
+        if (i + 4 <= n) *reinterpret_cast<int4*>(out + i) = w4;
+        else {
+            if (i < n) out[i] = w4.x;
+            if (i + 1 < n) out[i + 1] = w4.y;
+            if (i + 2 < n) out[i + 2] = w4.z;
+        }
+        carry += __shfl(incl, 63, 64);
+    }
+    if (threadIdx.x == 0) {
+        int t = 0;
+        for (int w = 0; w < SCAN1_WAVES; ++w) t += wtot[w];
+        out[n] = t;
+    }
+}
+constexpr int64_t SCAN1_MAX_N = (int64_t)1 << 15;
+
+struct PairLayout {
+    int64_t e4, tn4, nbt4, row, total;
+};
+static PairLayout pair_layout(int64_t E) {
+    PairLayout L;
+    const int64_t nblk = ceil_div(E, RS_TILE);
+    L.e4 = (E + 3) & ~(int64_t)3;
+    L.tn4 = 256 * nblk + 4;
+    L.nbt4 = (ceil_div(256 * nblk, SCAN_TILE) + 1 + 3) & ~(int64_t)3;
+    L.row = 4 * L.e4 + 2 * L.tn4 + L.nbt4;
+    L.total = 4 + 2 * L.row;
+    return L;
+}
+
+template <typename IDX>
+int csr_build_pair_t(const IDX* edge_index, int64_t E, const int64_t Q[2], int32_t* const out[2][4], void* ws,
+                     hipStream_t st) {
+    const PairLayout L = pair_layout(E);
+    const int nblk = (int)ceil_div(E, RS_TILE);
+    PairArgs a;
+    a.flags = (int*)ws;
+    int maxp = 0;
+    for (int y = 0; y < 2; ++y) {
+        PairRow& r = a.r[y];
+        int* base = a.flags + 4 + y * L.row;
+        r.keys = edge_index + (y ? E : 0);
+        r.other = edge_index + (y ? 0 : E);
+        r.Q = Q[y];
+        const int bits = rs_bits(Q[y]);
+        r.passes = (bits + 7) / 8;
+        r.width = (bits + r.passes - 1) / r.passes;
+        maxp = std::max(maxp, r.passes);
+        r.rowptr = out[y][0];
+        r.perm = out[y][1];
+        r.key_sorted = out[y][2];
+        r.other_sorted = out[y][3];
+        r.kbuf[0] = base;
+        r.kbuf[1] = base + L.e4;
+        r.ibuf[0] = base + 2 * L.e4;
+        r.ibuf[1] = base + 3 * L.e4;
+        r.table = base + 4 * L.e4;
+        r.tscan = r.table + L.tn4;
+        r.bsum = r.tscan + L.tn4;
+    }
+    GAOT_KLAUNCH(k_zero_flags, dim3(1), dim3(64), 0, st, a.flags, 4);
+    if (E == 0) {
+        for (int y = 0; y < 2; ++y) (void)hipMemsetAsync(out[y][0], 0, sizeof(int) * (size_t)(Q[y] + 1), st);
+        return GAOT_OK;
+    }
+    int64_t scan1_max = SCAN1_MAX_N;
+    if (const char* e = getenv("GAOT_CSR_SCAN1_MAX")) scan1_max = atoll(e);
+    const int tb = 256;
+    const int gb = (int)std::min<int64_t>(ceil_div(E, tb), 256 * 16);
+    GAOT_KLAUNCH((k_check_sorted_pair<IDX>), dim3(gb, 2), dim3(tb), 0, st, a, E);
+    GAOT_KLAUNCH((k_sorted_build_pair<IDX>), dim3(gb, 2), dim3(tb), 0, st, a, E);
+    for (int p = 0; p < maxp; ++p) {
+        int64_t n = 0;
+        for (int y = 0; y < 2; ++y)
+            if (p < a.r[y].passes) n = std::max(n, ((int64_t)1 << a.r[y].width) * nblk);
+        if (p == 0) GAOT_KLAUNCH((k_rs_hist_pair<IDX>), dim3(nblk, 2), dim3(256), 0, st, a, E, p, nblk);
+        else GAOT_KLAUNCH((k_rs_hist_pair<int>), dim3(nblk, 2), dim3(256), 0, st, a, E, p, nblk);
+        if (n <= scan1_max) {
+            GAOT_KLAUNCH(k_scan_single_pair, dim3(1, 2), dim3(SCAN1_THREADS), 0, st, a, p, nblk);
+        } else {
+            const int nb = (int)ceil_div(n, SCAN_TILE);
+            GAOT_KLAUNCH(k_scan_reduce_pair, dim3(nb, 2), dim3(SCAN_BLOCK), 0, st, a, p, nblk);
+            GAOT_KLAUNCH(k_scan_blocksums_pair, dim3(1, 2), dim3(SCAN_BLOCK), 0, st, a, p, nblk);
+            GAOT_KLAUNCH(k_scan_apply_pair, dim3(nb, 2), dim3(SCAN_BLOCK), 0, st, a, p, nblk);
+        }
+        if (p == 0) GAOT_KLAUNCH((k_rs_scatter_pair<IDX>), dim3(nblk, 2), dim3(256), 0, st, a, E, p, nblk);
+        else GAOT_KLAUNCH((k_rs_scatter_pair<int>), dim3(nblk, 2), dim3(256), 0, st, a, E, p, nblk);
+    }
+    GAOT_KLAUNCH((k_emit_sorted_pair<IDX>), dim3(gb, 2), dim3(tb), 0, st, a, E);
+    return GAOT_OK;
+}
+
+}
diff --git a/gaot_3d_amd/csrc/ffn_fused.hip b/gaot_3d_amd/csrc/ffn_fused.hip
--- a/gaot_3d_amd/csrc/ffn_fused.hip
+++ b/gaot_3d_amd/csrc/ffn_fused.hip
@@ -1444,6 +1444,7 @@
     const float* X; int ldx; const float* NW; float eps; const u32x4* Wp; bf16_t* IMG; bf16_t* YB; float* RSTD;
     const float* table; int S, nq, nk; float qscale; int M, N;
     const float* XB; int ldxb; const u32x4* WSp; const float* BS; float* XO;
+    float* KN;
 };
 constexpr int QKV_LDS = H_BYTES + 256 + 64 * 144, QKV_LDS_CAT = 2 * H_BYTES + 256 + 1024 + 64 * 144;
 template <bool CAT>
@@ -1629,6 +1630,8 @@
     }
     __builtin_amdgcn_s_barrier();
     f32x16 accc[2][2], accn[2][2];
+    u32x4 ksave = {0u, 0u, 0u, 0u};
+    float kmx[2] = {0.f, 0.f};
     bf16x8 hn0 = *reinterpret_cast<const bf16x8*>(hb + ((hf ^ sw) << 4)), hn1 = *reinterpret_cast<const bf16x8*>(hb + 32 * 512 + ((hf ^ sw) << 4));
     auto panel_step = [&](f32x16 (&acc)[2][2], int pn, int st, auto epi) {
         const int g = 4 * pn + st;
@@ -1698,6 +1701,22 @@
             const auto r1 = __builtin_amdgcn_permlane32_swap(pk[0][1], pk[1][1], false, false);
             const u32x4 v = {(unsigned)r0[0], (unsigned)r1[0], (unsigned)r0[1], (unsigned)r1[1]};
             __builtin_amdgcn_raw_buffer_store_b128(v, irs, rowoff + (head * 32 + 8 * q0 + 16 * hf) * 2, 0, 0);
+            if (a.KN && head >= a.nq && head < a.nq + a.nk) {
+                if (q0 == 0) ksave = v;
+                else {
+                    auto chain = [](float n2, const u32x4& w) {
+#pragma unroll
+                        for (int j = 0; j < 4; ++j) {
+                            const float lo = __uint_as_float(w[j] << 16), hi = __uint_as_float(w[j] & 0xffff0000u);
+                            n2 = fmaf(lo, lo, fmaf(hi, hi, n2));
+                        }
+                        return n2;
+                    };
+                    const float low = chain(chain(0.f, ksave), v);
+                    const float full = chain(chain(__shfl_xor(low, 32, 64), ksave), v);
+                    kmx[jt] = fmaxf(kmx[jt], (hf && m < M) ? full : 0.f);
+                }
+            }
         };
         zero4(accn);
 #pragma unroll
@@ -1708,6 +1727,20 @@
         for (int jt = 0; jt < 2; ++jt)
 #pragma unroll
             for (int i = 0; i < 2; ++i) accc[jt][i] = accn[jt][i];
+        if (a.KN) {
+#pragma unroll
+            for (int jt = 0; jt < 2; ++jt) {
+                const int head = 8 * pn + 2 * wave + jt;
+                if (head >= a.nq && head < a.nq + a.nk) {
+                    float mx = kmx[jt];
+#pragma unroll
+                    for (int o = 32; o > 0; o >>= 1) mx = fmaxf(mx, __shfl_xor(mx, o, 64));
+                    const int bb = m0 / a.S;
+                    if (lane == 0) a.KN[((int64_t)bb * (a.S / 64) + (m0 - bb * a.S) / 64) * a.nk + (head - a.nq)] = mx;
+                }
+                kmx[jt] = 0.f;
+            }
+        }
     }
 }
 }
@@ -1731,8 +1764,27 @@
     return GAOT_OK;
 }
 
+static float* key_norm_area(void* image, int64_t rows, int S, int H, int HKV, int write_key_norms) {
+    if (!write_key_norms || !image || S <= 0 || S % 64 != 0 || rows % S != 0) return nullptr;
+    return reinterpret_cast<float*>(reinterpret_cast<char*>(image) + gaot_attn_bf16_key_norm_offset((int)(rows / S), S, H, HKV));
+}
+
+static int norm_qkv_image_impl(const float* x, int64_t ldx, const float* norm_weight, float eps, const void* packed, void* image, void* yb,
+                               float* rstd, int64_t rows, int S, int H, int HKV, const float* rope_table, float qscale, int write_key_norms,
+                               gaot_stream_t stream);
 extern "C" int gaot_norm_qkv_image(const float* x, int64_t ldx, const float* norm_weight, float eps, const void* packed, void* image, void* yb,
                                    float* rstd, int64_t rows, int S, int H, int HKV, const float* rope_table, float qscale, gaot_stream_t stream) {
+    return norm_qkv_image_impl(x, ldx, norm_weight, eps, packed, image, yb, rstd, rows, S, H, HKV, rope_table, qscale, 0, stream);
+}
+extern "C" int gaot_norm_qkv_image_kn(const float* x, int64_t ldx, const float* norm_weight, float eps, const void* packed, void* image, void* yb,
+                                      float* rstd, int64_t rows, int S, int H, int HKV, const float* rope_table, float qscale,
+                                      gaot_stream_t stream) {
+    GAOT_CHECK_ARG(S > 0 && S % 64 == 0 && rows % S == 0, "key norms need S a multiple of 64 and rows a multiple of S");
+    return norm_qkv_image_impl(x, ldx, norm_weight, eps, packed, image, yb, rstd, rows, S, H, HKV, rope_table, qscale, 1, stream);
+}
+static int norm_qkv_image_impl(const float* x, int64_t ldx, const float* norm_weight, float eps, const void* packed, void* image, void* yb,
+                               float* rstd, int64_t rows, int S, int H, int HKV, const float* rope_table, float qscale, int write_key_norms,
+                               gaot_stream_t stream) {
     GAOT_ENTER();
     const int64_t N = (int64_t)(H + 2 * HKV) * 32;
     GAOT_CHECK_ARG(x && norm_weight && packed && image && yb && rstd && rows > 0 && S > 0 && H > 0 && HKV > 0 && N % 256 == 0,
@@ -1753,7 +1805,7 @@
         attr_set = true;
     }
     const QkvArgs a{x, (int)ldx, norm_weight, eps, (const u32x4*)packed, (bf16_t*)image, (bf16_t*)yb, rstd, rope_table, S, H, HKV, qscale, (int)rows, (int)N,
-                    nullptr, 0, nullptr, nullptr, nullptr};
+                    nullptr, 0, nullptr, nullptr, nullptr, key_norm_area(image, rows, S, H, HKV, write_key_norms)};
     const int nblk = ((int)rows + RB - 1) / RB, per = (nblk + 7) / 8;
     GAOT_KLAUNCH(k_norm_qkv<false>, dim3((unsigned)(8 * per)), dim3(256), QKV_LDS, (hipStream_t)stream, a);
     GAOT_LAUNCH_CHECK();
@@ -1776,9 +1828,28 @@
     GAOT_LAUNCH_CHECK();
     return GAOT_OK;
 }
+static int cat_norm_qkv_image_impl(const float* xa, int64_t ldxa, const float* xb, int64_t ldxb, const void* skip_packed, const float* skip_bias,
+                                   float* x_out, const float* norm_weight, float eps, const void* packed, void* image, void* yb, float* rstd,
+                                   int64_t rows, int S, int H, int HKV, const float* rope_table, float qscale, int write_key_norms,
+                                   gaot_stream_t stream);
 extern "C" int gaot_cat_norm_qkv_image(const float* xa, int64_t ldxa, const float* xb, int64_t ldxb, const void* skip_packed, const float* skip_bias,
                                        float* x_out, const float* norm_weight, float eps, const void* packed, void* image, void* yb, float* rstd,
                                        int64_t rows, int S, int H, int HKV, const float* rope_table, float qscale, gaot_stream_t stream) {
+    return cat_norm_qkv_image_impl(xa, ldxa, xb, ldxb, skip_packed, skip_bias, x_out, norm_weight, eps, packed, image, yb, rstd, rows, S, H, HKV,
+                                   rope_table, qscale, 0, stream);
+}
+extern "C" int gaot_cat_norm_qkv_image_kn(const float* xa, int64_t ldxa, const float* xb, int64_t ldxb, const void* skip_packed,
+                                          const float* skip_bias, float* x_out, const float* norm_weight, float eps, const void* packed, void* image,
+                                          void* yb, float* rstd, int64_t rows, int S, int H, int HKV, const float* rope_table, float qscale,
+                                          gaot_stream_t stream) {
+    GAOT_CHECK_ARG(S > 0 && S % 64 == 0 && rows % S == 0, "key norms need S a multiple of 64 and rows a multiple of S");
+    return cat_norm_qkv_image_impl(xa, ldxa, xb, ldxb, skip_packed, skip_bias, x_out, norm_weight, eps, packed, image, yb, rstd, rows, S, H, HKV,
+                                   rope_table, qscale, 1, stream);
+}
+static int cat_norm_qkv_image_impl(const float* xa, int64_t ldxa, const float* xb, int64_t ldxb, const void* skip_packed, const float* skip_bias,
+                                   float* x_out, const float* norm_weight, float eps, const void* packed, void* image, void* yb, float* rstd,
+                                   int64_t rows, int S, int H, int HKV, const float* rope_table, float qscale, int write_key_norms,
+                                   gaot_stream_t stream) {
     GAOT_ENTER();
     const int64_t N = (int64_t)(H + 2 * HKV) * 32;
     GAOT_CHECK_ARG(xa && xb && skip_packed && x_out && norm_weight && packed && image && yb && rstd && rows > 0 && S > 0 && H > 0 && HKV > 0 &&
@@ -1800,7 +1871,7 @@
         attr_set = true;
     }
     const QkvArgs a{xa, (int)ldxa, norm_weight, eps, (const u32x4*)packed, (bf16_t*)image, (bf16_t*)yb, rstd, rope_table, S, H, HKV, qscale, (int)rows, (int)N,
-                    xb, (int)ldxb, (const u32x4*)skip_packed, skip_bias, x_out};
+                    xb, (int)ldxb, (const u32x4*)skip_packed, skip_bias, x_out, key_norm_area(image, rows, S, H, HKV, write_key_norms)};
     const int nblk = ((int)rows + RB - 1) / RB, per = (nblk + 7) / 8;
     GAOT_KLAUNCH(k_norm_qkv<true>, dim3((unsigned)(8 * per)), dim3(256), QKV_LDS_CAT, (hipStream_t)stream, a);
     GAOT_LAUNCH_CHECK();
diff --git a/gaot_3d_amd/csrc/gno.hip b/gaot_3d_amd/csrc/gno.hip
--- a/gaot_3d_amd/csrc/gno.hip
+++ b/gaot_3d_amd/csrc/gno.hip
@@ -766,7 +766,7 @@
         const int in_dim = (l == 0) ? IN0 : h;
         pt.w[l] = wt + off;
         pt.b[l] = p.b[l];
-        if (num_edges > 0)
+        if (num_edges > 0 && (precision != 1 || l == 0))
             GAOT_KLAUNCH(k_transpose_w, dim3((unsigned)ceil_div(out_dim * in_dim, 256)), dim3(256), 0, st, p.w[l],
                                out_dim, in_dim, wt + off);
         off += out_dim * in_dim;
diff --git a/gaot_3d_amd/ops.py b/gaot_3d_amd/ops.py
--- a/gaot_3d_amd/ops.py
+++ b/gaot_3d_amd/ops.py
@@ -114,8 +114,35 @@
     num_dst: int
 
 
+def csr_build_pair(edge_index: Tensor, num_rows0: int, num_rows1: int) -> Tuple[SortedEdges, SortedEdges]:
+    lib = _lib.load()
+    if edge_index.dtype not in (torch.int32, torch.int64):
+        raise GaotError(f"edge_index must be int32 or int64, got {edge_index.dtype}")
+    ei = _req(edge_index, edge_index.dtype, "edge_index")
+    if ei.dim() != 2 or ei.shape[0] != 2:
+        raise GaotError(f"edge_index must be [2,E], got {tuple(ei.shape)}")
+    e = int(ei.shape[1])
+    dev = ei.device
+    res = []
+    for nr in (num_rows0, num_rows1):
+        res.append(SortedEdges(torch.empty(nr + 1, dtype=torch.int32, device=dev),
+                               torch.empty(e, dtype=torch.int32, device=dev),
+                               torch.empty(e, dtype=torch.int32, device=dev),
+                               torch.empty(e, dtype=torch.int32, device=dev), nr))
+    ws = _ws(lib.gaot_csr_pair_workspace_bytes(e, num_rows0, num_rows1), dev)
+    s0, s1 = res
+    check(lib.gaot_csr_build_pair(_ptr(ei), int(ei.dtype == torch.int64), e, num_rows0, num_rows1,
+                                  _ptr(s0.rowptr), _ptr(s0.perm), _ptr(s0.key), _ptr(s0.other),
+                                  _ptr(s1.rowptr), _ptr(s1.perm), _ptr(s1.key), _ptr(s1.other),
+                                  _ptr(ws), ws.numel(), _stream()), "gaot_csr_build_pair")
+    return s0, s1
+
+
 def build_graph(edge_index: Tensor, num_src: int, num_dst: int) -> BipartiteGraph:
-    return BipartiteGraph(csr_build(edge_index, 1, num_dst), csr_build(edge_index, 0, num_src), num_src, num_dst)
+    if os.environ.get("GAOT_CSR_PAIR", "1") == "0":
+        return BipartiteGraph(csr_build(edge_index, 1, num_dst), csr_build(edge_index, 0, num_src), num_src, num_dst)
+    by_src, by_dst = csr_build_pair(edge_index, num_src, num_dst)
+    return BipartiteGraph(by_dst, by_src, num_src, num_dst)
 
 
 def _mlp_struct(weights: Sequence[Tensor], biases: Sequence[Tensor]) -> Tuple[MlpT, List[Tensor]]:
@@ -619,11 +646,22 @@
     o = torch.empty(b * s, h * 32, dtype=torch.float32, device=dev)
     lse = torch.empty(b, h, s, dtype=torch.float32, device=dev)
     img = image if image is not None else _ws(lib.gaot_attn_bf16_image_bytes(b, s, h, hkv), dev)
+    kn = int(getattr(image, "_gaot_key_norm_parts", 0)) if image is not None else 0
     with _timed("attn_fwd"):
         dp, sp = _drop_args(dropout_p, seed)
-        check(lib.gaot_attn_fwd_bf16(_ptr(None if image is not None else qkv), _ptr(freqs), _ptr(img), _ptr(o), _ptr(lse), b, s,
-                                     h, hkv, 32, float(scale), dp, sp, int(head0), int(heads_total), _stream()), "gaot_attn_fwd_bf16")
+        if kn and kn * 64 == s:
+            check(lib.gaot_attn_fwd_bf16_kn(_ptr(img), _ptr(o), _ptr(lse), b, s, h, hkv, 32, float(scale), dp, sp, int(head0),
+                                            int(heads_total), kn, _stream()), "gaot_attn_fwd_bf16_kn")
+        else:
+            check(lib.gaot_attn_fwd_bf16(_ptr(None if image is not None else qkv), _ptr(freqs), _ptr(img), _ptr(o), _ptr(lse), b, s,
+                                         h, hkv, 32, float(scale), dp, sp, int(head0), int(heads_total), _stream()), "gaot_attn_fwd_bf16")
     return o, lse, img
+
+
+def _key_norm_parts(s: int) -> int:
+    if os.environ.get("GAOT_QKV_KEYNORM", "1") == "0" or s % 64 != 0:
+        return 0
+    return s // 64
 
 
 _ROPE_TABLES: dict = {}
@@ -956,9 +994,12 @@
     rstd = torch.empty(rows, dtype=torch.float32, device=xa.device)
     table = rope_table(freqs, s) if freqs is not None else None
     with _timed("cat_norm_qkv_image"):
-        check(lib.gaot_cat_norm_qkv_image(_ptr(xa), xa.stride(0), _ptr(xb), xb.stride(0), _ptr(skip_packed), _ptr(bs), _ptr(xo), _ptr(nw), float(eps),
-                                          _ptr(packed), _ptr(img), _ptr(yb), _ptr(rstd), rows, s, h, hkv, _ptr(table), _qscale(scale), _stream()),
+        kn = _key_norm_parts(s)
+        fn = lib.gaot_cat_norm_qkv_image_kn if kn else lib.gaot_cat_norm_qkv_image
+        check(fn(_ptr(xa), xa.stride(0), _ptr(xb), xb.stride(0), _ptr(skip_packed), _ptr(bs), _ptr(xo), _ptr(nw), float(eps),
+                 _ptr(packed), _ptr(img), _ptr(yb), _ptr(rstd), rows, s, h, hkv, _ptr(table), _qscale(scale), _stream()),
               "gaot_cat_norm_qkv_image")
+    img._gaot_key_norm_parts = kn
     return img, xo, yb, rstd
 
 
@@ -974,8 +1015,11 @@
     rstd = torch.empty(rows, dtype=torch.float32, device=x.device)
     table = rope_table(freqs, s) if freqs is not None else None
     with _timed("norm_qkv_image"):
-        check(lib.gaot_norm_qkv_image(_ptr(x), x.stride(0), _ptr(nw), float(eps), _ptr(packed), _ptr(img), _ptr(yb), _ptr(rstd), rows, s, h, hkv,
-                                      _ptr(table), _qscale(scale), _stream()), "gaot_norm_qkv_image")
+        kn = _key_norm_parts(s)
+        fn = lib.gaot_norm_qkv_image_kn if kn else lib.gaot_norm_qkv_image
+        check(fn(_ptr(x), x.stride(0), _ptr(nw), float(eps), _ptr(packed), _ptr(img), _ptr(yb), _ptr(rstd), rows, s, h, hkv,
+                 _ptr(table), _qscale(scale), _stream()), "gaot_norm_qkv_image")
+    img._gaot_key_norm_parts = kn
     return img, yb, rstd
 
 
diff --git a/include/gaot3d_hip.h b/include/gaot3d_hip.h
--- a/include/gaot3d_hip.h
+++ b/include/gaot3d_hip.h
@@ -26,6 +26,11 @@
 int gaot_csr_build(const void* edge_index, int index_is_i64, int64_t num_edges, int sort_row, int64_t num_rows,
                    int32_t* rowptr, int32_t* perm, int32_t* key_sorted, int32_t* other_sorted, void* workspace,
                    size_t workspace_bytes, gaot_stream_t stream);
+size_t gaot_csr_pair_workspace_bytes(int64_t num_edges, int64_t num_rows0, int64_t num_rows1);
+int gaot_csr_build_pair(const void* edge_index, int index_is_i64, int64_t num_edges, int64_t num_rows0, int64_t num_rows1,
+                        int32_t* rowptr0, int32_t* perm0, int32_t* key_sorted0, int32_t* other_sorted0, int32_t* rowptr1,
+                        int32_t* perm1, int32_t* key_sorted1, int32_t* other_sorted1, void* workspace,
+                        size_t workspace_bytes, gaot_stream_t stream);
 
 typedef struct {
     int n_hidden;
@@ -127,6 +132,10 @@
 int gaot_attn_fwd_bf16(const float* qkv, const float* rope_freqs, void* qkv_image, float* o, float* lse, int B, int S,
                        int H, int HKV, int head_dim, float scale, float dropout_p,
                        const unsigned long long* dropout_seed, int head0, int heads_total, gaot_stream_t stream);
+size_t gaot_attn_bf16_key_norm_offset(int B, int S, int H, int HKV);
+int gaot_attn_fwd_bf16_kn(void* qkv_image, float* o, float* lse, int B, int S, int H, int HKV, int head_dim, float scale,
+                          float dropout_p, const unsigned long long* dropout_seed, int head0, int heads_total, int key_norm_parts,
+                          gaot_stream_t stream);
 int gaot_attn_bwd_bf16(const void* qkv_image, const float* o, const float* d_o, const float* lse, void* do_image,
                        float* delta, float* dqkv, const float* rope_freqs, int B, int S, int H, int HKV, int head_dim,
                        float scale, float dropout_p, const unsigned long long* dropout_seed, int head0, int heads_total,
@@ -211,6 +220,11 @@
 int gaot_cat_norm_qkv_image(const float* xa, int64_t ldxa, const float* xb, int64_t ldxb, const void* skip_packed, const float* skip_bias,
                             float* x_out, const float* norm_weight, float eps, const void* packed, void* image, void* yb, float* rstd,
                             int64_t rows, int S, int H, int HKV, const float* rope_table, float qscale, gaot_stream_t stream);
+int gaot_norm_qkv_image_kn(const float* x, int64_t ldx, const float* norm_weight, float eps, const void* packed, void* image, void* yb,
+                           float* rstd, int64_t rows, int S, int H, int HKV, const float* rope_table, float qscale, gaot_stream_t stream);
+int gaot_cat_norm_qkv_image_kn(const float* xa, int64_t ldxa, const float* xb, int64_t ldxb, const void* skip_packed, const float* skip_bias,
+                               float* x_out, const float* norm_weight, float eps, const void* packed, void* image, void* yb, float* rstd,
+                               int64_t rows, int S, int H, int HKV, const float* rope_table, float qscale, gaot_stream_t stream);
 int64_t gaot_norm_bwd_parts(int64_t rows);
 int gaot_ffn_bwd_norm(const void* yb, const float* dy, const void* packed, const float* h, int64_t ldh, const float* norm_weight,
                       const float* rstd, void* dag, void* u, void* dyb, float* dh, float* dw_part, int64_t rows, int F, gaot_stream_t stream);
```

Result: no change. 25.19 million points/s (-0.0%).
